# saiakarsh193/GenVox

Hardware: AMD Instinct MI355X
Metric: mel-frames/sec (teacher-forced batch) (higher is better)
Workload: dtype f32

## Files before the change

genvox_amd/_lib.py:

```python
from __future__ import annotations

import ctypes as C
import os

_HERE = os.path.dirname(os.path.abspath(__file__))
LIB_PATH = os.path.join(_HERE, os.environ.get("GVX_LIB", "libgenvox_amd.so"))


class GvxError(RuntimeError):
    pass


class gvx_dims(C.Structure):
    _fields_ = [(n, C.c_int32) for n in (
        "n_tokens", "embed_dim", "enc_kernel", "enc_n_conv", "prenet_dim", "att_rnn_dim", "dec_rnn_dim", "att_dim",
        "att_loc_filters", "att_loc_kernel", "postnet_dim", "postnet_kernel", "postnet_n_conv", "n_mels")]


class gvx_weight_desc(C.Structure):
    _fields_ = [("name", C.c_char_p), ("data", C.c_void_p), ("numel", C.c_int64)]


_vp, _i, _sz, _f, _l = C.c_void_p, C.c_int, C.c_size_t, C.c_float, C.c_long

# ... 137 lines not shown
    "gvx_wav_finalize_ragged": (_i, [_vp, _i, C.c_long, _vp, _i, _i, _i, C.POINTER(C.c_double), C.POINTER(C.c_double), _i, _vp, _vp, _vp]),
    "gvx_wav_to_mel_ragged_workspace_bytes": (_sz, [_vp, _i, C.c_long, _i]),
    "gvx_wav_trim_bounds": (_i, [_vp, _i, _i, C.c_long, _vp, _i, _f, _vp, _vp]),
    "gvx_wav_to_mel_ragged": (_i, [_vp, _vp, _i, _vp, _vp, _i, C.c_long, _vp, _i, _i, _i, _f, _i, _vp, _vp, _vp, _vp, _vp, _sz, _vp]),
    "gvx_resample_uses_lds_table": (_i, [_i, _i, _i]),
    "gvx_wav_mixdown": (_i, [_vp, _i, _i, C.c_long, _i, _vp, _vp]),
    "gvx_wav_resample_ragged": (_i, [_vp, _i, _i, C.c_long, _vp, _i, _i, _vp, _i, _vp, C.c_long, _vp, _vp]),
    "gvx_alignment_stats": (_i, [_vp, _vp, _vp, _i, _i, _i, _vp, _vp, _vp, _vp, _vp, _vp]),
    "gvx_mel_project": (_i, [_vp, _i, _i, _i, _vp, _i, _vp, _vp]),
    "gvx_dtw_workspace_bytes": (_sz, [_i, _i, _i, _i]),
    "gvx_dtw_uses_lds_tables": (_i, [_i, _i, _i]),
    "gvx_dtw_distance": (_i, [_vp, _vp, _vp, _vp, _i, _i, _i, _i, _vp, _vp, _vp, _sz, _vp]),
    "gvx_monotonic_align_workspace_bytes": (_sz, [_i, _i, _i]),
    "gvx_monotonic_align_uses_lds": (_i, [_i, _i]),
    "gvx_monotonic_align": (_i, [_vp, _vp, _vp, _i, _i, _i, _f, _vp, _vp, _vp, _vp, _vp, _vp, _vp, _sz, _vp]),
    "gvx_duration_scale": (_i, [_vp, _vp, _vp, _i, _i, _f, _vp, _vp, _vp, _vp, _vp]),
    "gvx_mel_time_warp": (_i, [_vp, _vp, _vp, _vp, _i, _i, _i, _i, _i, _vp, _vp, _vp, _vp, _vp]),
    "gvx_pitch_frames": (_i, [_l, _i]),
    "gvx_pitch_tile_frames": (_i, [C.POINTER(gvx_pitch_params)]),
    "gvx_pitch_yin": (_i, [_vp, _vp, _i, _l, C.POINTER(gvx_pitch_params), _vp, _vp, _vp, _vp, _vp]),
    "gvx_f0_compare": (_i, [_vp, _vp, _vp, _vp, _i, _i, _vp, _vp, _vp, _vp, _vp]),
    "gvx_psola_max_marks": (_l, [_l, _i]),
    "gvx_psola_max_grains": (_l, [_l, _i]),
    "gvx_psola_plan": (_i, [_vp, _vp, _vp, _vp, _i, _l, C.POINTER(gvx_psola_params), _vp, _vp, _vp, _vp, _vp, _vp, _vp]),
    "gvx_psola_synth": (_i, [_vp, _vp, _vp, _vp, _vp, _vp, _vp, _vp, _i, _l, C.POINTER(gvx_psola_params), _vp, _vp]),
    "gvx_melgan_blob_floats":(_sz, [C.POINTER(gvx_melgan_dims)]),
    "gvx_melgan_workspace_bytes": (_sz, [C.POINTER(gvx_melgan_dims), _i, _i]),
    "gvx_melgan_pack_weights_device": (_i, [C.POINTER(gvx_melgan_dims), C.POINTER(gvx_weight_desc), _i, _vp, _vp]),
    "gvx_melgan_create": (_i, [C.POINTER(gvx_melgan_dims), C.POINTER(_vp)]),
    "gvx_melgan_destroy": (None, [_vp]),
    "gvx_melgan_bind": (_i, [_vp, _vp]),
    "gvx_melgan_forward": (_i, [_vp, _vp, _vp, _i, _i, _vp, C.POINTER(_vp), _vp, _sz, _vp]),
    "gvx_melgan_timing_enable": (_i, [_vp, _i]),
    "gvx_melgan_stage_times_ms": (_i, [_vp, C.POINTER(_f), C.POINTER(_i)]),
    "gvx_melgan_tape_bytes": (_sz, [C.POINTER(gvx_melgan_dims), _i, _i]),
    "gvx_melgan_tape_layout": (_i, [C.POINTER(gvx_melgan_dims), _i, _i, C.POINTER(gvx_melgan_tape_entry), _i]),
    "gvx_melgan_backward_workspace_bytes": (_sz, [C.POINTER(gvx_melgan_dims), _i, _i]),
    "gvx_melgan_forward_train": (_i, [_vp, _vp, _vp, _i, _i, _vp, _vp, _sz, _vp, _sz, _vp]),
    "gvx_melgan_backward": (_i, [_vp, _vp, _vp, _i, _i, _vp, _sz, C.POINTER(gvx_weight_desc), _i, _vp, _vp, _sz, _vp]),
    "gvx_hifigan_blob_floats": (_sz, [C.POINTER(gvx_hifigan_dims)]),
    "gvx_hifigan_workspace_bytes": (_sz, [C.POINTER(gvx_hifigan_dims), _i, _i]),
    "gvx_hifigan_pack_weights_device": (_i, [C.POINTER(gvx_hifigan_dims), C.POINTER(gvx_weight_desc), _i, _vp, _vp]),
    "gvx_hifigan_create": (_i, [C.POINTER(gvx_hifigan_dims), C.POINTER(_vp)]),
    "gvx_hifigan_destroy": (None, [_vp]),
    "gvx_hifigan_bind": (_i, [_vp, _vp]),
    "gvx_hifigan_forward": (_i, [_vp, _vp, _vp, _i, _i, _vp, C.POINTER(_vp), _vp, _sz, _vp]),
    "gvx_hifigan_timing_enable": (_i, [_vp, _i]),
    "gvx_hifigan_stage_times_ms": (_i, [_vp, C.POINTER(_f), C.POINTER(_i)]),
    "gvx_hifigan_backward_stage_times_ms": (_i, [_vp, C.POINTER(_f), C.POINTER(_i)]),
    "gvx_hifigan_tape_bytes": (_sz, [C.POINTER(gvx_hifigan_dims), _i, _i]),
    "gvx_hifigan_tape_layout": (_i, [C.POINTER(gvx_hifigan_dims), _i, _i, C.POINTER(gvx_melgan_tape_entry), _i]),
    "gvx_hifigan_backward_workspace_bytes": (_sz, [C.POINTER(gvx_hifigan_dims), _i, _i]),
    "gvx_hifigan_forward_train": (_i, [_vp, _vp, _vp, _i, _i, _vp, _vp, _sz, _vp, _sz, _vp]),
    "gvx_hifigan_backward": (_i, [_vp, _vp, _vp, _i, _i, _vp, _sz, C.POINTER(gvx_weight_desc), _i, _vp, _vp, _sz, _vp]),
    "gvx_melgan_disc_blob_floats": (_sz, [C.POINTER(gvx_melgan_disc_dims)]),
    "gvx_melgan_disc_pack_weights_device": (_i, [C.POINTER(gvx_melgan_disc_dims), C.POINTER(gvx_weight_desc), _i, _vp, _vp]),
    "gvx_melgan_disc_create": (_i, [C.POINTER(gvx_melgan_disc_dims), C.POINTER(_vp)]),
    "gvx_melgan_disc_destroy": (None, [_vp]),
    "gvx_melgan_disc_bind": (_i, [_vp, _vp]),
    "gvx_melgan_disc_layout": (_i, [C.POINTER(gvx_melgan_disc_dims), _i, _i, C.POINTER(gvx_melgan_disc_entry), _i]),
    "gvx_melgan_disc_features_bytes": (_sz, [C.POINTER(gvx_melgan_disc_dims), _i, _i]),
    "gvx_melgan_disc_workspace_bytes": (_sz, [C.POINTER(gvx_melgan_disc_dims), _i, _i, _i]),
    "gvx_melgan_disc_forward": (_i, [_vp, _vp, _vp, _i, _i, _vp, _sz, _vp, _sz, _vp]),
    "gvx_melgan_disc_backward": (_i, [_vp, _vp, _vp, _i, _i, _vp, _vp, C.POINTER(gvx_weight_desc), _i, _vp, _vp, _sz, _vp]),
    "gvx_hifigan_mpd_blob_floats": (_sz, [C.POINTER(gvx_hifigan_mpd_dims)]),
    "gvx_hifigan_mpd_pack_weights_device": (_i, [C.POINTER(gvx_hifigan_mpd_dims), C.POINTER(gvx_weight_desc), _i, _vp, _vp]),
    "gvx_hifigan_mpd_create": (_i, [C.POINTER(gvx_hifigan_mpd_dims), C.POINTER(_vp)]),
    "gvx_hifigan_mpd_destroy": (None, [_vp]),
    "gvx_hifigan_mpd_bind": (_i, [_vp, _vp]),
    "gvx_hifigan_mpd_layout": (_i, [C.POINTER(gvx_hifigan_mpd_dims), _i, _i, C.POINTER(gvx_hifigan_mpd_entry), _i]),
    "gvx_hifigan_mpd_features_bytes": (_sz, [C.POINTER(gvx_hifigan_mpd_dims), _i, _i]),
    "gvx_hifigan_mpd_workspace_bytes": (_sz, [C.POINTER(gvx_hifigan_mpd_dims), _i, _i, _i]),
    "gvx_hifigan_mpd_forward": (_i, [_vp, _vp, _vp, _i, _i, _vp, _sz, _vp, _sz, _vp]),
    "gvx_hifigan_mpd_backward": (_i, [_vp, _vp, _vp, _i, _i, _vp, _vp, C.POINTER(gvx_weight_desc), _i, _vp, _vp, _sz, _vp]),
    "gvx_hifigan_mpd_timing_enable": (_i, [_vp, _i]),
    "gvx_hifigan_mpd_layer_times_ms": (_i, [_vp, C.POINTER(_f), C.POINTER(_f), C.POINTER(_i)]),
    "gvx_stft_loss_create": (_i, [C.POINTER(gvx_stft_resolution), _i, _f, _f, _f, C.POINTER(_vp)]),
    "gvx_stft_loss_destroy": (None, [_vp]),
    "gvx_stft_loss_workspace_bytes": (_sz, [_vp, _i, _l]),
    "gvx_stft_loss": (_i, [_vp, _vp, _vp, _vp, _i, _l, _vp, _vp, _vp, C.POINTER(gvx_stft_loss_debug), _vp, _sz, _vp]),
    "gvx_kernel_timing_enable": (_i, [_vp, _i]),
    "gvx_model_set_persistent_attention": (_i, [_vp, _i]),
    "gvx_model_set_resident_kernels": (_i, [_vp, _i]),
    "gvx_teacher_forced_rows_per_call": (_i, [_vp, _i]),
    "gvx_teacher_forced_resident": (_i, [_vp, _i, _i]),
    "gvx_teacher_forced_loop_kind": (_i, [_vp, _i, _i]),
    "gvx_autoregressive_loop_kind": (_i, [_vp, _i, _i]),
    "gvx_autoregressive_windowed_loop_kind": (_i, [_vp, _i, _i]),
    "gvx_kernel_times_ms": (_i, [_vp, C.POINTER(_f), C.POINTER(_f), C.POINTER(_i)]),
}

_lib = None


def load() -> C.CDLL:
    global _lib
    if _lib is not None:
        return _lib
    if not os.path.exists(LIB_PATH):
        raise ImportError(
            f"{LIB_PATH} not found: build the gfx950 library first (python -m genvox_amd.build, or "
            f"__graft_entry__.build()). genvox_amd has no CPU or eager fallback.")
    import torch

    lib = C.CDLL(LIB_PATH)
    for name, (res, args) in SIGNATURES.items():
        fn = getattr(lib, name)
        fn.restype = res
        fn.argtypes = args
    _lib = lib
    return lib


def check(rc: int) -> None:
    if rc != 0:
        msg = load().gvx_last_error()
        raise GvxError(f"genvox_amd error {rc}: {msg.decode() if msg else '?'}")
```

genvox_amd/build.py:

```python
from __future__ import annotations

import glob
import os
import subprocess
import sys
from concurrent.futures import ThreadPoolExecutor

HERE = os.path.dirname(os.path.abspath(__file__))
CSRC = os.path.join(HERE, "csrc")
LIB = os.path.join(HERE, "libgenvox_amd.so")
SOURCES = ["gemm_f32.hip", "skinny.hip", "dec_resident.hip", "attention.hip", "attn_persist.hip", "misc.hip", "griffinlim.hip", "wav_finalize.hip", "wav_to_mel.hip", "resample.hip", "eval_metrics.hip", "mas.hip", "time_warp.hip", "melgan.hip", "melgan_train.hip", "melgan_disc.hip", "hifigan.hip", "hifigan_train.hip", "hifigan_disc.hip", "pitch.hip", "psola.hip", "stft_loss.hip",
           "train_conv.hip", "train_ops.hip", "train_bptt_decoder.hip", "train_bptt_encoder.hip", "train_guided.hip", "gvx_pack.hip", "gvx_decoder.hip", "gvx_api.hip"]
ARCH = "gfx950"
HIPCC = os.environ.get("HIPCC", "/opt/rocm/bin/hipcc")
CXXFLAGS = ["-O3", "-std=c++17", "-fPIC", f"--offload-arch={ARCH}", "-Wall", "-Wno-unused-function",
            "-ffp-contract=off"]


def _newer(a: str, b: str) -> bool:
    return not os.path.exists(b) or os.path.getmtime(a) > os.path.getmtime(b)


def build(force: bool = False, verbose: bool = True, stamps: bool = False) -> str:
    objs, jobs = [], []
    flags = CXXFLAGS + (["-DGVX_STAMPS"] if stamps else []) + os.environ.get("GVX_EXTRA_FLAGS", "").split()
    lib = LIB.replace(".so", "_stamps.so") if stamps else LIB
    if os.environ.get("GVX_LIB_NAME"):
        lib = os.path.join(HERE, os.environ["GVX_LIB_NAME"])
    sfx = ".stamps.o" if stamps else ".o"
    if os.environ.get("GVX_LIB_NAME"):
        sfx = "." + os.environ["GVX_LIB_NAME"] + ".o"
    headers = sorted(glob.glob(os.path.join(CSRC, "*.h"))) + [os.path.join(os.path.dirname(HERE), "include", "genvox_amd.h")]
    for src in SOURCES:
        s = os.path.join(CSRC, src)
        o = os.path.join(CSRC, src.replace(".hip", sfx))
        objs.append(o)
        if force or _newer(s, o) or any(_newer(h, o) for h in headers):
            jobs.append([HIPCC, *flags, "-c", s, "-o", o])

    def run(cmd):
        if verbose:
            print(" ".join(cmd), flush=True)
        subprocess.run(cmd, check=True)

    if jobs:
        with ThreadPoolExecutor(max_workers=min(4, len(jobs))) as ex:
            list(ex.map(run, jobs))
    if jobs or not os.path.exists(lib):
        run([HIPCC, "-shared", "-fPIC", f"--offload-arch={ARCH}", *objs, "-L/opt/rocm/lib", "-lrocfft", "-Wl,-rpath,/opt/rocm/lib", "-o", lib])
    if not stamps and not os.environ.get("GVX_LIB_NAME"):
        variant = LIB.replace(".so", "_stamps.so")
        if os.path.exists(variant) and os.path.getmtime(variant) < os.path.getmtime(headers[-1]):
            os.remove(variant)
    return lib


if __name__ == "__main__":
    print(build(force="--force" in sys.argv, stamps="--stamps" in sys.argv))
```

genvox_amd/csrc/gemm_f32.hip:

```cpp
#include "gvx_kernels.h"

#include <cstdlib>

namespace gvx {

using f32x16 = __attribute__((ext_vector_type(16))) float;

constexpr int BK32 = 32;

__device__ __forceinline__ long row_off(const RowMap& m, int row) {
    return (long)(row / m.R) * m.s1 + (long)(row % m.R) * m.s0;
}

template <int WR, int WC, int TM, int TN, bool KMAJ = false, int BK = BK32>
__device__ __forceinline__ void gemm_f32_body(const GemmParams& p, const int block_x, const int tid, float* smem) {
    constexpr int LDS_LD = BK + 4;
    static_assert(BK == 32 || (BK == 64 && !KMAJ), "k-tiles of 32, or 64 for the row-major form");
    constexpr int BM = WR * TM * 32;
    constexpr int BN = WC * TN * 32;
    constexpr int NT = WR * WC * 64;
    constexpr int TPR = BK / 4;
    constexpr int RPP = NT / TPR;
    constexpr int A_V4 = (BM + RPP - 1) / RPP;
    constexpr int B_V4 = (BN + RPP - 1) / RPP;
    static_assert(!KMAJ || NT == 256, "the K-major loaders are written for 256 threads");
    float* As = smem;
    float* Bs = smem + 2 * BM * LDS_LD;

    const int lane = tid & 63, wave = tid >> 6;
    const int wr = wave / WC, wc = wave % WC;
    const int r = lane & 31, h = lane >> 5;
    const int n_tiles = (p.N + BN - 1) / BN;
    const int mt = block_x / n_tiles, nt = block_x % n_tiles;
    const int m0 = p.m_begin + mt * BM, n0 = nt * BN;
    const int k_begin = p.splitk > 1 ? (int)blockIdx.y * p.kchunk : 0;
    const int k_end = p.splitk > 1 ? min(p.K, k_begin + p.kchunk) : p.K;
    float* const Cout = p.C + (p.splitk > 1 ? (long)blockIdx.y * p.c_split : 0);

    const int ld_row = tid / TPR, ld_c4 = tid % TPR;
    const float* a_ptr[A_V4]; bool a_ok[A_V4];
    const float* b_ptr[B_V4]; bool b_ok[B_V4];
    constexpr int A_MQ = BM / 4, B_NQ = BN / 4;
    constexpr int A_P = (8 * A_MQ + 255) / 256, B_P = (8 * B_NQ + 255) / 256;
    const int amq = tid % A_MQ, akq = tid / A_MQ, bnq = tid % B_NQ, bkq = tid / B_NQ;
    const int a_col = min(m0 + 4 * amq, p.M - 4), b_col = min(n0 + 4 * bnq, p.N - 4);
    int ak_g[A_P], ak_i[A_P], bk_g[B_P], bk_i[B_P];
    long a_safe = 0, b_safe = 0;
    float4 ka_reg[A_P][4], kb_reg[B_P][4];
    if (KMAJ) {
#pragma unroll
        for (int i = 0; i < A_P; ++i) { const int k = k_begin + 4 * (akq + (256 / A_MQ) * i); ak_g[i] = k / p.amap.R; ak_i[i] = k - ak_g[i] * p.amap.R; }
#pragma unroll
        for (int i = 0; i < B_P; ++i) { const int k = k_begin + 4 * (bkq + (256 / B_NQ) * i); bk_g[i] = k / p.wmap.R; bk_i[i] = k - bk_g[i] * p.wmap.R; }
        a_safe = row_off(p.amap, k_begin); b_safe = row_off(p.wmap, k_begin);
    }
    if (!KMAJ) {
#pragma unroll
        for (int i = 0; i < A_V4; ++i) {
            int m = m0 + ld_row + RPP * i;
            a_ok[i] = m < p.M;
            a_ptr[i] = p.A + (a_ok[i] ? row_off(p.amap, m) : 0);
        }
#pragma unroll
        for (int i = 0; i < B_V4; ++i) {
            int n = n0 + ld_row + RPP * i;
            b_ok[i] = n < p.N;
            b_ptr[i] = p.W + (b_ok[i] ? (long)n * p.ldw : 0);
        }
    }
    float4 a_reg[A_V4], b_reg[B_V4];

#define GEMM_KMAJ_LOAD(NP, QPP, KQ, KG, KI, MAP, SAFE, PTR, COL, REG)                                        \
        _Pragma("unroll") for (int i = 0; i < NP; ++i) {                                                    \
            const int c_ = KQ + QPP * i;                                                                    \
            if (c_ < BK / 4) {                                                                              \
                const int kq_ = (K0_) + 4 * c_;                                                             \
                int g_ = KG[i], x_ = KI[i];                                                                 \
                _Pragma("unroll") for (int j = 0; j < 4; ++j) {                                             \
                    const bool ok_ = kq_ + j < k_end;                                                       \
                    REG[i][j] = *reinterpret_cast<const float4*>(PTR + (ok_ ? (long)g_ * MAP.s1 + (long)x_ * MAP.s0 : SAFE) + COL); \
                    if (++x_ == MAP.R) { x_ = 0; ++g_; }                                                    \
                }                                                                                           \
                x_ = KI[i] + BK; g_ = KG[i];                                                                \
                while (x_ >= MAP.R) { x_ -= MAP.R; ++g_; }                                                  \
                KI[i] = x_; KG[i] = g_;                                                                     \
            }                                                                                               \
        }
#define GEMM_LOAD_TILE(K0)                                                                                  \
    if (KMAJ) {                                                                                             \
        const int K0_ = (K0);                                                                               \
        GEMM_KMAJ_LOAD(A_P, (256 / A_MQ), akq, ak_g, ak_i, p.amap, a_safe, p.A, a_col, ka_reg)              \
        GEMM_KMAJ_LOAD(B_P, (256 / B_NQ), bkq, bk_g, bk_i, p.wmap, b_safe, p.W, b_col, kb_reg)              \
    } else                                                                                                  \
    {                                                                                                       \
        const int k_ = (K0) + 4 * ld_c4;                                                                    \
        const bool k_ok_ = k_ < k_end;                                                                      \
        const long a_koff_ = (long)(k_ >> 3) * p.a_kblk + (k_ & 7);                                         \
        _Pragma("unroll") for (int i = 0; i < A_V4; ++i) {                                                  \
            if (BM % RPP != 0 && ld_row + RPP * i >= BM) continue;                                          \
            a_reg[i] = *reinterpret_cast<const float4*>(a_ptr[i] + (k_ok_ ? a_koff_ : 0));                  \
        }                                                                                                   \
        _Pragma("unroll") for (int i = 0; i < B_V4; ++i) {                                                  \
            if (BN % RPP != 0 && ld_row + RPP * i >= BN) continue;                                          \
            b_reg[i] = *reinterpret_cast<const float4*>(b_ptr[i] + (k_ok_ ? k_ : 0));                       \
        }                                                                                                   \
    }
#define GEMM_KMAJ_STORE(NP, QPP, KQ, SM, ROWS, RQ, REG, BUF)                                                 \
        _Pragma("unroll") for (int i = 0; i < NP; ++i) {                                                    \
            const int c_ = KQ + QPP * i;                                                                    \
            if (c_ < BK / 4) {                                                                              \
                float* d_ = &SM[((BUF) * ROWS + 4 * RQ) * LDS_LD + 4 * c_];                                 \
                const int kq_ = (KS_) + 4 * c_;    \
                const bool o0_ = kq_ < k_end, o1_ = kq_ + 1 < k_end, o2_ = kq_ + 2 < k_end, o3_ = kq_ + 3 < k_end;   \
                *reinterpret_cast<float4*>(d_) = make_float4(o0_ ? REG[i][0].x : 0.f, o1_ ? REG[i][1].x : 0.f, o2_ ? REG[i][2].x : 0.f, o3_ ? REG[i][3].x : 0.f);              \
                *reinterpret_cast<float4*>(d_ + LDS_LD) = make_float4(o0_ ? REG[i][0].y : 0.f, o1_ ? REG[i][1].y : 0.f, o2_ ? REG[i][2].y : 0.f, o3_ ? REG[i][3].y : 0.f);     \
                *reinterpret_cast<float4*>(d_ + 2 * LDS_LD) = make_float4(o0_ ? REG[i][0].z : 0.f, o1_ ? REG[i][1].z : 0.f, o2_ ? REG[i][2].z : 0.f, o3_ ? REG[i][3].z : 0.f); \
                *reinterpret_cast<float4*>(d_ + 3 * LDS_LD) = make_float4(o0_ ? REG[i][0].w : 0.f, o1_ ? REG[i][1].w : 0.f, o2_ ? REG[i][2].w : 0.f, o3_ ? REG[i][3].w : 0.f); \
            }                                                                                               \
        }
#define GEMM_STORE_TILE(BUF, K0)                                                                            \
    if (KMAJ) {                                                                                             \
        const int KS_ = (K0);                                                                               \
        GEMM_KMAJ_STORE(A_P, (256 / A_MQ), akq, As, BM, amq, ka_reg, BUF)                                   \
        GEMM_KMAJ_STORE(B_P, (256 / B_NQ), bkq, Bs, BN, bnq, kb_reg, BUF)                                   \
    } else                                                                                                  \
    {                                                                                                       \
        const bool s_ok_ = (K0) + 4 * ld_c4 < k_end;    \
        _Pragma("unroll") for (int i = 0; i < A_V4; ++i)                                                    \
            if (BM % RPP == 0 || ld_row + RPP * i < BM)                                                     \
                *reinterpret_cast<float4*>(&As[((BUF) * BM + ld_row + RPP * i) * LDS_LD + 4 * ld_c4]) =     \
                    make_float4(s_ok_ ? a_reg[i].x : 0.f, s_ok_ ? a_reg[i].y : 0.f, s_ok_ ? a_reg[i].z : 0.f, s_ok_ ? a_reg[i].w : 0.f); \
        _Pragma("unroll") for (int i = 0; i < B_V4; ++i)                                                    \
            if (BN % RPP == 0 || ld_row + RPP * i < BN)                                                     \
                *reinterpret_cast<float4*>(&Bs[((BUF) * BN + ld_row + RPP * i) * LDS_LD + 4 * ld_c4]) =     \
                    make_float4(s_ok_ ? b_reg[i].x : 0.f, s_ok_ ? b_reg[i].y : 0.f, s_ok_ ? b_reg[i].z : 0.f, s_ok_ ? b_reg[i].w : 0.f); \
    }
#define GEMM_COMPUTE_TILE(BUF) GEMM_COMPUTE_KGS(BUF, 0, BK / 8)
#define GEMM_COMPUTE_KGS(BUF, KG0, KG1)              \
    {                                                                                                       \
        const float* a_base = &As[((BUF) * BM + wr * TM * 32 + r) * LDS_LD + 4 * h];                        \
        const float* b_base = &Bs[((BUF) * BN + wc * TN * 32 + r) * LDS_LD + 4 * h];                        \
        _Pragma("unroll") for (int kg = (KG0); kg < (KG1); ++kg) {                                          \
            float4 af[TM], bf[TN];                                                                          \
            _Pragma("unroll") for (int i = 0; i < TM; ++i)                                                  \
                af[i] = *reinterpret_cast<const float4*>(a_base + i * 32 * LDS_LD + 8 * kg);                \
            _Pragma("unroll") for (int j = 0; j < TN; ++j)                                                  \
                bf[j] = *reinterpret_cast<const float4*>(b_base + j * 32 * LDS_LD + 8 * kg);                \
            _Pragma("unroll") for (int i = 0; i < TM; ++i)                                                  \
                _Pragma("unroll") for (int j = 0; j < TN; ++j) {                                            \
                    acc[i][j] = __builtin_amdgcn_mfma_f32_32x32x2f32(af[i].x, bf[j].x, acc[i][j], 0, 0, 0); \
                    acc[i][j] = __builtin_amdgcn_mfma_f32_32x32x2f32(af[i].y, bf[j].y, acc[i][j], 0, 0, 0); \
                    acc[i][j] = __builtin_amdgcn_mfma_f32_32x32x2f32(af[i].z, bf[j].z, acc[i][j], 0, 0, 0); \
                    acc[i][j] = __builtin_amdgcn_mfma_f32_32x32x2f32(af[i].w, bf[j].w, acc[i][j], 0, 0, 0); \
                }                                                                                           \
        }                                                                                                   \
    }

    f32x16 acc[TM][TN];
#pragma unroll
    for (int i = 0; i < TM; ++i)
#pragma unroll
        for (int j = 0; j < TN; ++j)
#pragma unroll
            for (int q = 0; q < 16; ++q) acc[i][j][q] = 0.f;

    const int nkt = (k_end - k_begin + BK - 1) / BK;
    GEMM_LOAD_TILE(k_begin)
    GEMM_STORE_TILE(0, k_begin)
    __syncthreads();
    int kt = 0;
    for (; kt + 1 < nkt; ++kt) {
        const int cur = kt & 1;
        GEMM_LOAD_TILE(k_begin + (kt + 1) * BK)
        __builtin_amdgcn_sched_barrier(0);
        GEMM_COMPUTE_KGS(cur, 0, BK / 8 - 1)
        __builtin_amdgcn_sched_barrier(0);
        GEMM_COMPUTE_KGS(cur, BK / 8 - 1, BK / 8)
        GEMM_STORE_TILE(cur ^ 1, k_begin + (kt + 1) * BK)
        __syncthreads();
    }
    GEMM_COMPUTE_TILE(kt & 1)
#undef GEMM_LOAD_TILE
#undef GEMM_KMAJ_LOAD
#undef GEMM_KMAJ_STORE
#undef GEMM_STORE_TILE
#undef GEMM_COMPUTE_TILE
#undef GEMM_COMPUTE_KGS

#pragma unroll
    for (int i = 0; i < TM; ++i) {
#pragma unroll
        for (int q = 0; q < 16; ++q) {
            const int m = m0 + (wr * TM + i) * 32 + (q & 3) + 8 * (q >> 2) + 4 * h;
            if (m >= p.M) continue;
            const long c_off = row_off(p.cmap, m);
            const int grp = m / p.cmap.R, idx = m - grp * p.cmap.R;
            const bool live = !p.row_len || idx < p.row_len[grp];
            const bool halo_front = p.c_halo > 0 && idx < p.c_halo;
            const bool halo_back = p.c_halo > 0 && idx >= p.cmap.R - p.c_halo;
            const long halo_step = (long)p.c_halo * p.cmap.s0;
#pragma unroll
            for (int j = 0; j < TN; ++j) {
                const int n = n0 + (wc * TN + j) * 32 + r;
                if (n >= p.N) continue;
                float v = acc[i][j][q];
                if (p.bias) v += p.bias[n];
                if (p.act == ACT_RELU) v = fmaxf(v, 0.f);
                else if (p.act == ACT_TANH) v = tanhf(v);
                if (p.keep) v = p.keep[(long)m * p.keep_ld + n] ? 2.f * v : 0.f;
                const long col = (long)(n >> 3) * p.c_nblk + (n & 7);
                Cout[c_off + col] = live ? v : 0.f;
                if (halo_front) Cout[c_off - halo_step + col] = 0.f;
                if (halo_back) Cout[c_off + halo_step + col] = 0.f;
            }
        }
    }
}

template <int WR, int WC, int TM, int TN, bool KMAJ = false, int BK = BK32>
__global__ __launch_bounds__(WR * WC * 64) void gemm_f32_kernel(GemmParams p) {
    extern __shared__ __attribute__((aligned(16))) float smem[];
    gemm_f32_body<WR, WC, TM, TN, KMAJ, BK>(p, (int)blockIdx.x, (int)threadIdx.x, smem);
}

template <int WR, int WC, int TM, int TN, int BK = BK32>
static size_t lds_bytes_cfg() { return (size_t)2 * (WR * TM * 32 + WC * TN * 32) * (BK + 4) * sizeof(float); }

template <int WR, int WC, int TM, int TN, bool KMAJ = false, int BK = BK32>
static hipError_t init_cfg() {
    return hipFuncSetAttribute(reinterpret_cast<const void*>(gemm_f32_kernel<WR, WC, TM, TN, KMAJ, BK>),
                               hipFuncAttributeMaxDynamicSharedMemorySize, (int)lds_bytes_cfg<WR, WC, TM, TN, BK>());
}

hipError_t gemm_init() {
    hipError_t e = init_cfg<2, 2, 2, 2>();
    if (e != hipSuccess) return e;
    e = init_cfg<2, 2, 1, 2>();
    if (e != hipSuccess) return e;
    e = init_cfg<4, 1, 1, 3>();
    if (e != hipSuccess) return e;
    e = init_cfg<2, 3, 1, 1>();
    if (e != hipSuccess) return e;
    e = init_cfg<4, 2, 1, 2>();
    if (e != hipSuccess) return e;
    e = init_cfg<2, 2, 1, 1>();
    if (e != hipSuccess) return e;
    e = init_cfg<2, 2, 2, 2, true>();
    if (e != hipSuccess) return e;
    e = init_cfg<2, 2, 1, 2, true>();
    if (e != hipSuccess) return e;
    return init_cfg<4, 1, 1, 1>();
}

template <int WR, int WC, int TM, int TN, bool KMAJ = false, int BK = BK32>
static hipError_t launch_cfg(const GemmParams& p, hipStream_t s) {
    constexpr int BM = WR * TM * 32, BN = WC * TN * 32;
    const int grid = ((p.M - p.m_begin + BM - 1) / BM) * ((p.N + BN - 1) / BN);
    gemm_f32_kernel<WR, WC, TM, TN, KMAJ, BK><<<dim3(grid, p.splitk > 1 ? p.splitk : 1), dim3(WR * WC * 64), lds_bytes_cfg<WR, WC, TM, TN, BK>(), s>>>(p);
    return hipGetLastError();
}

static bool four_waves() {
    static const bool on = [] { const char* e = std::getenv("GVX_GEMM_8W"); return e && e[0] == '0'; }();
    return on;
}

GemmPlan plan_gemm(const GemmParams& p) {
    GemmPlan pl{hipSuccess, 0, 0};
    if (p.M <= 0 || p.N <= 0) return pl;
    if (p.kmajor) {
        if ((p.M & 3) || (p.N & 3) || p.M < 4 || p.N < 4 || ((p.amap.s0 | p.amap.s1 | p.wmap.s0 | p.wmap.s1) & 3)) { pl.err = hipErrorInvalidValue; return pl; }
        const long t128 = (long)((p.M + 127) / 128) * ((p.N + 127) / 128);
        pl.tile = t128 < 384 ? 2212 : 2222;
        return pl;
    }
    if (p.K & 3) { pl.err = hipErrorInvalidValue; return pl; }
    if (p.N <= 32) { pl.tile = 4111; return pl; }
    if (p.N <= 96) {
        pl.tile = p.M - p.m_begin <= 4096 ? 2311 : 4113;
        return pl;
    }
    const long n_tiles = (p.N + 127) / 128, tiles128 = (long)((p.M + 127) / 128) * n_tiles;
    if (tiles128 < 192) { pl.tile = 2211; return pl; }
    if (tiles128 < 384) { pl.tile = 2212; return pl; }
    pl.tile = four_waves() ? 2222 : 4212;
    const long rem = tiles128 % 256;
    if (p.splitk <= 1 && p.m_begin == 0 && rem > 0 && rem <= 64) {
        const long rows_big = ((tiles128 - rem) / n_tiles) * 128;
        if (rows_big > 0 && rows_big < p.M) pl.rows_big = (int)rows_big;
    }
    return pl;
}

static hipError_t launch_tile(int tile, const GemmParams& p, hipStream_t s) {
    switch (tile) {
        case 4111: return launch_cfg<4, 1, 1, 1>(p, s);
        case 2311: return launch_cfg<2, 3, 1, 1>(p, s);
        case 4113: return launch_cfg<4, 1, 1, 3>(p, s);
        case 2211: return launch_cfg<2, 2, 1, 1>(p, s);
        case 2212: return p.kmajor ? launch_cfg<2, 2, 1, 2, true>(p, s) : launch_cfg<2, 2, 1, 2>(p, s);
        case 2222: return p.kmajor ? launch_cfg<2, 2, 2, 2, true>(p, s) : launch_cfg<2, 2, 2, 2>(p, s);
        case 4212: return launch_cfg<4, 2, 1, 2>(p, s);
    }
    return hipErrorInvalidValue;
}

hipError_t launch_gemm(const GemmParams& p, hipStream_t s) {
    const GemmPlan pl = plan_gemm(p);
    if (pl.err != hipSuccess || pl.tile == 0) return pl.err;
    if (pl.rows_big == 0) return launch_tile(pl.tile, p, s);
    GemmParams a = p, b = p;
    a.M = pl.rows_big;
    b.m_begin = pl.rows_big;
    const hipError_t e = launch_tile(pl.tile, a, s);
    if (e != hipSuccess) return e;
    return launch_tile(2211, b, s);
}

void set_splitk(GemmParams& p, int splitk) {
    p.kchunk = ((p.K + splitk - 1) / splitk + 63) / 64 * 64;
    p.splitk = (p.K + p.kchunk - 1) / p.kchunk;
}

__global__ void splitk_reduce_kernel(const float* part, int splitk, long MN, int N, const float* bias, float* out, long ldc) {
    for (long i = (long)blockIdx.x * blockDim.x + threadIdx.x; i < MN; i += (long)gridDim.x * blockDim.x) {
        float v = part[i];
        for (int s = 1; s < splitk; ++s) v += part[(long)s * MN + i];
        const int n = (int)(i % N);
        if (bias) v += bias[n];
        out[(i / N) * ldc + n] = v;
    }
}

hipError_t launch_gemm_splitk(const GemmParams& p0, int splitk, float* scratch, hipStream_t s) {
    if (splitk <= 1) return launch_gemm(p0, s);
    if (p0.act != ACT_NONE || p0.keep || p0.row_len || p0.c_halo || p0.c_nblk != 8 || p0.cmap.s1 != 0 || p0.cmap.R < p0.M || !scratch)
        return hipErrorInvalidValue;
    GemmParams p = p0;
    set_splitk(p, splitk);
    p.C = scratch; p.cmap = RowMap{p.M, 0, (long)p.N};
    p.c_split = (long)p.M * p.N;
    p.bias = nullptr;
    hipError_t e = launch_gemm(p, s);
    if (e != hipSuccess) return e;
    const long MN = (long)p.M * p.N;
    long blocks = (MN + 255) / 256;
    if (blocks > 2048) blocks = 2048;
    splitk_reduce_kernel<<<dim3((unsigned)blocks), dim3(256), 0, s>>>(scratch, p.splitk, MN, p.N, p0.bias, p0.C, p0.cmap.s0);
    return hipGetLastError();
}

}
```

genvox_amd/csrc/gvx_api.hip:

```cpp
#include "gvx_internal.h"

namespace gvx {
#ifdef GVX_STAMPS
hipError_t read_stamps_skinny(unsigned long long* host96);
hipError_t read_stamps_attention(unsigned long long* host96);
hipError_t read_stamps_persist(unsigned long long* host96);
hipError_t read_wg_spans(unsigned long long* host1024);
hipError_t read_stamps_resident(unsigned long long* host480);
hipError_t read_wg_stamps_resident(unsigned long long* host896);
hipError_t read_wg_stamps_resident_ar(unsigned long long* host896);
hipError_t read_row_stamps_persist_ar(unsigned long long* host256);
hipError_t read_loc_stamps_persist(unsigned long long* host32);
hipError_t read_row_stamps_persist(unsigned long long* host512);
#endif
hipError_t skinny_init();
hipError_t gemm_init();
hipError_t attention_init();
hipError_t attention_persistent_init();
}

using namespace gvx;

namespace {
thread_local std::string g_err;
std::mutex g_capture_mutex;
}
namespace gvx {
int set_error(int code, const char* msg) { g_err = msg; return code; }

int fail(int code, const char* fmt, ...) {
    char buf[1024];
    va_list ap;
    va_start(ap, fmt);
    vsnprintf(buf, sizeof buf, fmt, ap);
    va_end(ap);
    g_err = buf;
    return code;
}

std::mutex& capture_mutex() { return g_capture_mutex; }

WsPlan make_ws_plan(const gvx_model* m, int B, int L, int T, int mode) {
    const gvx_dims& d = m->d;
    const int E = d.embed_dim, H = E / 2, M = d.n_mels, P = d.prenet_dim, A = d.att_rnn_dim, D = d.dec_rnn_dim;
    const int pe = (d.enc_kernel - 1) / 2, pp = (d.postnet_kernel - 1) / 2;
    WsPlan w{};
    size_t off = 0;
    auto take = [&](size_t floats) { size_t o = off; off = align_up(off + floats * sizeof(float), 256); return o; };
    w.flags = take(128);
    w.sync = take(HANDOFF_WORDS);
    w.xa = take((size_t)B * (L + 2 * pe) * E);
    w.xb = take((size_t)B * (L + 2 * pe) * E);
    w.xg = take((size_t)B * L * 8 * H);
    w.enc_h = take((size_t)2 * 2 * B * H);
    w.enc_c = take((size_t)2 * B * H);
    w.memory = take((size_t)B * L * E);
    w.len_copy = take((size_t)B);
    w.pm = take((size_t)B * L * d.att_dim);
    w.frames = take((size_t)(T + 1) * B * M);
    w.pre1 = take((size_t)(T + 1) * B * P);
    w.prenet = take((size_t)(T + 1) * B * P);
    w.h_a = take((size_t)RS_HA_SLOTS * B * A);
    w.c_a = take((size_t)B * A);
    w.c_d = take((size_t)B * D);
    w.hc = take((size_t)(T + 1) * B * (D + E));
    w.w_cum = take((size_t)B * L);
    w.q_slab = take((size_t)(A / 8) * B * d.att_dim);
    w.proj = take((size_t)B * T * m->PSB());
    w.energies = take((size_t)B * L);
    w.align_tm = take((size_t)T * B * L);
    w.loc = take((size_t)B * L * d.att_dim);
    w.p_slab = take((size_t)(D / 8) * B * m->PSB());
    w.p_ctx = take((size_t)B * m->PSB());
    w.att_part = take((size_t)2 * B * 4 * A);
    w.dec_part = take((size_t)2 * B * 4 * D);
    w.pre_gate = take(mode == WS_TEACHER_FORCED && plan_teacher_forced(m, B, L, TF_INFERENCE).pre_gate ? (size_t)T * B * 4 * A : 0);
    w.xchg = take(attention_persistent_xchg_floats(B));
    w.ar_masks = take(((size_t)2 * T * B * P + 3) / 4);
    const int cmax = d.postnet_dim > M ? d.postnet_dim : M;
    w.ya = take((size_t)B * (T + 2 * pp) * cmax);
    w.yb = take((size_t)B * (T + 2 * pp) * cmax);
    w.total = off;
    return w;
}

gvx_model::GraphSet* touch_graph_set(gvx_model* m, std::vector<gvx_model::GraphSet>& cache, const gvx_model::LoopKey& key) {
    gvx_model::GraphSet* hit = nullptr;
    for (auto& gs : cache)
        if (gs.key == key) hit = &gs;
    if (!hit) {
        if (cache.size() >= gvx_model::GRAPH_SETS) {
            size_t lru = 0;
            for (size_t i = 1; i < cache.size(); ++i)
                if (cache[i].last_use < cache[lru].last_use) lru = i;
            for (auto e : cache[lru].execs)
                if (e) (void)hipGraphExecDestroy(e);
            cache.erase(cache.begin() + lru);
        }
        cache.emplace_back();
        hit = &cache.back();
        hit->key = key;
    }
    ++hit->sightings;
    hit->last_use = ++m->use_clock;
    return hit;
}

int check_common(const gvx_model* m, int B, int L, int T, void* ws, size_t ws_bytes, int mode) {
    if (!m) return fail(GVX_ERR_INVALID_ARG, "null model");
    if (!m->dev_blob) return fail(GVX_ERR_STATE, "weights not bound (call gvx_model_bind_blob)");
    if (B < 1 || B > 64) return fail(GVX_ERR_UNSUPPORTED, "batch %d not in [1, 64] (shard larger batches across calls / GPUs)", B);
    if (L < 1 || T < 1) return fail(GVX_ERR_INVALID_ARG, "L and T must be >= 1");
    if (!ws) return fail(GVX_ERR_WORKSPACE, "null workspace");
    if (reinterpret_cast<uintptr_t>(ws) & 255) return fail(GVX_ERR_WORKSPACE, "workspace must be 256-byte aligned");
    const size_t need = make_ws_plan(m, B, L, T, mode).total;
    if (ws_bytes < need) return fail(GVX_ERR_WORKSPACE, "workspace too small: %zu < %zu bytes", ws_bytes, need);
    if (!attention_supported(L, m->d.att_dim, m->d.att_loc_filters, m->d.att_loc_kernel, m->d.embed_dim))
        return fail(GVX_ERR_UNSUPPORTED, "L = %d is too long for the attention kernels' LDS budget", L);
    return GVX_OK;
}

}

namespace {

int check_dims(const gvx_dims& d) {
    if (d.n_tokens < 1) return fail(GVX_ERR_INVALID_ARG, "n_tokens must be >= 1");
    const int dims8[] = {d.embed_dim, d.prenet_dim, d.att_rnn_dim, d.dec_rnn_dim, d.att_dim, d.postnet_dim, d.n_mels};
    const char* names[] = {"embed_dim", "prenet_dim", "att_rnn_dim", "dec_rnn_dim", "att_dim", "postnet_dim", "n_mels"};
    for (int i = 0; i < 7; ++i)
        if (dims8[i] < 8 || dims8[i] % 8) return fail(GVX_ERR_UNSUPPORTED, "%s = %d must be a positive multiple of 8", names[i], dims8[i]);
    if (d.embed_dim % 16) return fail(GVX_ERR_UNSUPPORTED, "embed_dim = %d must be a multiple of 16 (BiLSTM halves are multiples of 8)", d.embed_dim);
    if (d.att_dim > 256) return fail(GVX_ERR_UNSUPPORTED, "att_dim = %d > 256 is not supported", d.att_dim);
    if (d.att_loc_filters < 1 || d.att_loc_filters > 32) return fail(GVX_ERR_UNSUPPORTED, "att_loc_filters = %d must be in [1, 32]", d.att_loc_filters);
    const int ks[] = {d.enc_kernel, d.att_loc_kernel, d.postnet_kernel};
    for (int k : ks)
        if (k < 1 || k % 2 == 0) return fail(GVX_ERR_UNSUPPORTED, "kernel size %d must be odd (the reference pads (k-1)/2 on both sides)", k);
    if (d.enc_n_conv < 1 || d.enc_n_conv > MAX_CONV || d.postnet_n_conv < 1 || d.postnet_n_conv > MAX_CONV)
        return fail(GVX_ERR_UNSUPPORTED, "number of convolutions must be in [1, %d]", MAX_CONV);
    return GVX_OK;
}

void read_knobs(gvx_model* m) {
    auto env = [](const char* name) { const char* e = std::getenv(name); return e ? e : ""; };
    auto flag = [&](const char* name, bool dflt) { const char c = env(name)[0]; return c == '\0' ? dflt : dflt ? c != '0' : c == '1'; };
    auto number = [&](const char* name, int dflt) { const char* e = env(name); return e[0] ? std::atoi(e) : dflt; };
    m->use_graph = !flag("GVX_NO_GRAPH", false);
    m->capture_first = flag("GVX_GRAPH_FIRST", false);
    m->attn_one_launch = !flag("GVX_ATTN_SPLIT", false);
    m->attn_persistent = flag("GVX_ATTN_PERSISTENT", true);
    for (const char* name : {"AMD_SERIALIZE_KERNEL", "HIP_LAUNCH_BLOCKING"})
        if (env(name)[0] != '\0' && env(name)[0] != '0') m->attn_persistent = false;
    m->ar_resident = flag("GVX_AR_RESIDENT", false);
    m->ar_split_h = flag("GVX_AR_SPLIT_H", true);
    m->enc_persistent = flag("GVX_ENC_PERSISTENT", true);
    m->enc_fork_after = number("GVX_ENC_FORK_AFTER", 1);
    m->train_resident = flag("GVX_TRAIN_RESIDENT", true);
    m->train_resident_loop = flag("GVX_TRAIN_RESIDENT_LOOP", true);
    m->tf_rows64 = flag("GVX_TF_ROWS64", false);
    m->tf_resident = flag("GVX_TF_RESIDENT", true);
    m->ar_resident_loop = flag("GVX_AR_RESIDENT_LOOP", true);
    m->tf_long_rows_224 = flag("GVX_TF_LONG_224", true);
    m->attn_prefetch = flag("GVX_ATTN_PREFETCH", true);
    m->pa_depth = number("GVX_PA_DEPTH", 4) == 6 ? 6 : 4;
    m->side_pool = env("GVX_SIDE_POOL")[0] == '2' ? 2u : 1u;
    m->spin_limit = (unsigned)std::strtoul(env("GVX_HANDOFF_SPIN_LIMIT"), nullptr, 10);
    m->rs_debug = number("GVX_RS_DEBUG", 0);
    m->debug_skip_resident = flag("GVX_DEBUG_SKIP_RESIDENT", false);
    m->debug_enc_skip_block = number("GVX_DEBUG_ENC_SKIP_BLOCK", -1);
    m->debug_plan = std::getenv("GVX_DEBUG_PLAN") != nullptr;
}

}

extern "C" {

const char* gvx_last_error(void) { return g_err.c_str(); }
int gvx_version(void) { return 1; }

int gvx_model_create(const gvx_dims* dims, gvx_model** out) {
    if (!dims || !out) return fail(GVX_ERR_INVALID_ARG, "null argument");
    int rc = check_dims(*dims);
    if (rc != GVX_OK) return rc;
    gvx_model* m = new gvx_model();
    m->d = *dims;
    m->blob = make_blob_layout(*dims);
    read_knobs(m);
    *out = m;
    return GVX_OK;
}

void gvx_model_destroy(gvx_model* m) {
    if (m) {
        if (m->gather_off) (void)hipFree(m->gather_off);
        if (m->gather_tid) (void)hipFree(m->gather_tid);
    }
    if (!m) return;
    if (m->ev_valid)
        for (auto& e : m->ev) (void)hipEventDestroy(e);
    for (auto& e : m->kev) (void)hipEventDestroy(e);
    m->drop_graphs();
    if (m->cap_stream) (void)hipStreamDestroy(m->cap_stream);
    if (m->pa_fork) (void)hipEventDestroy(m->pa_fork);
    if (m->pa_join) (void)hipEventDestroy(m->pa_join);
    if (m->enc_mid) (void)hipEventDestroy(m->enc_mid);
    if (m->ar_done_host) (void)hipHostFree(m->ar_done_host);
    for (hipEvent_t e : m->ar_ev)
        if (e) (void)hipEventDestroy(e);
    delete m;
}

size_t gvx_model_blob_bytes(const gvx_model* m) { return m ? m->blob.total * sizeof(float) : 0; }

int gvx_model_bind_blob(gvx_model* m, const void* device_blob) {
    if (!m || !device_blob) return fail(GVX_ERR_INVALID_ARG, "null argument");
    if (reinterpret_cast<uintptr_t>(device_blob) & 255) return fail(GVX_ERR_INVALID_ARG, "blob must be 256-byte aligned");
    if (m->dev_blob != device_blob) m->drop_graphs();
    m->dev_blob = reinterpret_cast<const float*>(device_blob);
    HIP_TRY(gemm_init());
    HIP_TRY(skinny_init());
    HIP_TRY(attention_init());
    HIP_TRY(attention_persistent_init());
    HIP_TRY(decoder_resident_init());
    return GVX_OK;
}

size_t gvx_workspace_bytes(const gvx_model* m, int B, int L, int T) {
    if (!m || B < 1 || L < 1 || T < 1) return 0;
    return make_ws_plan(m, B, L, T).total;
}

size_t gvx_workspace_bytes_autoregressive(const gvx_model* m, int B, int L, int max_steps) {
    if (!m || B < 1 || L < 1 || max_steps < 1) return 0;
    return make_ws_plan(m, B, L, max_steps, WS_AUTOREGRESSIVE).total;
}

}

namespace {

int conv_layer(const gvx_model* m, const float* in, float* out, int B, int T, int cin, int cout, int k, size_t w_off, size_t b_off,
               int act, int out_halo, hipStream_t s) {
    const int p = (k - 1) / 2;
    GemmParams g{};
    g.A = in; g.amap = RowMap{T, (long)(T + 2 * p) * cin, (long)cin};
    g.W = m->dev_blob + w_off; g.ldw = (long)k * cin;
    g.C = out + (long)out_halo * cout; g.cmap = RowMap{T, (long)(T + 2 * out_halo) * cout, (long)cout};
    g.bias = m->dev_blob + b_off;
    g.M = B * T; g.N = cout; g.K = k * cin; g.act = act;
    HIP_TRY(launch_gemm(g, s));
    return GVX_OK;
}

// ... 11 lines not shown
    float* cur = xa;
    float* nxt = xb;
    if (conv_out) {
        HIP_TRY(launch_to_channels_last(conv_out, xa, B, E, L, pe, nullptr, s));
    } else {
        HIP_TRY(launch_embed(tokens, m->dev_blob + m->blob.emb, d.n_tokens, xa, xb, B, L, E, pe, flags + FLAG_TOKEN, s));
        for (int i = 0; i < d.enc_n_conv; ++i) {
            if (dense_done && i == m->enc_fork_after) { HIP_TRY(hipEventRecord(dense_done, s)); dense_done = nullptr; }
            int rc = conv_layer(m, cur, nxt, B, L, E, E, d.enc_kernel, m->blob.enc_w[i], m->blob.enc_b[i], ACT_RELU, pe, s);
            if (rc != GVX_OK) return rc;
            float* t = cur; cur = nxt; nxt = t;
        }
    }
    if (dense_done) HIP_TRY(hipEventRecord(dense_done, s));
    {
        GemmParams g{};
        g.A = cur + (long)pe * E; g.amap = RowMap{L, (long)(L + 2 * pe) * E, (long)E};
        g.W = m->dev_blob + m->blob.enc_wih; g.ldw = E;
        g.C = xg; g.cmap = RowMap{B * L, 0, (long)8 * H};
        g.bias = m->dev_blob + m->blob.enc_bih;
        g.M = B * L; g.N = 8 * H; g.K = E; g.act = ACT_NONE;
        HIP_TRY(launch_gemm(g, s));
    }
    const bool resident = m->enc_persistent && encoder_persistent_supported(B, H);
    if (!resident) HIP_TRY(zero_async(enc_h, (size_t)4 * B * H * sizeof(float), s));
    if (!resident) HIP_TRY(zero_async(enc_c, (size_t)2 * B * H * sizeof(float), s));
    float* mem_ws = ws_ptr<float>(ws, wp.memory);
    if (!resident) HIP_TRY(zero_async(mem_ws, (size_t)B * L * E * sizeof(float), s));
    const int32_t* len_ws = nullptr;
    if (lengths) {
        int32_t* lc = ws_ptr<int32_t>(ws, wp.len_copy);
        HIP_TRY(hipMemcpyAsync(lc, lengths, (size_t)B * sizeof(int32_t), hipMemcpyDeviceToDevice, s));
        len_ws = lc;
    }
    auto enqueue = [&](hipStream_t st) -> int {
        for (int step = 0; step < L; ++step) {
            SkinnyJob jobs[2];
            for (int dir = 0; dir < 2; ++dir) {
                SkinnyJob& J = jobs[dir];
                std::memset(&J, 0, sizeof J);
                float* h_cur = enc_h + ((size_t)dir * 2 + (step & 1)) * B * H;
                float* h_nxt = enc_h + ((size_t)dir * 2 + ((step + 1) & 1)) * B * H;
                J.Wp = m->dev_blob + m->blob.enc_whh_frag[dir];
                J.x[0] = XSeg{h_cur, H};
                J.N = 4 * H; J.nkg = H / 8; J.mode = 0; J.B = B;
                J.c = enc_c + (size_t)dir * B * H;
                J.h_out = h_nxt;
                J.addend = xg + (size_t)dir * 4 * H; J.add_bs = (long)L * 8 * H; J.add_ts = 8 * H;
                J.lengths = len_ws; J.step = step; J.reverse = dir; J.seq_len = L;
                J.seq_out = mem_ws + (size_t)dir * H; J.seq_bs = (long)L * E; J.seq_ts = E;
                if (c_seq_out) J.c_seq_out = c_seq_out + (size_t)dir * H;
                J.h_prev = h_cur;
            }
            HIP_TRY(launch_skinny(jobs, 2, SK_ENCODER, st));
        }
        return GVX_OK;
    };
    if (resident) {
        unsigned* sync = ws_ptr<unsigned>(ws, wp.sync);
        void* const zp[2] = {enc_h, sync + HANDOFF_TIMEOUT};
        const size_t zb[2] = {(size_t)4 * B * H * sizeof(float), sizeof(unsigned)};
        HIP_TRY(launch_zero_many(zp, zb, 2, s));
        EncPersistParams ep{};
        ep.Wp[0] = m->dev_blob + m->blob.enc_whh_frag[0]; ep.Wp[1] = m->dev_blob + m->blob.enc_whh_frag[1];
        ep.xg = xg; ep.lengths = len_ws; ep.hx = enc_h; ep.seq_out = mem_ws; ep.c_seq_out = c_seq_out;
        ep.sync = sync; ep.spin_limit = m->spin_limit; ep.B = B; ep.L = L; ep.H = H;
        ep.debug_skip_block = m->debug_enc_skip_block;
        HIP_TRY(launch_encoder_persistent(ep, s));
        float* outs[2] = {mem_ws, c_seq_out};
        const size_t counts[2] = {(size_t)B * L * E, (size_t)B * L * E};
        HIP_TRY(launch_poison_on_timeout(sync + HANDOFF_TIMEOUT, flags + FLAG_TIMEOUT, outs, counts, c_seq_out ? 2 : 1, s));
    } else {
        const gvx_model::LoopKey key{ws, mem_ws, m->dev_blob, B, L, 0, lengths != nullptr};
        const int rc = run_chunk(m, m->use_graph && !c_seq_out ? touch_graph_set(m, m->enc_graphs, key) : nullptr, 0, s, enqueue);
        if (rc != GVX_OK) return rc;
    }
    if (xg_out) HIP_TRY(hipMemcpyAsync(xg_out, xg, (size_t)B * L * 8 * H * sizeof(float), hipMemcpyDeviceToDevice, s));
    if (memory_out != mem_ws)
        HIP_TRY(hipMemcpyAsync(memory_out, mem_ws, (size_t)B * L * E * sizeof(float), hipMemcpyDeviceToDevice, s));
    return GVX_OK;
}

int postnet_impl(gvx_model* m, const float* mel_in, const int32_t* mel_lengths, int B, int T, float* mel_post_out, float* ya,
                 float* yb, hipStream_t s) {
    const gvx_dims& d = m->d;
    const int M = d.n_mels, pp = (d.postnet_kernel - 1) / 2, n = d.postnet_n_conv;
    HIP_TRY(launch_to_channels_last(mel_in, ya, B, M, T, pp, mel_lengths, s));
    float* cur = ya;
    float* nxt = yb;
    for (int i = 0; i < n; ++i) {
        const int cin = i == 0 ? M : d.postnet_dim, cout = i == n - 1 ? M : d.postnet_dim;
        const bool last = i == n - 1;
        const int out_halo = last ? 0 : pp;
        const bool fused_halo = out_halo > 0 && T >= out_halo;
        if (out_halo > 0 && !fused_halo) HIP_TRY(launch_zero_halo(nxt, B, T, pp, cout, s));
        GemmParams g{};
        g.A = cur; g.amap = RowMap{T, (long)(T + 2 * pp) * cin, (long)cin};
        g.W = m->dev_blob + m->blob.post_w[i]; g.ldw = (long)d.postnet_kernel * cin;
        g.C = nxt + (long)out_halo * cout; g.cmap = RowMap{T, (long)(T + 2 * out_halo) * cout, (long)cout};
        g.bias = m->dev_blob + m->blob.post_b[i];
        g.M = B * T; g.N = cout; g.K = d.postnet_kernel * cin; g.act = last ? ACT_NONE : ACT_TANH;
        g.row_len = last ? nullptr : mel_lengths;
        g.c_halo = fused_halo ? out_halo : 0;
        HIP_TRY(launch_gemm(g, s));
        float* t = cur; cur = nxt; nxt = t;
    }
    HIP_TRY(launch_residual_to_channels_first(mel_in, cur, mel_post_out, B, M, T, mel_lengths, s));
    return GVX_OK;
}

struct PostnetPlan { size_t ya, yb, total; };
PostnetPlan make_postnet_plan(const gvx_model* m, int B, int T) {
    const gvx_dims& d = m->d;
    const int pp = (d.postnet_kernel - 1) / 2, cmax = d.postnet_dim > d.n_mels ? d.postnet_dim : d.n_mels;
    const size_t buf = align_up((size_t)B * (T + 2 * pp) * cmax * sizeof(float), 256);
    PostnetPlan p;
    p.ya = align_up((128 + HANDOFF_WORDS) * sizeof(float), 256);
    p.yb = p.ya + buf;
    p.total = p.yb + buf;
    return p;
}

}

extern "C" {

int gvx_teacher_forced_rows_per_call(const gvx_model* m, int L) {
    if (!m) return 0;
    return plan_teacher_forced(m, 64, L, TF_INFERENCE).kind != 0 ? 64 : 32;
}

int gvx_teacher_forced_resident(const gvx_model* m, int B, int L) {
    if (!m || B < 1 || L < 1) return 0;
    return plan_teacher_forced(m, B, L, TF_INFERENCE).kind != 0 ? 1 : 0;
}

int gvx_teacher_forced_loop_kind(const gvx_model* m, int B, int L) {
    if (!m || B < 1 || L < 1) return 0;
    return plan_teacher_forced(m, B, L, TF_INFERENCE).kind;
}

int gvx_autoregressive_loop_kind(const gvx_model* m, int B, int L) {
    if (!m || B < 1 || L < 1) return 0;
    return plan_autoregressive(m, B, L).kind;
}

int gvx_autoregressive_windowed_loop_kind(const gvx_model* m, int B, int L) {
    if (!m || B < 1 || L < 1) return 0;
    return plan_autoregressive(m, B, L, true).kind;
}

int gvx_debug_decoder_plan_windowed(const gvx_model* m, int B, int L, int* out) {
    if (!m || !out) return fail(GVX_ERR_INVALID_ARG, "null argument");
    if (B < 1 || L < 1) return fail(GVX_ERR_INVALID_ARG, "B, L >= 1 (got %d, %d)", B, L);
    const ArLoopPlan a = plan_autoregressive(m, B, L, true);
    out[0] = a.kind; out[1] = a.split_h; out[2] = a.fold; out[3] = a.graph;
    return GVX_OK;
}

int gvx_debug_decoder_plan(const gvx_model* m, int mode, int B, int L, int* out) {
    if (!m || !out) return fail(GVX_ERR_INVALID_ARG, "null argument");
    if (mode < 0 || mode > 2 || B < 1 || L < 1) return fail(GVX_ERR_INVALID_ARG, "mode must be 0, 1 or 2 and B, L >= 1 (got %d, %d, %d)", mode, B, L);
    const TfLoopPlan t = plan_teacher_forced(m, B, L, (TfMode)mode);
    const ArLoopPlan a = plan_autoregressive(m, B, L);
    const int v[12] = {t.kind, t.pa_layout, t.tile_layout, t.rows64, t.pre_gate, t.timeout_check, t.side_stream, t.graph,
                       a.kind, a.split_h, a.fold, a.graph};
    for (int i = 0; i < 12; ++i) out[i] = v[i];
    return GVX_OK;
}

long long gvx_debug_graph_replays(const gvx_model* m) { return m ? (long long)m->graph_replays : -1; }

int gvx_debug_encoder_resident(const gvx_model* m, int B) {
    if (!m || B < 1) return 0;
    return m->enc_persistent && encoder_persistent_supported(B, m->H()) ? 1 : 0;
}

int gvx_model_set_persistent_attention(gvx_model* m, int enable) {
    if (!m) return fail(GVX_ERR_INVALID_ARG, "null argument");
    m->attn_persistent = enable != 0;
    return GVX_OK;
}

int gvx_model_set_resident_kernels(gvx_model* m, int enable) {
    if (!m) return fail(GVX_ERR_INVALID_ARG, "null argument");
    m->attn_persistent = m->enc_persistent = m->tf_resident = enable != 0;
    if (!enable) m->ar_resident = false;
    return GVX_OK;
}

int gvx_workspace_status(const gvx_model* m, void* ws, size_t ws_bytes, void* stream, int32_t* host_out) {
    if (!m || !ws || !host_out) return fail(GVX_ERR_INVALID_ARG, "null argument");
    const WsPlan wp = make_ws_plan(m, 1, 1, 1, WS_AUTOREGRESSIVE);
    if (ws_bytes < wp.flags + 4 * sizeof(int32_t)) return fail(GVX_ERR_WORKSPACE, "workspace too small");
    hipStream_t s = (hipStream_t)stream;
    int32_t h[4] = {0, 0, 0, 0}, tmo = 0;
    int32_t* flags = ws_ptr<int32_t>(ws, wp.flags);
    HIP_TRY(hipMemcpyAsync(h, flags, sizeof h, hipMemcpyDeviceToHost, s));
    if (ws_bytes >= wp.sync + HANDOFF_WORDS * sizeof(unsigned))
        HIP_TRY(hipMemcpyAsync(&tmo, reinterpret_cast<const char*>(ws) + wp.sync + HANDOFF_TIMEOUT * sizeof(unsigned), sizeof tmo,
                               hipMemcpyDeviceToHost, s));
    HIP_TRY(zero_async(flags + FLAG_TOKEN, sizeof(int32_t), s));
    HIP_TRY(zero_async(flags + FLAG_TIMEOUT, sizeof(int32_t), s));
    if (ws_bytes >= wp.sync + HANDOFF_WORDS * sizeof(unsigned))
        HIP_TRY(zero_async(ws_ptr<unsigned>(ws, wp.sync) + HANDOFF_TIMEOUT, sizeof(unsigned), s));
    HIP_TRY(hipStreamSynchronize(s));
    host_out[0] = h[FLAG_TOKEN];
    host_out[1] = h[FLAG_TIMEOUT] ? h[FLAG_TIMEOUT] : tmo;
    return GVX_OK;
}

int gvx_encoder_forward(gvx_model* m, const int64_t* tokens, const int32_t* lengths, int B, int L, float* memory_out,
                        void* ws, size_t ws_bytes, void* stream) {
    int rc = check_common(m, B, L, 1, ws, ws_bytes, WS_AUTOREGRESSIVE);
    if (rc != GVX_OK) return rc;
    if (!tokens || !memory_out) return fail(GVX_ERR_INVALID_ARG, "null argument");
    return encoder_impl(m, tokens, lengths, B, L, memory_out, ws, make_ws_plan(m, B, L, 1, WS_AUTOREGRESSIVE), (hipStream_t)stream);
}

int gvx_decoder_teacher_forced(gvx_model* m, const float* memory, const int32_t* lengths, int B, int L, const float* mel_in, int T,
                               const uint8_t* keep_masks, float* mel_out, float* gate_out, float* align_out, void* ws,
                               size_t ws_bytes, void* stream) {
    int rc = check_common(m, B, L, T, ws, ws_bytes);
    if (rc != GVX_OK) return rc;
    if (!memory || !mel_in || !keep_masks || !mel_out || !gate_out || !align_out) return fail(GVX_ERR_INVALID_ARG, "null argument");
    const WsPlan wp = make_ws_plan(m, B, L, T);
    rc = decoder_tf_impl(m, memory, lengths, B, L, mel_in, T, keep_masks, mel_out, gate_out, align_out, ws, wp, (hipStream_t)stream);
    if (rc != GVX_OK) return rc;
    float* outs[3] = {mel_out, gate_out, align_out};
    const size_t counts[3] = {(size_t)B * m->d.n_mels * T, (size_t)B * T, (size_t)B * T * L};
    return poison_if_timed_out(m, B, L, ws, wp, outs, counts, 3, (hipStream_t)stream);
}

int gvx_encoder_lstm_forward(gvx_model* m, const float* conv_out, const int32_t* lengths, int B, int L, float* memory_out,
                             float* cell_states_out, float* input_preact_out, void* ws, size_t ws_bytes, void* stream) {
    int rc = check_common(m, B, L, 1, ws, ws_bytes, WS_AUTOREGRESSIVE);
    if (rc != GVX_OK) return rc;
    if (!conv_out || !memory_out) return fail(GVX_ERR_INVALID_ARG, "null argument");
    if (cell_states_out) HIP_TRY(zero_async(cell_states_out, (size_t)B * L * m->d.embed_dim * sizeof(float), (hipStream_t)stream));
    return encoder_impl(m, nullptr, lengths, B, L, memory_out, ws, make_ws_plan(m, B, L, 1, WS_AUTOREGRESSIVE), (hipStream_t)stream, conv_out,
                        cell_states_out, input_preact_out);
}

int gvx_decoder_teacher_forced_train(gvx_model* m, const float* memory, const int32_t* lengths, int B, int L, const float* mel_in, int T,
                                     const uint8_t* keep_masks, const uint8_t* att_keep, const uint8_t* dec_keep, float p_att, float p_dec,
                                     float* mel_out, float* gate_out, float* align_out, float* att_hidden_all, float* att_cell_all,
                                     float* dec_cell_all, float* dec_hidden_context_all, float* att_preact_all, float* dec_preact_all,
                                     void* ws, size_t ws_bytes, void* stream) {
    int rc = check_common(m, B, L, T, ws, ws_bytes);
    if (rc != GVX_OK) return rc;
    if (!memory || !mel_in || !keep_masks || !att_keep || !dec_keep || !mel_out || !gate_out || !align_out) return fail(GVX_ERR_INVALID_ARG, "null argument");
    if (!(p_att >= 0.f && p_att < 1.f && p_dec >= 0.f && p_dec < 1.f)) return fail(GVX_ERR_INVALID_ARG, "dropout probabilities must be in [0, 1)");
    if (plan_teacher_forced(m, B, L, TF_TRAIN_PARTIAL_TAPE).rows64)
        return fail(GVX_ERR_UNSUPPORTED, "training mode with %d rows on a GVX_TF_ROWS64 handle: the 64-row loop has no dropout and no tape (at most 32 rows per call)", B);
    hipStream_t s = (hipStream_t)stream;
    const int A = m->d.att_rnn_dim, D = m->d.dec_rnn_dim, E = m->d.embed_dim;
    const LstmDropout tr{att_keep, dec_keep, 1.f / (1.f - p_att), 1.f / (1.f - p_dec), att_hidden_all, att_cell_all, dec_cell_all, att_preact_all, dec_preact_all};
    if (att_hidden_all) HIP_TRY(zero_async(att_hidden_all, (size_t)B * A * sizeof(float), s));
    if (att_cell_all) HIP_TRY(zero_async(att_cell_all, (size_t)B * A * sizeof(float), s));
    if (dec_cell_all) HIP_TRY(zero_async(dec_cell_all, (size_t)B * D * sizeof(float), s));
    const WsPlan wp = make_ws_plan(m, B, L, T);
    rc = decoder_tf_impl(m, memory, lengths, B, L, mel_in, T, keep_masks, mel_out, gate_out, align_out, ws, wp, s, false, &tr);
    if (rc != GVX_OK) return rc;
    {
        float* outs[3] = {mel_out, gate_out, align_out};
        const size_t counts[3] = {(size_t)B * m->d.n_mels * T, (size_t)B * T, (size_t)B * T * L};
        rc = poison_if_timed_out(m, B, L, ws, wp, outs, counts, 3, s);
        if (rc != GVX_OK) return rc;
    }
    if (dec_hidden_context_all)
        HIP_TRY(hipMemcpyAsync(dec_hidden_context_all, ws_ptr<float>(ws, wp.hc), (size_t)(T + 1) * B * (D + E) * sizeof(float),
                               hipMemcpyDeviceToDevice, s));
    return GVX_OK;
}

int gvx_train_export(const gvx_model* m, const void* ws_c, size_t ws_bytes, int B, int L, int T, int what, float* dst, void* stream) {
    void* ws = const_cast<void*>(ws_c);
    if (!m || !ws || !dst) return fail(GVX_ERR_INVALID_ARG, "null argument");
    const WsPlan wp = make_ws_plan(m, B, L, T);
    if (ws_bytes < wp.total) return fail(GVX_ERR_WORKSPACE, "workspace too small");
    const gvx_dims& d = m->d;
    hipStream_t s = (hipStream_t)stream;
    const size_t rows = (size_t)(T + 1) * B;
    switch (what) {
        case 0: HIP_TRY(hipMemcpyAsync(dst, ws_ptr<float>(ws, wp.frames), rows * d.n_mels * sizeof(float), hipMemcpyDeviceToDevice, s)); break;
        case 1: HIP_TRY(hipMemcpyAsync(dst, ws_ptr<float>(ws, wp.pre1), rows * d.prenet_dim * sizeof(float), hipMemcpyDeviceToDevice, s)); break;
        case 2: return gvx_train_unblock(ws_ptr<float>(ws, wp.prenet), dst, T + 1, B, d.prenet_dim, stream);
        case 3: HIP_TRY(hipMemcpyAsync(dst, ws_ptr<float>(ws, wp.pm), (size_t)B * L * d.att_dim * sizeof(float), hipMemcpyDeviceToDevice, s)); break;
        default: return fail(GVX_ERR_INVALID_ARG, "gvx_train_export: unknown buffer %d", what);
    }
    return GVX_OK;
}

size_t gvx_postnet_workspace_bytes(const gvx_model* m, int B, int T) {
    if (!m || B < 1 || T < 1) return 0;
    return make_postnet_plan(m, B, T).total;
}

int gvx_postnet_forward(gvx_model* m, const float* mel_in, const int32_t* mel_lengths, int B, int T, float* mel_post_out, void* ws,
                        size_t ws_bytes, void* stream) {
    if (!m) return fail(GVX_ERR_INVALID_ARG, "null model");
    if (!m->dev_blob) return fail(GVX_ERR_STATE, "weights not bound (call gvx_model_bind_blob)");
    if (B < 1 || T < 1) return fail(GVX_ERR_INVALID_ARG, "B and T must be >= 1");
    if ((long)B * T > (1L << 30)) return fail(GVX_ERR_UNSUPPORTED, "B * T = %ld frames exceed the GEMM row index range", (long)B * T);
    if (!ws) return fail(GVX_ERR_WORKSPACE, "null workspace");
    if (reinterpret_cast<uintptr_t>(ws) & 255) return fail(GVX_ERR_WORKSPACE, "workspace must be 256-byte aligned");
    const PostnetPlan pp = make_postnet_plan(m, B, T);
    if (ws_bytes < pp.total) return fail(GVX_ERR_WORKSPACE, "workspace too small: %zu < %zu bytes", ws_bytes, pp.total);
    if (!mel_in || !mel_post_out) return fail(GVX_ERR_INVALID_ARG, "null argument");
    return postnet_impl(m, mel_in, mel_lengths, B, T, mel_post_out, ws_ptr<float>(ws, pp.ya), ws_ptr<float>(ws, pp.yb), (hipStream_t)stream);
}

int gvx_mask_padding(float* mel, float* mel_post, float* gate, const int32_t* mel_lengths, int B, int n_mels, int T, void* stream) {
    if (!mel_lengths || B < 1 || T < 1 || n_mels < 1) return fail(GVX_ERR_INVALID_ARG, "bad argument");
    HIP_TRY(launch_mask_padding(mel, mel_post, gate, mel_lengths, B, n_mels, T, (hipStream_t)stream));
    return GVX_OK;
}

int gvx_tacotron2_forward(gvx_model* m, const int64_t* tokens, const int32_t* token_lengths, int B, int L, const float* mel_in,
                          const int32_t* mel_lengths, int T, const uint8_t* keep_masks, float* mel_out, float* mel_post_out,
                          float* gate_out, float* align_out, void* ws, size_t ws_bytes, void* stream) {
    int rc = check_common(m, B, L, T, ws, ws_bytes);
    if (rc != GVX_OK) return rc;
    if (!tokens || !mel_in || !keep_masks || !mel_out || !gate_out || !align_out)
        return fail(GVX_ERR_INVALID_ARG, "null argument");
    hipStream_t s = (hipStream_t)stream;
    const WsPlan wp = make_ws_plan(m, B, L, T);
    const bool timed = m->timing && m->ev_valid;
    float* memory = ws_ptr<float>(ws, wp.memory);
    if (timed) HIP_TRY(hipEventRecord(m->ev[0], s));
    const bool overlap = plan_teacher_forced(m, B, L, TF_INFERENCE).side_stream;
    if (overlap) {
        rc = ensure_side_stream(m);
        if (rc != GVX_OK) return rc;
        HIP_TRY(hipEventRecord(m->pa_fork, s));
        HIP_TRY(hipStreamWaitEvent(m->pa_stream, m->pa_fork, 0));
        rc = encoder_impl(m, tokens, token_lengths, B, L, memory, ws, wp, m->pa_stream, nullptr, nullptr, nullptr, m->enc_mid);
        if (rc != GVX_OK) return rc;
        rc = decoder_init_states(m, memory, B, L, decoder_buffers(ws, wp), m->pa_stream);
        if (rc != GVX_OK) return rc;
        HIP_TRY(hipEventRecord(m->pa_join, m->pa_stream));
        HIP_TRY(hipStreamWaitEvent(s, m->enc_mid, 0));
        rc = decoder_prenet_part(m, B, L, mel_in, T, keep_masks, ws, wp, s);
        if (rc != GVX_OK) return rc;
        HIP_TRY(hipStreamWaitEvent(s, m->pa_join, 0));
    } else {
        rc = encoder_impl(m, tokens, token_lengths, B, L, memory, ws, wp, s);
        if (rc != GVX_OK) return rc;
    }
    if (timed) HIP_TRY(hipEventRecord(m->ev[1], s));
    rc = decoder_tf_impl(m, memory, token_lengths, B, L, mel_in, T, keep_masks, mel_out, gate_out, align_out, ws, wp, s, overlap);
    if (rc != GVX_OK) return rc;
    if (timed) HIP_TRY(hipEventRecord(m->ev[4], s));
    if (mel_post_out) {
        rc = postnet_impl(m, mel_out, nullptr, B, T, mel_post_out, ws_ptr<float>(ws, wp.ya), ws_ptr<float>(ws, wp.yb), s);
        if (rc != GVX_OK) return rc;
        if (mel_lengths) HIP_TRY(launch_mask_padding(mel_out, mel_post_out, gate_out, mel_lengths, B, m->d.n_mels, T, s));
    }
    float* outs[4] = {mel_out, gate_out, align_out, mel_post_out};
    const size_t nm = (size_t)B * m->d.n_mels * T;
    const size_t counts[4] = {nm, (size_t)B * T, (size_t)B * T * L, nm};
    rc = poison_if_timed_out(m, B, L, ws, wp, outs, counts, mel_post_out ? 4 : 3, s);
    if (rc != GVX_OK) return rc;
    if (timed) HIP_TRY(hipEventRecord(m->ev[5], s));
    return GVX_OK;
}

int gvx_tacotron2_loss(const float* mel_out, const float* mel_post_out, const float* gate_out, const float* mel_target,
                       const float* gate_target, int B, int n_mels, int T, float* loss_out, void* scratch, size_t scratch_bytes,
                       void* stream) {
    if (!mel_out || !mel_post_out || !gate_out || !mel_target || !gate_target || !loss_out || !scratch)
        return fail(GVX_ERR_INVALID_ARG, "null argument");
    if (B < 1 || n_mels < 1 || T < 1) return fail(GVX_ERR_INVALID_ARG, "B, n_mels and T must be >= 1");
    if (scratch_bytes < loss_scratch_bytes() || (reinterpret_cast<uintptr_t>(scratch) & 7))
        return fail(GVX_ERR_WORKSPACE, "scratch too small (%zu bytes needed) or not 8-byte aligned", loss_scratch_bytes());
    HIP_TRY(launch_tacotron2_loss(mel_out, mel_post_out, gate_out, mel_target, gate_target, (long)B * n_mels * T, (long)B * T,
                                  reinterpret_cast<double*>(scratch), loss_out, (hipStream_t)stream));
    return GVX_OK;
}

int gvx_prenet_masks_generate(uint8_t* masks_out, size_t n, uint64_t seed, void* stream) {
    if (!masks_out) return fail(GVX_ERR_INVALID_ARG, "null argument");
    HIP_TRY(launch_mask_gen(masks_out, n, seed, (hipStream_t)stream));
    return GVX_OK;
}

int gvx_stage_timing_enable(gvx_model* m, int enable) {
    if (!m) return fail(GVX_ERR_INVALID_ARG, "null model");
    if (enable && !m->ev_valid) {
        for (auto& e : m->ev) HIP_TRY(hipEventCreate(&e));
        m->ev_valid = true;
    }
    m->timing = enable != 0;
    return GVX_OK;
}

int gvx_kernel_timing_enable(gvx_model* m, int enable) {
    if (!m) return fail(GVX_ERR_INVALID_ARG, "null model");
    m->ktiming = enable != 0;
    return GVX_OK;
}

int gvx_kernel_times_ms(gvx_model* m, float* lstm_avg_ms, float* attn_avg_ms, int* n_steps) {
    if (!m || !lstm_avg_ms || !attn_avg_ms) return fail(GVX_ERR_INVALID_ARG, "null argument");
    if (m->n_lstm_ev < 1) return fail(GVX_ERR_STATE, "no timed decoder loop has run");
    HIP_TRY(hipEventSynchronize(m->kev[2]));
    float a = 0, b = 0;
    HIP_TRY(hipEventElapsedTime(&a, m->kev[0], m->kev[1]));
    HIP_TRY(hipEventElapsedTime(&b, m->kev[1], m->kev[2]));
    *lstm_avg_ms = a / m->n_lstm_ev;
    *attn_avg_ms = m->n_attn_ev > 0 ? b / m->n_attn_ev : 0.f;
    if (n_steps) *n_steps = m->n_lstm_ev;
    return GVX_OK;
}

int gvx_stage_times_ms(gvx_model* m, float* t5, int* launches) {
    if (!m || !t5) return fail(GVX_ERR_INVALID_ARG, "null argument");
    if (!m->ev_valid) return fail(GVX_ERR_STATE, "stage timing was not enabled");
    HIP_TRY(hipEventSynchronize(m->ev[5]));
    for (int i = 0; i < 5; ++i) HIP_TRY(hipEventElapsedTime(&t5[i], m->ev[i], m->ev[i + 1]));
    if (launches) *launches = m->last_decoder_launches;
    return GVX_OK;
}
#ifdef GVX_STAMPS
int gvx_debug_read_stamps_skinny(unsigned long long* host96) {
    HIP_TRY(hipDeviceSynchronize());
    HIP_TRY(gvx::read_stamps_skinny(host96));
    return GVX_OK;
}
int gvx_debug_read_stamps_persist(unsigned long long* host96) {
    HIP_TRY(hipDeviceSynchronize());
    HIP_TRY(gvx::read_stamps_persist(host96));
    return GVX_OK;
}
int gvx_debug_read_wg_spans(unsigned long long* host1024) {
    HIP_TRY(hipDeviceSynchronize());
    HIP_TRY(gvx::read_wg_spans(host1024));
    return GVX_OK;
// ... 35 lines not shown
```

genvox_amd/csrc/gvx_internal.h:

```cpp
#pragma once
#include "../../include/genvox_amd.h"
#include "gvx_kernels.h"

#include <cmath>
#include <cstdarg>
#include <cstdio>
#include <cstdlib>
#include <cstring>
#include <mutex>
#include <string>
#include <unordered_map>
#include <vector>

namespace gvx {

int fail(int code, const char* fmt, ...);

#define HIP_TRY(expr)                                                                          \
    do {                                                                                       \
        hipError_t _e = (expr);                                                                \
        if (_e != hipSuccess) return fail(GVX_ERR_HIP, "%s failed: %s", #expr, hipGetErrorString(_e)); \
    } while (0)

constexpr int MAX_CONV = 8;
constexpr double BN_EPS = 1e-5;

struct Blob {
    size_t emb;
    size_t enc_w[MAX_CONV], enc_b[MAX_CONV];
    size_t enc_wih, enc_bih, enc_whh_frag[2];
    size_t pre_w0, pre_w1, pre_w0_t, pre_w1_t;
    size_t att_frag, att_bias, att_wpre, wq_t, wmem, v, loc_conv, loc_dense;
    size_t dec_frag, dec_bias;
    size_t proj_w, proj_b, proj_frag, proj_hd_t, proj_ctx_frag, proj_ctx_t;
    size_t post_w[MAX_CONV], post_b[MAX_CONV];
    size_t total;
};
Blob make_blob_layout(const gvx_dims& d);

inline size_t frag_floats(int N, int K) { return (size_t)((N + 31) / 32) * (K / 8) * 64 * 4; }

struct WsPlan {
    size_t xa, xb, xg, enc_h, enc_c, flags, sync, memory;
    size_t pm, frames, pre1, prenet, h_a, c_a, c_d, hc, w_cum, q_slab, proj, energies, align_tm, len_copy, loc, ar_masks, p_slab, p_ctx;
    size_t att_part, dec_part, pre_gate, xchg;
    size_t ya, yb;
    size_t total;
};

}

struct gvx_model {
    gvx_dims d;
    gvx::Blob blob;
    const float* dev_blob = nullptr;
    bool use_graph = true;
    bool capture_first = false;
    bool attn_one_launch = true;
    bool attn_persistent = true;
    bool ar_resident = false;
    bool enc_persistent = true;
    bool ar_split_h = true;
    bool tf_rows64 = false;
    bool tf_resident = true;
    bool ar_resident_loop = true;
    bool tf_long_rows_224 = true;
    bool train_resident = true;
    bool train_resident_loop = true;
    bool attn_prefetch = true;
    int enc_fork_after = 1;
    int pa_depth = 4;
    unsigned side_pool = 1;
    unsigned spin_limit = 0;
    int rs_debug = 0;
    bool debug_skip_resident = false;
    int debug_enc_skip_block = -1;
    bool debug_plan = false;
    bool timing = false;
    hipEvent_t ev[6] = {nullptr, nullptr, nullptr, nullptr, nullptr, nullptr};
    bool ev_valid = false;
    int last_decoder_launches = 0;
    struct LoopKey {
        const void* ws; const void* memory; const void* blob; int B, L, T; bool has_len;
        float threshold = 0.f;
        int variant = 0;
        const void* centres = nullptr; int win_back = 0, win_ahead = 0;
        bool operator==(const LoopKey& o) const {
            return ws == o.ws && memory == o.memory && blob == o.blob && B == o.B && L == o.L && T == o.T &&
                   has_len == o.has_len && threshold == o.threshold && variant == o.variant && centres == o.centres &&
                   win_back == o.win_back && win_ahead == o.win_ahead;
        }
    };
    struct GraphSet {
        LoopKey key;
        int sightings = 0;
        uint64_t last_use = 0;
        std::vector<hipGraphExec_t> execs;
    };
    static constexpr size_t GRAPH_SETS = 4;
    std::vector<GraphSet> ar_graphs, loop_graphs, enc_graphs;
    uint64_t use_clock = 0;
    uint64_t graph_replays = 0;
    hipStream_t pa_stream = nullptr;
    hipEvent_t pa_fork = nullptr, pa_join = nullptr, enc_mid = nullptr;
    int32_t* ar_done_host = nullptr;
    hipEvent_t ar_ev[2] = {nullptr, nullptr};
    std::vector<std::string> gather_names;
    std::vector<int64_t> gather_numel;
    int32_t* gather_off = nullptr;
    uint8_t* gather_tid = nullptr;
    void drop_graphs() {
        for (auto* c : {&ar_graphs, &loop_graphs, &enc_graphs}) {
            for (auto& gs : *c)
                for (auto e : gs.execs)
                    if (e) (void)hipGraphExecDestroy(e);
            c->clear();
        }
    }
    hipStream_t cap_stream = nullptr;
    bool ktiming = false;
    std::vector<hipEvent_t> kev;
    int n_lstm_ev = 0, n_attn_ev = 0;
    int reserve_events(size_t n) {
        while (kev.size() < n) {
            hipEvent_t e;
            if (hipEventCreate(&e) != hipSuccess) return GVX_ERR_HIP;
            kev.push_back(e);
        }
        return GVX_OK;
    }
    int H() const { return d.embed_dim / 2; }
    int PS() const { return (d.n_mels + 1 + 3) & ~3; }
    int PSB() const { return (d.n_mels + 1 + 7) & ~7; }
};

namespace gvx {

enum TfMode : int { TF_INFERENCE = 0, TF_TRAIN_WHOLE_TAPE = 1, TF_TRAIN_PARTIAL_TAPE = 2 };
struct TfLoopPlan {
    int kind;
    int pa_layout;
    int tile_layout;
    bool rows64;
    bool pre_gate;
    bool timeout_check;
    bool side_stream;
    bool graph;
};
struct ArLoopPlan {
    int kind;
    bool split_h;
    bool fold;
    bool graph;
};
TfLoopPlan plan_teacher_forced(const gvx_model* m, int B, int L, TfMode mode);
ArLoopPlan plan_autoregressive(const gvx_model* m, int B, int L, bool windowed = false);

enum WsMode : int { WS_TEACHER_FORCED = 0, WS_AUTOREGRESSIVE = 1 };

constexpr int FLAG_TOKEN = 0;
constexpr int FLAG_AR_DONE = 1;
constexpr int FLAG_TIMEOUT = 2;
constexpr int FLAG_AR_FRAMES = 64;

WsPlan make_ws_plan(const gvx_model* m, int B, int L, int T, int mode = WS_TEACHER_FORCED);
int check_common(const gvx_model* m, int B, int L, int T, void* ws, size_t ws_bytes, int mode = WS_TEACHER_FORCED);

template <typename T>
T* ws_ptr(void* ws, size_t off) { return reinterpret_cast<T*>(reinterpret_cast<char*>(ws) + off); }

inline hipError_t zero_async(void* p, size_t bytes, hipStream_t s) { return hipMemsetAsync(p, 0, bytes, s); }

gvx_model::GraphSet* touch_graph_set(gvx_model* m, std::vector<gvx_model::GraphSet>& cache, const gvx_model::LoopKey& key);
std::mutex& capture_mutex();

template <class F>
int run_chunk(gvx_model* m, gvx_model::GraphSet* gs, size_t chunk, hipStream_t s, F&& enqueue) {
    if (!m->use_graph || !gs || (gs->sightings < 2 && !m->capture_first)) return enqueue(s);
    if (gs->execs.size() <= chunk) gs->execs.resize(chunk + 1, nullptr);
    hipGraphExec_t exec = gs->execs[chunk];
    if (!exec) {
        std::lock_guard<std::mutex> lock(capture_mutex());
        hipGraph_t graph = nullptr;
        if (!m->cap_stream) HIP_TRY(hipStreamCreateWithFlags(&m->cap_stream, hipStreamNonBlocking));
        HIP_TRY(hipStreamBeginCapture(m->cap_stream, hipStreamCaptureModeThreadLocal));
        const int rc = enqueue(m->cap_stream);
        const hipError_t ce = hipStreamEndCapture(m->cap_stream, &graph);
        if (rc != GVX_OK) { if (graph) (void)hipGraphDestroy(graph); return rc; }
        HIP_TRY(ce);
        HIP_TRY(hipGraphInstantiate(&exec, graph, nullptr, nullptr, 0));
        HIP_TRY(hipGraphDestroy(graph));
        gs->execs[chunk] = exec;
    }
    HIP_TRY(hipGraphLaunch(exec, s));
    ++m->graph_replays;
    return GVX_OK;
}

struct DecoderBuffers {
    float *pm, *frames, *pre1, *prenet, *h_a, *c_a, *c_d, *hc, *w_cum, *q_slab, *proj, *energies, *align_tm, *loc, *p_slab, *p_ctx;
    float *att_part, *dec_part, *pre_gate;
    int32_t* len_copy;
};
DecoderBuffers decoder_buffers(void* ws, const WsPlan& wp);

struct LstmDropout {
    const uint8_t* att_keep; const uint8_t* dec_keep; float att_scale, dec_scale;
    float* h_a_all; float* c_a_all; float* c_d_all;
    float* pre_a_all; float* pre_d_all;
};

int ensure_side_stream(gvx_model* m);
int decoder_init_states(gvx_model* m, const float* memory, int B, int L, const DecoderBuffers& db, hipStream_t s);
int decoder_prenet_part(gvx_model* m, int B, int L, const float* mel_in, int T, const uint8_t* keep_masks, void* ws, const WsPlan& wp,
                        hipStream_t s);
int decoder_tf_impl(gvx_model* m, const float* memory, const int32_t* lengths, int B, int L, const float* mel_in, int T,
                    const uint8_t* keep_masks, float* mel_out, float* gate_out, float* align_out, void* ws, const WsPlan& wp,
                    hipStream_t s, bool prenet_done = false, const LstmDropout* train = nullptr);
int poison_if_timed_out(const gvx_model* m, int B, int L, void* ws, const WsPlan& wp, float* const* outs, const size_t* counts, int n,
                        hipStream_t s);

}
```

genvox_amd/csrc/gvx_kernels.h:

```cpp
#pragma once
#include <hip/hip_runtime.h>
#include <stddef.h>
#include <stdint.h>

#ifdef GVX_STAMPS
namespace gvx { namespace { __device__ unsigned long long gvx_stamps[3][32]; } }
#define GVX_STAMP(k, i)                                                                         \
    do {                                                                                        \
        if (blockIdx.x == 0 && blockIdx.y == 0 && threadIdx.x == 0) gvx::gvx_stamps[k][i] = wall_clock64(); \
    } while (0)
#else
#define GVX_STAMP(k, i) do { } while (0)
#endif

namespace gvx {

int set_error(int code, const char* msg);

inline size_t align_up(size_t x, size_t a) { return (x + a - 1) / a * a; }

enum Act : int { ACT_NONE = 0, ACT_RELU = 1, ACT_TANH = 2 };

struct RowMap {
    int R;
    long s1, s0;
};

struct GemmParams {
    const float* A; RowMap amap; long a_kblk = 8;
    const float* W; long ldw;
    float* C; RowMap cmap; long c_nblk = 8;
    const float* bias;
    const uint8_t* keep; long keep_ld;
    int M, N, K;
    int act;
    int splitk = 1; int kchunk = 0; long c_split = 0;
    bool kmajor = false; RowMap wmap{1, 0, 0};
    int m_begin = 0;
    const int32_t* row_len = nullptr;
    int c_halo = 0;
};
hipError_t launch_gemm(const GemmParams& p, hipStream_t s);
struct GemmPlan { hipError_t err; int tile; int rows_big; };
GemmPlan plan_gemm(const GemmParams& p);
void set_splitk(GemmParams& p, int splitk);
hipError_t launch_gemm_splitk(const GemmParams& p, int splitk, float* scratch, hipStream_t s);

struct XSeg { const float* p; int len; };

struct SkinnyJob {
    const float* Wp;
    const float* bias;
    XSeg x[3];
    int N;
    int nkg;
    int kg0, nkg_w;
    int mode;
    float* c;
    float* h_out;
    const float* addend; long add_bs, add_ts;
    const float* addend2;
    const int32_t* lengths; int step; int reverse; int seq_len;
    float* seq_out; long seq_bs, seq_ts;
    const float* h_prev;
    const uint8_t* h_keep; float h_scale;
    float* c_out; float* c_seq_out;
    float* pre_out;
    const float* Wq_t;
    float* q_slab; int att_dim;
    const float* xw; const float* xsrc;
    int defer_seg;
    const unsigned* ctx_cnt; unsigned ctx_target;
    unsigned* start_cnt;
    const unsigned* ready_cnt; unsigned ready_target;
    unsigned* tmo;
    unsigned spin_limit;
    float* y;
    const uint8_t* keep; long keep_stride;
    int act;
    int B;
};
struct LocJob {
    const float* w_prev; long w_prev_bs;
    const float* w_cum;
    const float* loc_conv_t;
    const float* loc_dense_t;
    const float* pm;
    float* loc_out;
    int B, L, a, kl, G;
};
enum SkinnyKind : int { SK_DECODER = 0, SK_ENCODER = 1, SK_AR = 2, SK_TRAIN = 3 };
hipError_t launch_skinny(const SkinnyJob* jobs, int njobs, int kind, hipStream_t s, const LocJob* loc = nullptr);
struct AttnParams;
hipError_t launch_skinny_attn(const SkinnyJob* jobs, int njobs, const AttnParams& ap, hipStream_t s);
struct EncPersistParams {
    const float* Wp[2];
    const float* xg;
    const int32_t* lengths;
    float* hx;
    float* seq_out;
    float* c_seq_out;
    unsigned* sync;
    unsigned spin_limit;
    int B, L, H;
    int debug_skip_block;
};
bool encoder_persistent_supported(int B, int H);
hipError_t launch_encoder_persistent(const EncPersistParams& p, hipStream_t s);
hipError_t launch_skinny_pa(const SkinnyJob& att, const SkinnyJob* dec, hipStream_t s, int depth = 4, int layout = 1);
hipError_t launch_skinny_pa64(const SkinnyJob* jobs, int njobs, hipStream_t s);

struct AttnParams {
    const float* q_slab; int n_slabs;
    float* w_cum;
    const float* loc;
    const float* v;
    const float* pm;
    const float* memory;
    const int32_t* lengths;
    float* energies;
    float* w_out; long w_out_bs;
    float* ctx_out;
    int B, L, a, F, kl, E, G;
// ... 67 lines not shown
    const uint8_t* tr_keep_a; const uint8_t* tr_keep_d; float tr_scale_a, tr_scale_d;
    float* tr_c_a; float* tr_c_d; float* tr_pre_a; float* tr_pre_d;
};
struct ArResidentParams {
    const float* att_frag; const float* att_bias; const float* wq_t;
    const float* dec_frag; const float* dec_bias;
    const float* proj_hd_t;
    const float* proj_ctx_t;
    const float* pre_w1;
    const uint8_t* keep1;
    float* prenet;
    const float* y1;
    float* h_a; float* hc; float* q_slab;
    float* p_slab;
    float* c_a; float* c_d;
    const int32_t* n_done;
    unsigned* sync;
    unsigned att_frag_bytes;
    int B, T, PSB;
    unsigned spin_limit;
    int debug;
};
bool decoder_resident_supported(int B, int L);
hipError_t launch_decoder_ar_resident(const ArResidentParams& p, hipStream_t s);
hipError_t decoder_resident_init();
hipError_t launch_decoder_resident(const DecResidentParams& p, hipStream_t s);

bool attention_persistent_supported(int B, int L, int a, int F, int kl, int E, int att_rnn_dim, int dec_rnn_dim);
int attention_persistent_layout(int B, int L);
int attention_persistent_slabs(int layout);
int attention_persistent_workgroups(int B, int L);
size_t attention_persistent_xchg_floats(int B);
hipError_t attention_persistent_init();
hipError_t launch_attention_persistent(const AttnPersistParams& p, hipStream_t s);
hipError_t launch_handoff_set(unsigned* word, hipStream_t s);

#if defined(__HIPCC__)
typedef __attribute__((ext_vector_type(4))) unsigned gvx_u32x4;
__device__ __forceinline__ __amdgpu_buffer_rsrc_t make_rsrc(const void* p) {
    return __builtin_amdgcn_make_buffer_rsrc(const_cast<void*>(p), 0, 0x7fffffff, 0x00020000);
}
__device__ __forceinline__ float4 load_sc1(__amdgpu_buffer_rsrc_t r, unsigned byte_off) {
    const gvx_u32x4 v = __builtin_amdgcn_raw_buffer_load_b128(r, (int)byte_off, 0, 16);
    return make_float4(__uint_as_float(v.x), __uint_as_float(v.y), __uint_as_float(v.z), __uint_as_float(v.w));
}
__device__ __forceinline__ float load_sc1_f32(__amdgpu_buffer_rsrc_t r, unsigned byte_off) {
    return __uint_as_float(__builtin_amdgcn_raw_buffer_load_b32(r, (int)byte_off, 0, 16));
}
__device__ __forceinline__ void store_sc1(__amdgpu_buffer_rsrc_t r, unsigned byte_off, float4 v) {
    gvx_u32x4 u;
    u.x = __float_as_uint(v.x); u.y = __float_as_uint(v.y); u.z = __float_as_uint(v.z); u.w = __float_as_uint(v.w);
    __builtin_amdgcn_raw_buffer_store_b128(u, r, (int)byte_off, 0, 16);
}
template <bool FEW_WAITERS = false>
__device__ __forceinline__ bool handoff_wait(const unsigned* cnt, unsigned target, unsigned* tmo, unsigned code, unsigned limit = 0u,
                                             const unsigned* stop = nullptr) {
    if (limit == 0u) limit = HANDOFF_SPIN_LIMIT;
    unsigned spins = 0;
    while (__hip_atomic_load(cnt, __ATOMIC_RELAXED, __HIP_MEMORY_SCOPE_AGENT) < target) {
        ++spins;
        if ((spins & (FEW_WAITERS ? 127u : 7u)) == 1u) {
            if (__hip_atomic_load(tmo, __ATOMIC_RELAXED, __HIP_MEMORY_SCOPE_AGENT) != 0u) return false;
            if (stop && __hip_atomic_load(stop, __ATOMIC_RELAXED, __HIP_MEMORY_SCOPE_AGENT) != 0u) return false;
            if (spins > (FEW_WAITERS ? 16u : 1u) * limit) {
                __hip_atomic_store(tmo, code, __ATOMIC_RELAXED, __HIP_MEMORY_SCOPE_AGENT);
                return false;
            }
        }
        if (FEW_WAITERS || spins < 8u) __builtin_amdgcn_s_sleep(FEW_WAITERS ? 2 : 8);
        else __builtin_amdgcn_s_sleep(64);
    }
    return true;
}
#endif

hipError_t launch_embed(const int64_t* tokens, const float* emb, int n_tokens, float* x, float* x2, int B, int L, int E, int halo,
                        int* err_flag, hipStream_t s);
hipError_t launch_frames_from_mel(const float* mel_in, float* frames, int B, int M, int T, hipStream_t s);
hipError_t launch_split_projection(const float* proj, float* mel_out, float* gate_out, int B, int M, int T, hipStream_t s);
hipError_t launch_to_channels_last(const float* src, float* dst, int B, int M, int T, int halo, const int32_t* lens, hipStream_t s);
hipError_t launch_residual_to_channels_first(const float* mel, const float* y, float* mel_post, int B, int M, int T,
                                             const int32_t* lens, hipStream_t s);
hipError_t launch_zero_halo(float* buf, int B, int T, int halo, int C, hipStream_t s);
hipError_t launch_mask_padding(float* mel, float* mel_post, float* gate, const int32_t* mel_lengths, int B, int M, int T,
                               hipStream_t s);
hipError_t launch_zero_many(void* const* ptrs, const size_t* bytes, int n_arrays, hipStream_t s);
hipError_t launch_poison_on_timeout(const unsigned* tmo, int* sticky, float* const* ptrs, const size_t* counts, int n_arrays, hipStream_t s);
hipError_t launch_permute01(const float* src, float* dst, int T, int B, int n, hipStream_t s);
size_t loss_scratch_bytes();
hipError_t launch_tacotron2_loss(const float* mel, const float* mel_post, const float* gate, const float* mel_t, const float* gate_t,
                                 long n_mel, long n_gate, double* scratch, float* out3, hipStream_t s);
hipError_t launch_mask_gen(uint8_t* out, size_t n, uint64_t seed, hipStream_t s);
hipError_t launch_ar_stop(const float* proj_t, int gate_col, float threshold, int t, int B,
                          int32_t* n_frames, int32_t* n_done, hipStream_t s);
hipError_t launch_ar_project(const float* p_slab, int n_slabs, const float* p_ctx, float* proj_t, int M, float threshold, int t, int B,
                             int32_t* n_frames, int32_t* n_done, const float* w0t, const float* w1t, int P, const uint8_t* keep0,
                             const uint8_t* keep1, float* prenet_out, hipStream_t s);
hipError_t launch_ar_centres_finish(int32_t* centres, const int32_t* n_frames, const unsigned* tmo, int B, int T, hipStream_t s);
hipError_t launch_ar_emit_all(const float* proj, float* mel_out, float* gate_out, int B, int M, int Tmax, int steps,
                              const int32_t* n_frames, hipStream_t s);
hipError_t launch_permute01_partial(const float* src, float* dst, int steps, int Tdst, int B, int n, const int32_t* n_frames,
                                    hipStream_t s);

}
```

genvox_amd/csrc/gvx_pack.hip:

```cpp
#include "gvx_internal.h"

using namespace gvx;

namespace gvx {

Blob make_blob_layout(const gvx_dims& d) {
    Blob b{};
    size_t off = 0;
    auto take = [&](size_t n) { size_t o = off; off = align_up(off + n, 64); return o; };
    const int E = d.embed_dim, H = E / 2, M = d.n_mels, P = d.prenet_dim, A = d.att_rnn_dim, D = d.dec_rnn_dim;
    b.emb = take((size_t)d.n_tokens * E);
    for (int i = 0; i < d.enc_n_conv; ++i) { b.enc_w[i] = take((size_t)E * d.enc_kernel * E); b.enc_b[i] = take(E); }
    b.enc_wih = take((size_t)8 * H * E);
    b.enc_bih = take((size_t)8 * H);
    for (int dir = 0; dir < 2; ++dir) b.enc_whh_frag[dir] = take(frag_floats(4 * H, H));
    b.pre_w0 = take((size_t)P * M); b.pre_w1 = take((size_t)P * P);
    b.pre_w0_t = take((size_t)M * P);
    b.pre_w1_t = take((size_t)P * P);
    b.att_frag = take(frag_floats(4 * A, P + E + A)); b.att_bias = take((size_t)4 * A);
    b.att_wpre = take((size_t)4 * A * P);
    b.wq_t = take((size_t)A * d.att_dim);
    b.wmem = take((size_t)d.att_dim * E); b.v = take(d.att_dim);
    b.loc_conv = take((size_t)2 * d.att_loc_kernel * 32);
    b.loc_dense = take((size_t)32 * d.att_dim);
    b.dec_frag = take(frag_floats(4 * D, A + E + D)); b.dec_bias = take((size_t)4 * D);
    b.proj_w = take((size_t)(M + 1) * (D + E)); b.proj_b = take(M + 1);
    b.proj_frag = take(frag_floats(M + 1, D + E));
    b.proj_hd_t = take((size_t)D * ((M + 1 + 7) & ~7));
    b.proj_ctx_frag = take(frag_floats(M + 1, E));
    b.proj_ctx_t = take((size_t)(E / 4) * ((M + 1 + 7) & ~7) * 4);
    for (int i = 0; i < d.postnet_n_conv; ++i) {
        const int cin = i == 0 ? M : d.postnet_dim, cout = i == d.postnet_n_conv - 1 ? M : d.postnet_dim;
        b.post_w[i] = take((size_t)cout * d.postnet_kernel * cin);
        b.post_b[i] = take(cout);
    }
    b.total = off;
    return b;
}

}

namespace {

void pack_frag(const std::vector<float>& W, int N, int K, float* out) {
    const int ntiles = (N + 31) / 32, nkg = K / 8;
    for (int t = 0; t < ntiles; ++t)
        for (int kg = 0; kg < nkg; ++kg)
            for (int lane = 0; lane < 64; ++lane) {
                const int n = t * 32 + (lane & 31), k = 8 * kg + 4 * (lane >> 5);
                float* o = out + (((size_t)t * nkg + kg) * 64 + lane) * 4;
                for (int s = 0; s < 4; ++s) o[s] = n < N ? W[(size_t)n * K + k + s] : 0.f;
            }
}

struct WeightTable {
    std::unordered_map<std::string, const gvx_weight_desc*> map;
    const float* get(const std::string& name, int64_t numel, int* rc) const {
        auto it = map.find(name);
        if (it == map.end()) { *rc = fail(GVX_ERR_MISSING_WEIGHT, "missing weight '%s'", name.c_str()); return nullptr; }
        if (it->second->numel != numel) {
            *rc = fail(GVX_ERR_SHAPE, "weight '%s' has %lld elements, expected %lld", name.c_str(), (long long)it->second->numel, (long long)numel);
            return nullptr;
        }
        return it->second->data;
    }
};

int pack_conv(const WeightTable& wt, const std::string& prefix, int cout, int cin, int k, float* w_out, float* b_out) {
    int rc = GVX_OK;
    const float* w = wt.get(prefix + ".0.conv.weight", (int64_t)cout * cin * k, &rc); if (!w) return rc;
    const float* b = wt.get(prefix + ".0.conv.bias", cout, &rc); if (!b) return rc;
    const float* g = wt.get(prefix + ".1.weight", cout, &rc); if (!g) return rc;
    const float* beta = wt.get(prefix + ".1.bias", cout, &rc); if (!beta) return rc;
    const float* mu = wt.get(prefix + ".1.running_mean", cout, &rc); if (!mu) return rc;
    const float* var = wt.get(prefix + ".1.running_var", cout, &rc); if (!var) return rc;
    for (int co = 0; co < cout; ++co) {
        const double scale = (double)g[co] / std::sqrt((double)var[co] + BN_EPS);
        for (int kk = 0; kk < k; ++kk)
            for (int ci = 0; ci < cin; ++ci)
                w_out[((size_t)co * k + kk) * cin + ci] = (float)((double)w[((size_t)co * cin + ci) * k + kk] * scale);
        b_out[co] = (float)(((double)b[co] - (double)mu[co]) * scale + (double)beta[co]);
    }
    return GVX_OK;
}

int pack_lstm(const WeightTable& wt, const std::string& wih_name, const std::string& whh_name, const std::string& bih_name,
              const std::string& bhh_name, int Hd, int Kin, std::vector<float>* wcat, float* bias_out) {
    int rc = GVX_OK;
    const float* wih = wt.get(wih_name, (int64_t)4 * Hd * Kin, &rc); if (!wih) return rc;
    const float* whh = wt.get(whh_name, (int64_t)4 * Hd * Hd, &rc); if (!whh) return rc;
    const float* bih = wt.get(bih_name, 4 * Hd, &rc); if (!bih) return rc;
    const float* bhh = wt.get(bhh_name, 4 * Hd, &rc); if (!bhh) return rc;
    const int K = Kin + Hd;
    wcat->assign((size_t)4 * Hd * K, 0.f);
    for (int j = 0; j < Hd; ++j)
        for (int q = 0; q < 4; ++q) {
            const int src = q * Hd + j, dst = 4 * j + q;
            std::memcpy(&(*wcat)[(size_t)dst * K], wih + (size_t)src * Kin, sizeof(float) * Kin);
            std::memcpy(&(*wcat)[(size_t)dst * K + Kin], whh + (size_t)src * Hd, sizeof(float) * Hd);
            bias_out[dst] = bih[src] + bhh[src];
        }
    return GVX_OK;
}

}

extern "C" {

int gvx_model_pack_weights(gvx_model* m, const gvx_weight_desc* table, int n, void* host_blob) {
    if (!m || !table || !host_blob) return fail(GVX_ERR_INVALID_ARG, "null argument");
    WeightTable wt;
    for (int i = 0; i < n; ++i) wt.map[table[i].name] = &table[i];
    const gvx_dims& d = m->d;
    const Blob& bl = m->blob;
    float* out = reinterpret_cast<float*>(host_blob);
    std::memset(out, 0, bl.total * sizeof(float));
    const int E = d.embed_dim, H = E / 2, M = d.n_mels, P = d.prenet_dim, A = d.att_rnn_dim, D = d.dec_rnn_dim, a = d.att_dim;
    int rc = GVX_OK;
    const float* src;

    if (!(src = wt.get("embedding.weight", (int64_t)d.n_tokens * E, &rc))) return rc;
    std::memcpy(out + bl.emb, src, sizeof(float) * d.n_tokens * E);

    for (int i = 0; i < d.enc_n_conv; ++i) {
        rc = pack_conv(wt, "encoder.convolutions." + std::to_string(i), E, E, d.enc_kernel, out + bl.enc_w[i], out + bl.enc_b[i]);
        if (rc != GVX_OK) return rc;
    }
    {
        const char* sfx[2] = {"", "_reverse"};
        for (int dir = 0; dir < 2; ++dir) {
            std::vector<float> wcat;
            std::vector<float> bias(4 * H);
            rc = pack_lstm(wt, std::string("encoder.lstm.weight_ih_l0") + sfx[dir], std::string("encoder.lstm.weight_hh_l0") + sfx[dir],
                           std::string("encoder.lstm.bias_ih_l0") + sfx[dir], std::string("encoder.lstm.bias_hh_l0") + sfx[dir], H, E, &wcat, bias.data());
            if (rc != GVX_OK) return rc;
            std::vector<float> whh((size_t)4 * H * H);
            for (int r = 0; r < 4 * H; ++r) {
                std::memcpy(out + bl.enc_wih + ((size_t)dir * 4 * H + r) * E, &wcat[(size_t)r * (E + H)], sizeof(float) * E);
                std::memcpy(&whh[(size_t)r * H], &wcat[(size_t)r * (E + H) + E], sizeof(float) * H);
            }
            std::memcpy(out + bl.enc_bih + (size_t)dir * 4 * H, bias.data(), sizeof(float) * 4 * H);
            pack_frag(whh, 4 * H, H, out + bl.enc_whh_frag[dir]);
        }
    }
    {
        if (!(src = wt.get("decoder.prenet.layers.0.linear_layer.weight", (int64_t)P * M, &rc))) return rc;
        std::memcpy(out + bl.pre_w0, src, sizeof(float) * P * M);
        for (int j = 0; j < P; ++j)
            for (int k = 0; k < M; ++k) out[bl.pre_w0_t + (size_t)k * P + j] = src[(size_t)j * M + k];
        if (!(src = wt.get("decoder.prenet.layers.1.linear_layer.weight", (int64_t)P * P, &rc))) return rc;
        std::memcpy(out + bl.pre_w1, src, sizeof(float) * P * P);
        for (int j = 0; j < P; ++j)
            for (int k = 0; k < P; ++k) out[bl.pre_w1_t + (size_t)k * P + j] = src[(size_t)j * P + k];
    }
    {
        std::vector<float> wcat;
        rc = pack_lstm(wt, "decoder.attention_rnn.weight_ih", "decoder.attention_rnn.weight_hh", "decoder.attention_rnn.bias_ih",
                       "decoder.attention_rnn.bias_hh", A, P + E, &wcat, out + bl.att_bias);
        if (rc != GVX_OK) return rc;
        pack_frag(wcat, 4 * A, P + E + A, out + bl.att_frag);
        for (int n = 0; n < 4 * A; ++n) std::memcpy(out + bl.att_wpre + (size_t)n * P, &wcat[(size_t)n * (P + E + A)], sizeof(float) * P);
    }
    {
        const std::string att = "decoder.attention_layer.";
        if (!(src = wt.get(att + "query_layer.linear_layer.weight", (int64_t)a * A, &rc))) return rc;
        for (int t = 0; t < A / 8; ++t)
            for (int dd = 0; dd < a; ++dd)
                for (int jj = 0; jj < 8; ++jj) out[bl.wq_t + ((size_t)t * a + dd) * 8 + jj] = src[(size_t)dd * A + t * 8 + jj];
        if (!(src = wt.get(att + "memory_layer.linear_layer.weight", (int64_t)a * E, &rc))) return rc;
        std::memcpy(out + bl.wmem, src, sizeof(float) * a * E);
        if (!(src = wt.get(att + "v.linear_layer.weight", a, &rc))) return rc;
        std::memcpy(out + bl.v, src, sizeof(float) * a);
        const int64_t nconv = (int64_t)d.att_loc_filters * 2 * d.att_loc_kernel;
        if (!(src = wt.get(att + "location_layer.location_conv.conv.weight", nconv, &rc))) return rc;
        for (int c = 0; c < d.att_loc_filters; ++c)
            for (int ck = 0; ck < 2 * d.att_loc_kernel; ++ck) out[bl.loc_conv + (size_t)ck * 32 + c] = src[(size_t)c * 2 * d.att_loc_kernel + ck];
        if (!(src = wt.get(att + "location_layer.location_dense.linear_layer.weight", (int64_t)a * d.att_loc_filters, &rc))) return rc;
        for (int dd = 0; dd < a; ++dd)
            for (int c = 0; c < d.att_loc_filters; ++c) out[bl.loc_dense + ((size_t)(c >> 2) * a + dd) * 4 + (c & 3)] = src[(size_t)dd * d.att_loc_filters + c];
    }
    {
        std::vector<float> wcat;
        rc = pack_lstm(wt, "decoder.decoder_rnn.weight_ih", "decoder.decoder_rnn.weight_hh", "decoder.decoder_rnn.bias_ih",
                       "decoder.decoder_rnn.bias_hh", D, A + E, &wcat, out + bl.dec_bias);
        if (rc != GVX_OK) return rc;
        pack_frag(wcat, 4 * D, A + E + D, out + bl.dec_frag);
    }
    {
        const int K = D + E;
        std::vector<float> w((size_t)(M + 1) * K);
        if (!(src = wt.get("decoder.linear_projection.linear_layer.weight", (int64_t)M * K, &rc))) return rc;
        std::memcpy(w.data(), src, sizeof(float) * M * K);
        if (!(src = wt.get("decoder.gate_layer.linear_layer.weight", K, &rc))) return rc;
        std::memcpy(w.data() + (size_t)M * K, src, sizeof(float) * K);
        std::memcpy(out + bl.proj_w, w.data(), sizeof(float) * w.size());
        pack_frag(w, M + 1, K, out + bl.proj_frag);
        const int PSBp = (M + 1 + 7) & ~7;
        for (int t = 0; t < D / 8; ++t)
            for (int n = 0; n < PSBp; ++n)
                for (int jj = 0; jj < 8; ++jj)
                    out[bl.proj_hd_t + ((size_t)t * PSBp + n) * 8 + jj] = n <= M ? w[(size_t)n * K + t * 8 + jj] : 0.f;
        std::vector<float> wc((size_t)(M + 1) * E);
        for (int n = 0; n <= M; ++n) std::memcpy(&wc[(size_t)n * E], &w[(size_t)n * K + D], sizeof(float) * E);
        pack_frag(wc, M + 1, E, out + bl.proj_ctx_frag);
        for (int t = 0; t < E / 4; ++t)
            for (int n = 0; n < PSBp; ++n)
                for (int jj = 0; jj < 4; ++jj)
                    out[bl.proj_ctx_t + ((size_t)t * PSBp + n) * 4 + jj] = n <= M ? w[(size_t)n * K + D + t * 4 + jj] : 0.f;
        if (!(src = wt.get("decoder.linear_projection.linear_layer.bias", M, &rc))) return rc;
        std::memcpy(out + bl.proj_b, src, sizeof(float) * M);
        if (!(src = wt.get("decoder.gate_layer.linear_layer.bias", 1, &rc))) return rc;
        out[bl.proj_b + M] = src[0];
    }
    for (int i = 0; i < d.postnet_n_conv; ++i) {
        const int cin = i == 0 ? M : d.postnet_dim, cout = i == d.postnet_n_conv - 1 ? M : d.postnet_dim;
        rc = pack_conv(wt, "postnet.convolutions." + std::to_string(i), cout, cin, d.postnet_kernel, out + bl.post_w[i], out + bl.post_b[i]);
        if (rc != GVX_OK) return rc;
    }
    return GVX_OK;
}

}

namespace {

constexpr int PACK_MAX_TENSORS = 192;
struct PackSources { const float* p[PACK_MAX_TENSORS]; };

__global__ void pack_gather_kernel(PackSources src, const int32_t* off, const uint8_t* tid, long n, float* blob) {
    for (long i = (long)blockIdx.x * blockDim.x + threadIdx.x; i < n; i += (long)gridDim.x * blockDim.x) {
        const int t = tid[i];
        if (t == 255) continue;
        blob[i] = t ? src.p[t - 1][off[i]] : 0.f;
    }
}
__global__ void pack_conv_fold_kernel(const float* w, const float* b, const float* g, const float* beta, const float* mu, const float* var,
                                      int cout, int cin, int k, float* w_out, float* b_out) {
    const long n = (long)cout * cin * k;
    for (long i = (long)blockIdx.x * blockDim.x + threadIdx.x; i < n; i += (long)gridDim.x * blockDim.x) {
        const int ci = (int)(i % cin), kk = (int)((i / cin) % k), co = (int)(i / ((long)cin * k));
        const double scale = (double)g[co] / sqrt((double)var[co] + BN_EPS);
        w_out[i] = (float)((double)w[((long)co * cin + ci) * k + kk] * scale);
        if (ci == 0 && kk == 0) b_out[co] = (float)(((double)b[co] - (double)mu[co]) * scale + (double)beta[co]);
    }
}
__global__ void pack_lstm_bias_kernel(const float* bih, const float* bhh, int Hd, float* out) {
    const int i = blockIdx.x * blockDim.x + threadIdx.x;
    if (i < 4 * Hd) { const int j = i >> 2, q = i & 3; out[i] = bih[q * Hd + j] + bhh[q * Hd + j]; }
}

struct DevTable {
    std::unordered_map<std::string, int> idx;
    const gvx_weight_desc* t;
    const float* get(const std::string& name, int64_t numel, int* rc) const {
        auto it = idx.find(name);
        if (it == idx.end()) { *rc = fail(GVX_ERR_MISSING_WEIGHT, "missing weight '%s'", name.c_str()); return nullptr; }
        if (t[it->second].numel != numel) { *rc = fail(GVX_ERR_SHAPE, "weight '%s' has %lld elements, expected %lld", name.c_str(), (long long)t[it->second].numel, (long long)numel); return nullptr; }
        return t[it->second].data;
    }
};

int ensure_gather_map(gvx_model* m, const gvx_weight_desc* table, int n) {
    bool same = m->gather_off && (int)m->gather_names.size() == n;
    for (int i = 0; same && i < n; ++i) same = m->gather_names[i] == table[i].name && m->gather_numel[i] == table[i].numel;
    if (same) return GVX_OK;
    if (n > PACK_MAX_TENSORS || n > 254) return fail(GVX_ERR_UNSUPPORTED, "pack_weights_device: more than %d tensors", 254);
    const size_t total = m->blob.total;
    std::vector<std::vector<float>> lo(n), hi(n);
    std::vector<gvx_weight_desc> tl(n), th(n);
    for (int i = 0; i < n; ++i) {
        if (table[i].numel < 0 || table[i].numel >= (int64_t)1 << 31) return fail(GVX_ERR_UNSUPPORTED, "pack_weights_device: tensor too large");
        lo[i].resize((size_t)table[i].numel); hi[i].resize((size_t)table[i].numel);
        for (int64_t e = 0; e < table[i].numel; ++e) { lo[i][e] = (float)((e & 4095) + 1); hi[i][e] = (float)((e >> 12) * 256 + i + 1); }
        tl[i] = gvx_weight_desc{table[i].name, lo[i].data(), table[i].numel};
        th[i] = gvx_weight_desc{table[i].name, hi[i].data(), table[i].numel};
    }
    std::vector<float> bl(total), bh(total);
    int rc = gvx_model_pack_weights(m, tl.data(), n, bl.data());
    if (rc != GVX_OK) return rc;
    rc = gvx_model_pack_weights(m, th.data(), n, bh.data());
    if (rc != GVX_OK) return rc;
    std::vector<int32_t> off(total);
    std::vector<uint8_t> tid(total);
    for (size_t i = 0; i < total; ++i) {
        if (bl[i] == 0.f && bh[i] == 0.f) { off[i] = 0; tid[i] = 0; continue; }
        const long h = (long)bh[i] - 1, l = (long)bl[i] - 1;
        const int t = (int)(h % 256);
        off[i] = (int32_t)((h / 256) * 4096 + l);
        tid[i] = (uint8_t)(t + 1);
    }
    const gvx_dims& d = m->d;
    const Blob& b = m->blob;
    auto mark = [&](size_t o, size_t cnt) { std::fill(tid.begin() + o, tid.begin() + o + cnt, (uint8_t)255); };
    const int E = d.embed_dim, H = E / 2, M = d.n_mels;
    for (int i = 0; i < d.enc_n_conv; ++i) { mark(b.enc_w[i], (size_t)E * d.enc_kernel * E); mark(b.enc_b[i], E); }
    for (int i = 0; i < d.postnet_n_conv; ++i) {
        const int cin = i == 0 ? M : d.postnet_dim, cout = i == d.postnet_n_conv - 1 ? M : d.postnet_dim;
        mark(b.post_w[i], (size_t)cout * d.postnet_kernel * cin); mark(b.post_b[i], cout);
    }
    mark(b.enc_bih, (size_t)8 * H); mark(b.att_bias, (size_t)4 * d.att_rnn_dim); mark(b.dec_bias, (size_t)4 * d.dec_rnn_dim);
    for (size_t i = 0; i < total; ++i)
        if (tid[i] && tid[i] != 255 && (tid[i] > n || off[i] < 0 || off[i] >= table[tid[i] - 1].numel))
            return fail(GVX_ERR_UNSUPPORTED, "pack_weights_device: gather map is inconsistent at blob float %zu", i);
    if (m->gather_off) { (void)hipFree(m->gather_off); m->gather_off = nullptr; }
    if (m->gather_tid) { (void)hipFree(m->gather_tid); m->gather_tid = nullptr; }
    HIP_TRY(hipMalloc(reinterpret_cast<void**>(&m->gather_off), total * sizeof(int32_t)));
    HIP_TRY(hipMalloc(reinterpret_cast<void**>(&m->gather_tid), total));
    HIP_TRY(hipMemcpy(m->gather_off, off.data(), total * sizeof(int32_t), hipMemcpyHostToDevice));
    HIP_TRY(hipMemcpy(m->gather_tid, tid.data(), total, hipMemcpyHostToDevice));
    m->gather_names.clear(); m->gather_numel.clear();
    for (int i = 0; i < n; ++i) { m->gather_names.push_back(table[i].name); m->gather_numel.push_back(table[i].numel); }
    return GVX_OK;
}

}

extern "C" {

int gvx_model_pack_weights_device(gvx_model* m, const gvx_weight_desc* table, int n, void* device_blob, void* stream) {
    if (!m || !table || !device_blob || n < 1) return fail(GVX_ERR_INVALID_ARG, "null argument");
    if (reinterpret_cast<uintptr_t>(device_blob) & 255) return fail(GVX_ERR_INVALID_ARG, "blob must be 256-byte aligned");
    int rc = ensure_gather_map(m, table, n);
    if (rc != GVX_OK) return rc;
    hipStream_t s = (hipStream_t)stream;
    float* out = reinterpret_cast<float*>(device_blob);
    PackSources src{};
    for (int i = 0; i < n; ++i) src.p[i] = table[i].data;
    const long total = (long)m->blob.total;
    hipLaunchKernelGGL(pack_gather_kernel, dim3(4096), dim3(256), 0, s, src, m->gather_off, m->gather_tid, total, out);
    DevTable dt; dt.t = table;
    for (int i = 0; i < n; ++i) dt.idx[table[i].name] = i;
    const gvx_dims& d = m->d;
    const Blob& bl = m->blob;
    const int E = d.embed_dim, H = E / 2, M = d.n_mels;
    auto conv = [&](const std::string& prefix, int cout, int cin, int k, size_t w_off, size_t b_off) -> int {
        int r = GVX_OK;
        const float* w = dt.get(prefix + ".0.conv.weight", (int64_t)cout * cin * k, &r); if (!w) return r;
        const float* b = dt.get(prefix + ".0.conv.bias", cout, &r); if (!b) return r;
        const float* g = dt.get(prefix + ".1.weight", cout, &r); if (!g) return r;
        const float* beta = dt.get(prefix + ".1.bias", cout, &r); if (!beta) return r;
        const float* mu = dt.get(prefix + ".1.running_mean", cout, &r); if (!mu) return r;
        const float* var = dt.get(prefix + ".1.running_var", cout, &r); if (!var) return r;
        const long cnt = (long)cout * cin * k;
        hipLaunchKernelGGL(pack_conv_fold_kernel, dim3((unsigned)((cnt + 255) / 256)), dim3(256), 0, s, w, b, g, beta, mu, var, cout, cin, k, out + w_off, out + b_off);
        return GVX_OK;
    };
    for (int i = 0; i < d.enc_n_conv; ++i)
        if ((rc = conv("encoder.convolutions." + std::to_string(i), E, E, d.enc_kernel, bl.enc_w[i], bl.enc_b[i])) != GVX_OK) return rc;
    for (int i = 0; i < d.postnet_n_conv; ++i) {
        const int cin = i == 0 ? M : d.postnet_dim, cout = i == d.postnet_n_conv - 1 ? M : d.postnet_dim;
        if ((rc = conv("postnet.convolutions." + std::to_string(i), cout, cin, d.postnet_kernel, bl.post_w[i], bl.post_b[i])) != GVX_OK) return rc;
    }
    auto bias = [&](const std::string& bih_n, const std::string& bhh_n, int Hd, size_t o) -> int {
        int r = GVX_OK;
        const float* bih = dt.get(bih_n, 4 * Hd, &r); if (!bih) return r;
        const float* bhh = dt.get(bhh_n, 4 * Hd, &r); if (!bhh) return r;
        hipLaunchKernelGGL(pack_lstm_bias_kernel, dim3((4 * Hd + 255) / 256), dim3(256), 0, s, bih, bhh, Hd, out + o);
        return GVX_OK;
    };
    if ((rc = bias("encoder.lstm.bias_ih_l0", "encoder.lstm.bias_hh_l0", H, bl.enc_bih)) != GVX_OK) return rc;
    if ((rc = bias("encoder.lstm.bias_ih_l0_reverse", "encoder.lstm.bias_hh_l0_reverse", H, bl.enc_bih + (size_t)4 * H)) != GVX_OK) return rc;
    if ((rc = bias("decoder.attention_rnn.bias_ih", "decoder.attention_rnn.bias_hh", d.att_rnn_dim, bl.att_bias)) != GVX_OK) return rc;
    if ((rc = bias("decoder.decoder_rnn.bias_ih", "decoder.decoder_rnn.bias_hh", d.dec_rnn_dim, bl.dec_bias)) != GVX_OK) return rc;
    HIP_TRY(hipGetLastError());
    return GVX_OK;
}

}
```

genvox_amd/csrc/train_ops.hip:

```cpp
#include "train_internal.h"

#include <cmath>
#include <cstdio>

namespace gvx {
namespace {

__global__ __launch_bounds__(1024) void col_reduce_kernel(const float* X, const float* Y, long rows, int C, float* sum_x, float* sum_xy) {
    __shared__ double sx[CR_LANES][33], sxy[CR_LANES][33];
    const int cl = threadIdx.x & 31, rl = threadIdx.x >> 5, c = blockIdx.x * 32 + cl;
    double a0 = 0.0, a1 = 0.0, a2 = 0.0, a3 = 0.0, b0 = 0.0, b1 = 0.0, b2 = 0.0, b3 = 0.0;
    if (c < C) {
        long r = rl;
        for (; r + 3 * CR_LANES < rows; r += 4 * CR_LANES) {
            const float x0 = X[r * C + c], x1 = X[(r + CR_LANES) * C + c], x2 = X[(r + 2 * CR_LANES) * C + c], x3 = X[(r + 3 * CR_LANES) * C + c];
            a0 += x0; a1 += x1; a2 += x2; a3 += x3;
            if (Y) {
                b0 += (double)x0 * (double)Y[r * C + c]; b1 += (double)x1 * (double)Y[(r + CR_LANES) * C + c];
                b2 += (double)x2 * (double)Y[(r + 2 * CR_LANES) * C + c]; b3 += (double)x3 * (double)Y[(r + 3 * CR_LANES) * C + c];
            }
        }
        for (; r < rows; r += CR_LANES) {
            const double x = X[r * C + c];
            a0 += x;
// ... 86 lines not shown
        if (e0 < E) demb[(long)row * E + e0] = a0;
        if (e1 < E) demb[(long)row * E + e1] = a1;
        if (e2 < E) demb[(long)row * E + e2] = a2;
        if (e3 < E) demb[(long)row * E + e3] = a3;
    }
}
constexpr int SQN_BLOCKS = 64;
__global__ __launch_bounds__(256) void sqnorm_many_kernel(const gvx_tensor_ref* refs, double* partials) {
    __shared__ double red[256];
    const gvx_tensor_ref r = refs[blockIdx.y];
    double s0 = 0.0, s1 = 0.0;
    long i = (long)blockIdx.x * 256 + threadIdx.x;
    const long stride = (long)SQN_BLOCKS * 256;
    for (; i + stride < r.numel; i += 2 * stride) {
        const double a = r.data[i], b = r.data[i + stride];
        s0 += a * a; s1 += b * b;
    }
    if (i < r.numel) { const double a = r.data[i]; s0 += a * a; }
    red[threadIdx.x] = s0 + s1;
    __syncthreads();
    for (int o = 128; o > 0; o >>= 1) { if ((int)threadIdx.x < o) red[threadIdx.x] += red[threadIdx.x + o]; __syncthreads(); }
    if (threadIdx.x == 0) partials[(long)blockIdx.y * SQN_BLOCKS + blockIdx.x] = red[0];
}
__global__ __launch_bounds__(256) void sqnorm_finish_kernel(const double* partials, int n, double* out) {
    __shared__ double red[256];
    double s = 0.0;
    for (int i = threadIdx.x; i < n; i += 256) s += partials[i];
    red[threadIdx.x] = s;
    __syncthreads();
    for (int o = 128; o > 0; o >>= 1) { if ((int)threadIdx.x < o) red[threadIdx.x] += red[threadIdx.x + o]; __syncthreads(); }
    if (threadIdx.x == 0) out[0] = red[0];
}
__global__ void adam_many_kernel(const gvx_adam_ref* refs, float gscale, float lr, float wd, float b1, float b2, float eps, float bc1,
                                 float bc2_sqrt) {
    const gvx_adam_ref r = refs[blockIdx.y];
    for (long i = (long)blockIdx.x * blockDim.x + threadIdx.x; i < r.numel; i += (long)gridDim.x * blockDim.x) {
        const float gi = r.grad[i] * gscale + wd * r.param[i];
        const float mi = b1 * r.exp_avg[i] + (1.f - b1) * gi;
        const float vi = b2 * r.exp_avg_sq[i] + (1.f - b2) * gi * gi;
        r.exp_avg[i] = mi; r.exp_avg_sq[i] = vi;
        r.param[i] -= (lr / bc1) * mi / (sqrtf(vi) / bc2_sqrt + eps);
    }
}

inline int train_gemm_splitk(int M, int N, int K, bool have_scratch, size_t scratch_bytes) {
    const long tiles = (long)((M + 63) / 64) * ((N + 127) / 128);
    int splitk = have_scratch ? choose_splitk(tiles, K) : 1;
    while (splitk > 1 && (size_t)splitk * M * N * sizeof(float) > scratch_bytes) --splitk;
    return splitk;
}

}

int tfail_hip(const char* expr, hipError_t e) {
    thread_local char msg[256];
    snprintf(msg, sizeof msg, "%s failed: %s", expr, hipGetErrorString(e));
    return set_error(GVX_ERR_HIP, msg);
}

void launch_col_reduce(const float* X, const float* Y, long rows, int C, float* sum_x, float* sum_xy, hipStream_t s) {
    hipLaunchKernelGGL(col_reduce_kernel, dim3((C + 31) / 32), dim3(1024), 0, s, X, Y, rows, C, sum_x, sum_xy);
}

}

using namespace gvx;

extern "C" {

int gvx_debug_gemm_plan(int M, int N, int K, int kmajor, int have_scratch, size_t scratch_bytes, int* tile_out, int* rows_big_out, int* k_pieces_out) {
    if (!tile_out || !rows_big_out || !k_pieces_out || M < 1 || N < 1 || K < 1) return GVX_ERR_INVALID_ARG;
    GemmParams g{};
    g.kmajor = kmajor != 0;
    g.amap = kmajor ? RowMap{K, 0, (long)M} : RowMap{M, 0, (long)K};
    g.wmap = RowMap{K, 0, (long)N};
    g.M = M; g.N = N; g.K = K;
    const int splitk = train_gemm_splitk(M, N, K, have_scratch != 0, scratch_bytes);
    if (splitk > 1) set_splitk(g, splitk);
    const GemmPlan pl = plan_gemm(g);
    *tile_out = pl.tile; *rows_big_out = pl.rows_big; *k_pieces_out = g.splitk;
    return pl.err == hipSuccess ? GVX_OK : GVX_ERR_INVALID_ARG;
}

int gvx_train_gemm_nt(const float* A, long lda, const float* W, long ldw, float* C, long ldc, int M, int N, int K, const float* bias,
                      float* scratch, size_t scratch_bytes, void* stream) {
    if (!A || !W || !C || M < 1 || N < 1 || K < 4 || (K & 3)) return tfail(GVX_ERR_INVALID_ARG, "gemm_nt: null argument or K not a positive multiple of 4");
    GemmParams g{};
    g.A = A; g.amap = RowMap{M, 0, lda};
    g.W = W; g.ldw = ldw;
    g.C = C; g.cmap = RowMap{M, 0, ldc};
    g.bias = bias; g.M = M; g.N = N; g.K = K; g.act = ACT_NONE;
    TR_TRY(launch_gemm_splitk(g, train_gemm_splitk(M, N, K, scratch != nullptr, scratch_bytes), scratch, (hipStream_t)stream));
    return GVX_OK;
}
int gvx_train_gemm_tn(const float* A, long lda, const float* Bm, long ldb, float* C, long ldc, int M, int N, long rows, float* scratch,
                      size_t scratch_bytes, void* stream) {
    if (!A || !Bm || !C || M < 1 || N < 1 || rows < 1 || rows > (1L << 30)) return tfail(GVX_ERR_INVALID_ARG, "gemm_tn: bad argument");
    GemmParams g{};
    g.kmajor = true;
    g.A = A; g.amap = RowMap{(int)rows, 0, lda};
    g.W = Bm; g.wmap = RowMap{(int)rows, 0, ldb};
    g.C = C; g.cmap = RowMap{M, 0, ldc};
    g.M = M; g.N = N; g.K = (int)rows; g.act = ACT_NONE;
    TR_TRY(launch_gemm_splitk(g, train_gemm_splitk(M, N, (int)rows, scratch != nullptr, scratch_bytes), scratch, (hipStream_t)stream));
    return GVX_OK;
}
int gvx_train_transpose(const float* src, long ld_src, float* dst, long rows, int cols, long rows_p, void* stream) {
    if (!src || !dst || rows < 1 || cols < 1 || rows_p < rows) return tfail(GVX_ERR_INVALID_ARG, "transpose: bad argument");
    if (ld_src != cols) return tfail(GVX_ERR_UNSUPPORTED, "transpose: source must be dense (ld == cols)");
    hipLaunchKernelGGL(transpose_pad_kernel, dim3((unsigned)((rows_p + 31) / 32), (cols + 31) / 32), dim3(256), 0, (hipStream_t)stream, src, dst, rows, cols, rows_p);
    TR_TRY(hipGetLastError());
    return GVX_OK;
}
int gvx_train_colsum(const float* X, long rows, int C, float* out, void* stream) {
    if (!X || !out || rows < 1 || C < 1) return tfail(GVX_ERR_INVALID_ARG, "colsum: bad argument");
    launch_col_reduce(X, nullptr, rows, C, out, nullptr, (hipStream_t)stream);
    TR_TRY(hipGetLastError());
    return GVX_OK;
}
int gvx_train_axpby(const float* a, long lda, float alpha, const float* b, long ldb, float beta, float* y, long ldy, long rows, int cols, void* stream) {
    if (!a || !y || rows < 1 || cols < 1) return tfail(GVX_ERR_INVALID_ARG, "axpby: bad argument");
    hipLaunchKernelGGL(axpby_kernel, dim3(blocks_for(rows * cols)), dim3(256), 0, (hipStream_t)stream, a, lda, alpha, b, ldb, beta, y, ldy, rows, cols);
    TR_TRY(hipGetLastError());
    return GVX_OK;
}
int gvx_train_relu_dropout_backward(const float* dy, const float* act_out, const uint8_t* keep, float scale, long n, float* dz, void* stream) {
    if (!dy || !act_out || !keep || !dz || n < 1) return tfail(GVX_ERR_INVALID_ARG, "relu_dropout_backward: bad argument");
    hipLaunchKernelGGL(relu_drop_bwd_kernel, dim3(blocks_for(n)), dim3(256), 0, (hipStream_t)stream, dy, act_out, keep, scale, n, dz);
    TR_TRY(hipGetLastError());
    return GVX_OK;
}
int gvx_train_unblock(const float* blocked, float* rows_out, long n_slots, int B, int K, void* stream) {
    if (!blocked || !rows_out || n_slots < 1 || B < 1 || K < 8 || (K & 7)) return tfail(GVX_ERR_INVALID_ARG, "unblock: bad argument");
    hipLaunchKernelGGL(unblock_kernel, dim3(blocks_for(n_slots * B * K)), dim3(256), 0, (hipStream_t)stream, blocked, rows_out, n_slots, B, K);
    TR_TRY(hipGetLastError());
    return GVX_OK;
}
int gvx_train_embedding_backward(const int64_t* tokens, const float* dx, long n_tokens_in_batch, int E, int n_rows, float* demb, void* stream) {
    if (!tokens || !dx || !demb || n_tokens_in_batch < 1 || E < 1 || n_rows < 1) return tfail(GVX_ERR_INVALID_ARG, "embedding_backward: bad argument");
    hipLaunchKernelGGL(embedding_bwd_kernel, dim3(n_rows), dim3(256), 0, (hipStream_t)stream, tokens, dx, n_tokens_in_batch, E, n_rows, demb);
    TR_TRY(hipGetLastError());
    return GVX_OK;
}
int gvx_train_sqnorm_many(const gvx_tensor_ref* refs_device, int n_tensors, double* scratch, double* sumsq_out, void* stream) {
    if (!refs_device || !scratch || !sumsq_out || n_tensors < 1) return tfail(GVX_ERR_INVALID_ARG, "sqnorm_many: bad argument");
    hipLaunchKernelGGL(sqnorm_many_kernel, dim3(SQN_BLOCKS, n_tensors), dim3(256), 0, (hipStream_t)stream, refs_device, scratch);
    hipLaunchKernelGGL(sqnorm_finish_kernel, dim3(1), dim3(256), 0, (hipStream_t)stream, scratch, SQN_BLOCKS * n_tensors, sumsq_out);
    TR_TRY(hipGetLastError());
    return GVX_OK;
}
size_t gvx_train_sqnorm_scratch_bytes(int n_tensors) { return n_tensors < 1 ? 0 : (size_t)SQN_BLOCKS * n_tensors * sizeof(double); }
int gvx_train_adam_step_many(const gvx_adam_ref* refs_device, int n_tensors, float grad_scale, float lr, float weight_decay, float beta1,
                             float beta2, float eps, int step, void* stream) {
    if (!refs_device || n_tensors < 1 || step < 1) return tfail(GVX_ERR_INVALID_ARG, "adam_step_many: bad argument");
    const float bc1 = (float)(1.0 - std::pow((double)beta1, (double)step)), bc2s = (float)std::sqrt(1.0 - std::pow((double)beta2, (double)step));
    hipLaunchKernelGGL(adam_many_kernel, dim3(128, n_tensors), dim3(256), 0, (hipStream_t)stream, refs_device, grad_scale, lr, weight_decay, beta1, beta2,
                       eps, bc1, bc2s);
    TR_TRY(hipGetLastError());
    return GVX_OK;
}

}
```

genvox_amd/tacotron2.py:

```python
from __future__ import annotations

import ctypes as C
import os
import math
import warnings
from typing import Dict, Optional

import numpy as np
import torch
from torch import nn

from . import _lib
from .configs import AudioConfig, BaseConfig, Tacotron2Config, TextConfig
from .weights import state_dict_spec

MAX_CALL_BATCH = 64
STREAM_ROWS = 32

_GAIN = {"linear": "linear", "sigmoid": "sigmoid", "tanh": "tanh", "relu": "relu"}


class _Node(nn.Module):

    def child(self, name: str) -> "_Node":
        if name not in self._modules:
            self.add_module(name, _Node())
        return self._modules[name]


def dims_from_configs(mc: Tacotron2Config, ac: AudioConfig, tc: TextConfig) -> _lib.gvx_dims:
    assert tc.n_tokens is not None and tc.n_tokens >= 1, "text_config.n_tokens must be set (size of the token map)"
    return _lib.gvx_dims(
        n_tokens=tc.n_tokens, embed_dim=mc.encoder_embedding_dim, enc_kernel=mc.encoder_kernel_size,
        enc_n_conv=mc.encoder_n_convolutions, prenet_dim=mc.prenet_dim, att_rnn_dim=mc.attention_rnn_dim,
        dec_rnn_dim=mc.decoder_rnn_dim, att_dim=mc.attention_dim, att_loc_filters=mc.attention_location_n_filters,
        att_loc_kernel=mc.attention_location_kernel_size, postnet_dim=mc.postnet_embedding_dim,
        postnet_kernel=mc.postnet_kernel_size, postnet_n_conv=mc.postnet_n_convolutions, n_mels=ac.n_mels)


class Tacotron2(nn.Module):
    def __init__(self, model_config: Tacotron2Config, audio_config: AudioConfig, text_config: TextConfig) -> None:
        super().__init__()
        self.model_name = self.__class__.__name__
        self.model_config = model_config
        self.audio_config = audio_config
        self.text_config = text_config
        self._spec = state_dict_spec(model_config, audio_config, text_config)
        for key, (shape, kind, arg) in self._spec.items():
            *path, leaf = key.split(".")
            node = self
            for name in path:
                node = node.child(name)
            if kind == "count":
                node.register_buffer(leaf, torch.zeros((), dtype=torch.long))
            elif kind in ("bn_mean", "bn_var"):
                node.register_buffer(leaf, torch.ones(shape) if kind == "bn_var" else torch.zeros(shape))
            else:
                t = torch.empty(shape)
                if kind == "xavier":
                    nn.init.xavier_uniform_(t, gain=nn.init.calculate_gain(_GAIN[arg]))
                elif kind == "uniform":
                    t.uniform_(-arg, arg)
                elif kind == "bn_w":
                    t.fill_(1.0)
                elif kind == "bn_b":
                    t.zero_()
                node.register_parameter(leaf, nn.Parameter(t, requires_grad=False))
        self._handle: Optional[int] = None
        self._key_tensors = None
        self._blob: Optional[torch.Tensor] = None
        self._host_repack = os.environ.get("GVX_HOST_REPACK") == "1"
        self._packed_key = None
        self._workspace: Optional[torch.Tensor] = None
        self._lane_ws = [None, None]
        self._lane_streams = None
        self._lane_handles = [None, None]
        self._timing = False
        self._sticky_bad = False
        self._sticky_stalled = False
        self._resident_off = False
        self._enc_bptt_resident = True
        self._enc_bptt_workspaces = []
        self.eval()

    def child(self, name: str) -> _Node:
        return _Node.child(self, name)

    def __del__(self):
        try:
            for h in [self._handle] + list(getattr(self, "_lane_handles", [])):
                if h is not None:
                    _lib.load().gvx_model_destroy(h)
        except Exception:
            pass

    def _device(self) -> torch.device:
        return self.embedding.weight.device

    def _require_gpu(self) -> torch.device:
        dev = self._device()
        if dev.type != "cuda":
            raise RuntimeError("genvox_amd.Tacotron2 runs on an MI355X only: move the model with .to('cuda:0'). "
                               "There is no CPU fallback (the reference's CPU path is the oracle under oracle/).")
        if self._lane_streams is None:
            self._lane_streams = [torch.cuda.Stream(device=dev), torch.cuda.Stream(device=dev)]
            for lane in self._lane_streams:
                with torch.cuda.stream(lane):
                    torch.zeros(1, device=dev)
        return dev

    def _weights_key(self):
        ts = self._key_tensors
        if ts is None:
            ts = self._key_tensors = [v for v in self.state_dict(keep_vars=True).values()]
        return (str(self._device()),) + tuple((v.data_ptr(), v._version) for v in ts)

    def _apply(self, fn, *args, **kwargs):
        out = super()._apply(fn, *args, **kwargs)
        self._key_tensors = None
        return out

    def _ensure_handle(self) -> int:
        if self._handle is None:
            h = C.c_void_p()
            dims = dims_from_configs(self.model_config, self.audio_config, self.text_config)
            _lib.check(_lib.load().gvx_model_create(C.byref(dims), C.byref(h)))
            self._handle = h.value
        return self._handle

    def blob_numel(self) -> int:
        return _lib.load().gvx_model_blob_bytes(self._ensure_handle()) // 4

    def pack_weights_host(self) -> torch.Tensor:
        lib = _lib.load()
        h = self._ensure_handle()
        host = {k: v.detach().to("cpu", torch.float32).contiguous() for k, v in self.state_dict().items()
                if v.is_floating_point()}
        table = (_lib.gvx_weight_desc * len(host))()
        for i, (k, v) in enumerate(host.items()):
            table[i] = _lib.gvx_weight_desc(k.encode(), v.data_ptr(), v.numel())
        blob_host = torch.empty(self.blob_numel(), dtype=torch.float32)
        _lib.check(lib.gvx_model_pack_weights(h, table, len(host), blob_host.data_ptr()))
        return blob_host

    def pack_weights_device(self, out: Optional[torch.Tensor] = None) -> torch.Tensor:
        dev = self._require_gpu()
        lib = _lib.load()
        h = self._ensure_handle()
        srcs = {k: v.detach() for k, v in self.state_dict().items() if v.is_floating_point()}
        for k, v in srcs.items():
            if v.device != dev or v.dtype != torch.float32 or not v.is_contiguous():
                srcs[k] = v.to(device=dev, dtype=torch.float32).contiguous()
        table = (_lib.gvx_weight_desc * len(srcs))()
        for i, (k, v) in enumerate(srcs.items()):
            table[i] = _lib.gvx_weight_desc(k.encode(), v.data_ptr(), v.numel())
        blob = torch.empty(self.blob_numel(), dtype=torch.float32, device=dev) if out is None else out
        _lib.check(lib.gvx_model_pack_weights_device(h, table, len(srcs), blob.data_ptr(), self._stream()))
        return blob
# ... 20 lines not shown
            _lib.check(lib.gvx_stage_timing_enable(self._handle, 1))

    def packed_blob(self) -> torch.Tensor:
        if self._device().type != "cuda":
            return self.pack_weights_host()
        self._ensure_packed()
        return self._blob

    def bind_packed_blob(self, blob: torch.Tensor) -> None:
        assert blob.dtype == torch.float32 and blob.is_contiguous() and blob.device == self._device()
        assert blob.numel() == self.blob_numel(), "blob size does not match this model's dims"
        if blob.device.type == "cuda":
            self._bind(blob)
        else:
            self._blob = blob
        self._packed_key = self._weights_key()

    def _get_workspace(self, B: int, L: int, T: int) -> torch.Tensor:
        return self._workspace_of(_lib.load().gvx_workspace_bytes(self._handle, B, L, T))

    def _workspace_of(self, need: int) -> torch.Tensor:
        dev = self._device()
        if self._workspace is None or self._workspace.numel() < need or self._workspace.device != dev:
            if self._workspace is not None:
                self._poll_status()
            self._workspace = self._new_workspace(need, dev)
        return self._workspace

    def _stream(self) -> int:
        return torch.cuda.current_stream(self._device()).cuda_stream

    @staticmethod
    def _new_workspace(nbytes: int, dev) -> torch.Tensor:
        ws = torch.empty(nbytes, dtype=torch.uint8, device=dev)
        ws[:65536].zero_()
        return ws

    def _poll_status(self) -> None:
        out = (C.c_int32 * 2)()
        for ws in [self._workspace] + self._lane_ws:
            if ws is None:
                continue
            _lib.check(_lib.load().gvx_workspace_status(self._handle, ws.data_ptr(), ws.numel(), self._stream(), out))
            self._sticky_bad |= bool(out[0])
            self._sticky_stalled |= bool(out[1])

    def check_status(self) -> None:
        self._poll_status()
        bad, stalled = self._sticky_bad, self._sticky_stalled
        self._sticky_bad = self._sticky_stalled = False
        if stalled:
            raise RuntimeError("genvox_amd: an in-launch hand-off of the decoder loop timed out; the last outputs are invalid")
        if bad:
            raise IndexError("genvox_amd: token id outside [0, n_tokens)")

    def _stalled_once(self) -> bool:
        self._poll_status()
        if not self._sticky_stalled:
            return False
        self._sticky_stalled = False
        if self._resident_off:
            raise RuntimeError("genvox_amd: a hand-off timed out although the resident kernels are switched off")
        import warnings

        warnings.warn("genvox_amd: an in-launch hand-off of a resident kernel timed out (the kernels could not run at the same "
                      "time on this GPU); switching this model to the launch-per-step kernels and running the call again")
        lib = _lib.load()
        for h in [self._handle] + self._lane_handles:
            if h is not None:
                _lib.check(lib.gvx_model_set_resident_kernels(h, 0))
        self._resident_off = True
        return True

    def _ensure_lane_handles(self) -> None:
        lib = _lib.load()
        for i in range(2):
            if self._lane_handles[i] is None:
                h = C.c_void_p()
                dims = dims_from_configs(self.model_config, self.audio_config, self.text_config)
                _lib.check(lib.gvx_model_create(C.byref(dims), C.byref(h)))
                _lib.check(lib.gvx_model_set_persistent_attention(h.value, 0))
                if self._resident_off:
                    _lib.check(lib.gvx_model_set_resident_kernels(h.value, 0))
                _lib.check(lib.gvx_model_bind_blob(h.value, self._blob.data_ptr()))
                if self._timing:
                    _lib.check(lib.gvx_stage_timing_enable(h.value, 1))
                self._lane_handles[i] = h.value

    def _lanes(self, dev, need_bytes: int):
        if self._lane_streams is None:
            self._lane_streams = [torch.cuda.Stream(device=dev), torch.cuda.Stream(device=dev)]
        for i in range(2):
            if self._lane_ws[i] is None or self._lane_ws[i].numel() < need_bytes or self._lane_ws[i].device != dev:
                if self._lane_ws[i] is not None:
                    self._poll_status()
                self._lane_ws[i] = self._new_workspace(need_bytes, dev)
        return self._lane_streams, self._lane_ws

    def enable_stage_timing(self, enable: bool = True) -> None:
        self._timing = enable
        for h in [self._handle] + self._lane_handles:
            if h is not None:
                _lib.check(_lib.load().gvx_stage_timing_enable(h, int(enable)))

    def stage_times_ms(self, lane: Optional[int] = None):
        t = (C.c_float * 5)()
        n = C.c_int()
        _lib.check(_lib.load().gvx_stage_times_ms(self._handle if lane is None else self._lane_handles[lane], t, C.byref(n)))
        names = ("encoder", "prenet", "decoder_loop", "projection", "postnet")
        return dict(zip(names, list(t))), n.value

    def enable_kernel_timing(self, enable: bool = True) -> None:
        self._ensure_packed()
        _lib.check(_lib.load().gvx_kernel_timing_enable(self._handle, int(enable)))

    def loop_kind(self, B: int, L: int) -> int:
        self._ensure_packed()
        return int(_lib.load().gvx_teacher_forced_loop_kind(self._handle, B, L))

    def ar_loop_kind(self, B: int, L: int) -> int:
        self._ensure_packed()
        return int(_lib.load().gvx_autoregressive_loop_kind(self._handle, B, L))

    def ar_windowed_loop_kind(self, B: int, L: int) -> int:
        self._ensure_packed()
        return int(_lib.load().gvx_autoregressive_windowed_loop_kind(self._handle, B, L))

    @staticmethod
    def _check_window(window):
        if window is None:
            return None
        try:
            back, ahead = (int(v) for v in window)
        except (TypeError, ValueError):
            raise ValueError(f"attention_window must be a pair (back, ahead) of non-negative integers, got {window!r}") from None
        if back < 0 or ahead < 0 or (back, ahead) != tuple(window):
            raise ValueError(f"attention_window must be a pair (back, ahead) of non-negative integers, got {window!r}")
        return back, ahead

    def kernel_times_ms(self):
        a, b, n = C.c_float(), C.c_float(), C.c_int()
        _lib.check(_lib.load().gvx_kernel_times_ms(self._handle, C.byref(a), C.byref(b), C.byref(n)))
        return {"decoder_lstm_step": a.value, "attention_step": b.value, "steps": n.value}

    def _keep_masks(self, given: Optional[torch.Tensor], n: int, dev) -> torch.Tensor:
        if given is not None:
            m = given.to(device=dev, dtype=torch.uint8).contiguous()
            assert m.numel() == n, f"prenet_keep_masks has {m.numel()} elements, expected {n}"
            return m
        seed = int(torch.randint(0, 2 ** 62, (1,)).item())
        m = torch.empty(n, dtype=torch.uint8, device=dev)
        _lib.check(_lib.load().gvx_prenet_masks_generate(m.data_ptr(), n, seed, self._stream()))
        return m

    def forward(self, batch: Dict[str, torch.Tensor], strict: bool = True) -> Dict[str, torch.Tensor]:
        out = self._forward_once(batch)
        if strict and not self.training and self._stalled_once():
            out = self._forward_once(batch)
            self._stalled_once()
        return out

    def _forward_once(self, batch: Dict[str, torch.Tensor]) -> Dict[str, torch.Tensor]:
        dev = self._require_gpu()
        if self.training:
            return self._forward_train(batch)[0]
        self._ensure_packed()
        tokens = batch["token_padded"].to(device=dev, dtype=torch.int64).contiguous()
        tok_len = batch["token_lengths"].to(device=dev, dtype=torch.int32).contiguous()
        mel_in = batch["mel_padded"].to(device=dev, dtype=torch.float32).contiguous()
        mel_len = batch["mel_lengths"].to(device=dev, dtype=torch.int32).contiguous()
        B, L = tokens.shape
        _, M, T = mel_in.shape
        assert M == self.audio_config.n_mels
        P = self.model_config.prenet_dim
        given = batch.get("prenet_keep_masks")
        if given is not None:
            given = given.to(device=dev, dtype=torch.uint8).reshape(2, T + 1, B, P)
        out = {"mel_outputs": torch.empty(B, M, T, device=dev), "mel_outputs_postnet": torch.empty(B, M, T, device=dev),
               "gate_outputs": torch.empty(B, T, device=dev), "alignments": torch.empty(B, T, L, device=dev)}
        lib = _lib.load()

        def run(lo: int, hi: int, ws: torch.Tensor, handle: int, postnet: bool = True) -> None:
            n = hi - lo
            masks = self._keep_masks(given[:, :, lo:hi].contiguous() if given is not None else None, 2 * (T + 1) * n * P, dev)
            _lib.check(lib.gvx_tacotron2_forward(
                handle, tokens[lo:hi].data_ptr(), tok_len[lo:hi].data_ptr(), n, L, mel_in[lo:hi].data_ptr(),
                mel_len[lo:hi].data_ptr() if self.model_config.mask_padding else None, T, masks.data_ptr(),
                out["mel_outputs"][lo:hi].data_ptr(), out["mel_outputs_postnet"][lo:hi].data_ptr() if postnet else None,
                out["gate_outputs"][lo:hi].data_ptr(), out["alignments"][lo:hi].data_ptr(),
                ws.data_ptr(), ws.numel(), self._stream()))

        rows = STREAM_ROWS
        if B > STREAM_ROWS and lib.gvx_teacher_forced_rows_per_call(self._handle, L) == MAX_CALL_BATCH:
            rows = MAX_CALL_BATCH
        self.last_forward_lanes = B > rows and rows == STREAM_ROWS
        self.last_forward_sequential32 = False
        if B <= rows:
# ... 441 lines not shown
```

include/genvox_amd.h:

```cpp
#ifndef GENVOX_AMD_H
#define GENVOX_AMD_H

#include <stddef.h>
#include <stdint.h>

#ifdef __cplusplus
extern "C" {
#endif

typedef enum gvx_status {
    GVX_OK = 0,
    GVX_ERR_INVALID_ARG = -1,
    GVX_ERR_UNSUPPORTED = -2,
    GVX_ERR_MISSING_WEIGHT = -3,
    GVX_ERR_SHAPE = -4,
    GVX_ERR_WORKSPACE = -5,
    GVX_ERR_HIP = -6,
    GVX_ERR_STATE = -7
} gvx_status;

typedef struct gvx_dims {
    int32_t n_tokens;
    int32_t embed_dim;
    int32_t enc_kernel;
    int32_t enc_n_conv;
    int32_t prenet_dim;
    int32_t att_rnn_dim;
    int32_t dec_rnn_dim;
    int32_t att_dim;
    int32_t att_loc_filters;
    int32_t att_loc_kernel;
    int32_t postnet_dim;
    int32_t postnet_kernel;
    int32_t postnet_n_conv;
    int32_t n_mels;
} gvx_dims;

typedef struct gvx_weight_desc {
    const char* name;
    const float* data;
    int64_t numel;
} gvx_weight_desc;

typedef struct gvx_model gvx_model;

#define GVX_WORKSPACE_CLEAR_BYTES 12804

const char* gvx_last_error(void);
int gvx_version(void);

int gvx_model_create(const gvx_dims* dims, gvx_model** out);
void gvx_model_destroy(gvx_model* model);
size_t gvx_model_blob_bytes(const gvx_model* model);
int gvx_model_pack_weights(gvx_model* model, const gvx_weight_desc* table, int n, void* host_blob);
int gvx_model_bind_blob(gvx_model* model, const void* device_blob);
int gvx_model_pack_weights_device(gvx_model* model, const gvx_weight_desc* table, int n, void* device_blob, void* stream);

size_t gvx_workspace_bytes(const gvx_model* model, int B, int L, int T);
size_t gvx_workspace_bytes_autoregressive(const gvx_model* model, int B, int L, int max_steps);

int gvx_workspace_status(const gvx_model* model, void* workspace, size_t workspace_bytes, void* stream, int32_t* host_out);

int gvx_model_set_persistent_attention(gvx_model* model, int enable);

int gvx_model_set_resident_kernels(gvx_model* model, int enable);

int gvx_teacher_forced_rows_per_call(const gvx_model* model, int L);

int gvx_teacher_forced_resident(const gvx_model* model, int B, int L);

int gvx_teacher_forced_loop_kind(const gvx_model* model, int B, int L);

int gvx_autoregressive_loop_kind(const gvx_model* model, int B, int L);
int gvx_autoregressive_windowed_loop_kind(const gvx_model* model, int B, int L);

int gvx_encoder_forward(gvx_model* model, const int64_t* tokens, const int32_t* lengths, int B, int L,
                        float* memory_out, void* workspace, size_t workspace_bytes, void* stream);

int gvx_decoder_teacher_forced(gvx_model* model, const float* memory, const int32_t* lengths, int B, int L,
                               const float* mel_in, int T, const uint8_t* keep_masks,
                               float* mel_out, float* gate_out, float* align_out,
                               void* workspace, size_t workspace_bytes, void* stream);

int gvx_decoder_autoregressive(gvx_model* model, const float* memory, const int32_t* lengths, int B, int L,
                               int max_steps, float gate_threshold, const uint8_t* keep_masks,
                               float* mel_out, float* gate_out, float* align_out, int32_t* n_frames_out,
                               int* steps_run_out, void* workspace, size_t workspace_bytes, void* stream);

int gvx_decoder_autoregressive_windowed(gvx_model* model, const float* memory, const int32_t* lengths, int B, int L,
                                        int max_steps, float gate_threshold, const uint8_t* keep_masks,
                                        float* mel_out, float* gate_out, float* align_out, int32_t* n_frames_out,
                                        int* steps_run_out, void* workspace, size_t workspace_bytes, void* stream,
                                        int window_back, int window_ahead, int32_t* centres_out);

size_t gvx_postnet_workspace_bytes(const gvx_model* model, int B, int T);
int gvx_postnet_forward(gvx_model* model, const float* mel_in, const int32_t* mel_lengths, int B, int T, float* mel_post_out,
                        void* workspace, size_t workspace_bytes, void* stream);

int gvx_mask_padding(float* mel, float* mel_post, float* gate, const int32_t* mel_lengths,
                     int B, int n_mels, int T, void* stream);

int gvx_tacotron2_forward(gvx_model* model, const int64_t* tokens, const int32_t* token_lengths, int B, int L,
                          const float* mel_in, const int32_t* mel_lengths, int T, const uint8_t* keep_masks,
                          float* mel_out, float* mel_post_out, float* gate_out, float* align_out,
                          void* workspace, size_t workspace_bytes, void* stream);

int gvx_tacotron2_loss(const float* mel_out, const float* mel_post_out, const float* gate_out, const float* mel_target,
                       const float* gate_target, int B, int n_mels, int T, float* loss_out, void* scratch, size_t scratch_bytes,
                       void* stream);

int gvx_encoder_lstm_forward(gvx_model* model, const float* conv_out, const int32_t* lengths, int B, int L, float* memory_out,
                             float* cell_states_out, float* input_preact_out, void* workspace, size_t workspace_bytes, void* stream);
int gvx_decoder_teacher_forced_train(gvx_model* model, const float* memory, const int32_t* lengths, int B, int L, const float* mel_in,
                                     int T, const uint8_t* keep_masks, const uint8_t* att_keep, const uint8_t* dec_keep, float p_att,
                                     float p_dec, float* mel_out, float* gate_out, float* align_out, float* att_hidden_all,
                                     float* att_cell_all, float* dec_cell_all, float* dec_hidden_context_all, float* att_preact_all,
                                     float* dec_preact_all, void* workspace, size_t workspace_bytes, void* stream);
int gvx_train_export(const gvx_model* model, const void* workspace, size_t workspace_bytes, int B, int L, int T, int what, float* dst, void* stream);
size_t gvx_conv_train_saved_bytes(int B, int Cin, int Cout, int T, int k);
size_t gvx_conv_train_workspace_bytes(int B, int Cin, int Cout, int T, int k);
int gvx_conv_bn_act_train_forward(const float* x, const float* w, const float* bias, const float* gamma, const float* beta,
                                  float* running_mean, float* running_var, int B, int Cin, int Cout, int T, int k, int act,
                                  const uint8_t* keep, float p_drop, float* y, void* saved, size_t saved_bytes, void* workspace,
                                  size_t workspace_bytes, void* stream);
int gvx_conv_bn_act_train_backward(const float* dy, const void* saved, size_t saved_bytes, const float* w, const float* gamma,
                                   const float* x_wgrad, int B, int Cin, int Cout, int T, int k, int act, const uint8_t* keep,
                                   float p_drop, float* dx, float* dw, float* dbias, float* dgamma, float* dbeta, void* workspace,
                                   size_t workspace_bytes, void* stream);
int gvx_tacotron2_loss_backward(const float* mel_out, const float* mel_post_out, const float* gate_out, const float* mel_target,
                                const float* gate_target, int B, int n_mels, int T, float* dmel_out, float* dmel_post_out,
                                float* dgate_out, void* stream);

int gvx_train_gemm_nt(const float* A, long lda, const float* W, long ldw, float* C, long ldc, int M, int N, int K, const float* bias,
                      float* scratch, size_t scratch_bytes, void* stream);
int gvx_train_gemm_tn(const float* A, long lda, const float* Bm, long ldb, float* C, long ldc, int M, int N, long rows, float* scratch,
                      size_t scratch_bytes, void* stream);
int gvx_train_transpose(const float* src, long ld_src, float* dst, long rows, int cols, long rows_padded, void* stream);
int gvx_train_colsum(const float* X, long rows, int C, float* out, void* stream);
int gvx_train_axpby(const float* a, long lda, float alpha, const float* b, long ldb, float beta, float* y, long ldy, long rows, int cols, void* stream);
int gvx_train_relu_dropout_backward(const float* dy, const float* act_out, const uint8_t* keep, float scale, long n, float* dz, void* stream);
int gvx_train_unblock(const float* blocked, float* rows_out, long n_slots, int B, int K, void* stream);
int gvx_train_embedding_backward(const int64_t* tokens, const float* dx, long n_tokens_in_batch, int E, int n_rows, float* demb, void* stream);
typedef struct gvx_tensor_ref { const float* data; int64_t numel; } gvx_tensor_ref;
typedef struct gvx_adam_ref { float* param; const float* grad; float* exp_avg; float* exp_avg_sq; int64_t numel; } gvx_adam_ref;
size_t gvx_train_sqnorm_scratch_bytes(int n_tensors);
int gvx_train_sqnorm_many(const gvx_tensor_ref* refs_device, int n_tensors, double* scratch, double* sumsq_out, void* stream);
int gvx_train_adam_step_many(const gvx_adam_ref* refs_device, int n_tensors, float grad_scale, float lr, float weight_decay, float beta1,
                             float beta2, float eps, int step, void* stream);
// ... 347 lines not shown
```

Measured before the change: 1.863 million.

## Add Winograd F(4,5) path for middle postnet convolutions with batched sliced GEMM

Replaces the direct 5-tap convolution of the inner postnet layers with Winograd F(4,5). The input is transformed into 8 points, multiplied by pre-transformed weights through 8 batched GEMM slices, and transformed back with bias, tanh, masking and halo zeroing fused into the output step. The GEMM kernel gains a slice dimension on gridDim.y so all 8 point-wise products run in one launch. This cuts the multiply count per output by about 5/2, at the cost of extra transform passes, scratch memory traffic and the reduced fp32 accuracy that large Winograd constants bring.

```diff
diff --git a/genvox_amd/_lib.py b/genvox_amd/_lib.py
--- a/genvox_amd/_lib.py
+++ b/genvox_amd/_lib.py
@@ -243,6 +243,8 @@
     "gvx_kernel_timing_enable": (_i, [_vp, _i]),
     "gvx_model_set_persistent_attention": (_i, [_vp, _i]),
     "gvx_model_set_resident_kernels": (_i, [_vp, _i]),
+    "gvx_model_set_winograd": (_i, [_vp, _i]),
+    "gvx_debug_conv_plan": (_i, [_vp, _i, _i, _i]),
     "gvx_teacher_forced_rows_per_call": (_i, [_vp, _i]),
     "gvx_teacher_forced_resident": (_i, [_vp, _i, _i]),
     "gvx_teacher_forced_loop_kind": (_i, [_vp, _i, _i]),
diff --git a/genvox_amd/build.py b/genvox_amd/build.py
--- a/genvox_amd/build.py
+++ b/genvox_amd/build.py
@@ -9,7 +9,7 @@
 HERE = os.path.dirname(os.path.abspath(__file__))
 CSRC = os.path.join(HERE, "csrc")
 LIB = os.path.join(HERE, "libgenvox_amd.so")
-SOURCES = ["gemm_f32.hip", "skinny.hip", "dec_resident.hip", "attention.hip", "attn_persist.hip", "misc.hip", "griffinlim.hip", "wav_finalize.hip", "wav_to_mel.hip", "resample.hip", "eval_metrics.hip", "mas.hip", "time_warp.hip", "melgan.hip", "melgan_train.hip", "melgan_disc.hip", "hifigan.hip", "hifigan_train.hip", "hifigan_disc.hip", "pitch.hip", "psola.hip", "stft_loss.hip",
+SOURCES = ["gemm_f32.hip", "winograd_conv.hip", "skinny.hip", "dec_resident.hip", "attention.hip", "attn_persist.hip", "misc.hip", "griffinlim.hip", "wav_finalize.hip", "wav_to_mel.hip", "resample.hip", "eval_metrics.hip", "mas.hip", "time_warp.hip", "melgan.hip", "melgan_train.hip", "melgan_disc.hip", "hifigan.hip", "hifigan_train.hip", "hifigan_disc.hip", "pitch.hip", "psola.hip", "stft_loss.hip",
            "train_conv.hip", "train_ops.hip", "train_bptt_decoder.hip", "train_bptt_encoder.hip", "train_guided.hip", "gvx_pack.hip", "gvx_decoder.hip", "gvx_api.hip"]
 ARCH = "gfx950"
 HIPCC = os.environ.get("HIPCC", "/opt/rocm/bin/hipcc")
diff --git a/genvox_amd/csrc/gemm_f32.hip b/genvox_amd/csrc/gemm_f32.hip
--- a/genvox_amd/csrc/gemm_f32.hip
+++ b/genvox_amd/csrc/gemm_f32.hip
@@ -35,7 +35,10 @@
     const int m0 = p.m_begin + mt * BM, n0 = nt * BN;
     const int k_begin = p.splitk > 1 ? (int)blockIdx.y * p.kchunk : 0;
     const int k_end = p.splitk > 1 ? min(p.K, k_begin + p.kchunk) : p.K;
-    float* const Cout = p.C + (p.splitk > 1 ? (long)blockIdx.y * p.c_split : 0);
+    const long slice = p.splitk > 1 ? 0 : (long)blockIdx.y;
+    const float* const Ab = p.A + slice * p.a_slice;
+    const float* const Wb = p.W + slice * p.w_slice;
+    float* const Cout = p.C + (p.splitk > 1 ? (long)blockIdx.y * p.c_split : slice * p.c_slice);
 
     const int ld_row = tid / TPR, ld_c4 = tid % TPR;
     const float* a_ptr[A_V4]; bool a_ok[A_V4];
@@ -59,13 +62,13 @@
         for (int i = 0; i < A_V4; ++i) {
             int m = m0 + ld_row + RPP * i;
             a_ok[i] = m < p.M;
-            a_ptr[i] = p.A + (a_ok[i] ? row_off(p.amap, m) : 0);
+            a_ptr[i] = Ab + (a_ok[i] ? row_off(p.amap, m) : 0);
         }
 #pragma unroll
         for (int i = 0; i < B_V4; ++i) {
             int n = n0 + ld_row + RPP * i;
             b_ok[i] = n < p.N;
-            b_ptr[i] = p.W + (b_ok[i] ? (long)n * p.ldw : 0);
+            b_ptr[i] = Wb + (b_ok[i] ? (long)n * p.ldw : 0);
         }
     }
     float4 a_reg[A_V4], b_reg[B_V4];
@@ -89,8 +92,8 @@
 #define GEMM_LOAD_TILE(K0)                                                                                  \
     if (KMAJ) {                                                                                             \
         const int K0_ = (K0);                                                                               \
-        GEMM_KMAJ_LOAD(A_P, (256 / A_MQ), akq, ak_g, ak_i, p.amap, a_safe, p.A, a_col, ka_reg)              \
-        GEMM_KMAJ_LOAD(B_P, (256 / B_NQ), bkq, bk_g, bk_i, p.wmap, b_safe, p.W, b_col, kb_reg)              \
+        GEMM_KMAJ_LOAD(A_P, (256 / A_MQ), akq, ak_g, ak_i, p.amap, a_safe, Ab, a_col, ka_reg)              \
+        GEMM_KMAJ_LOAD(B_P, (256 / B_NQ), bkq, bk_g, bk_i, p.wmap, b_safe, Wb, b_col, kb_reg)              \
     } else                                                                                                  \
     {                                                                                                       \
         const int k_ = (K0) + 4 * ld_c4;                                                                    \
@@ -256,7 +259,7 @@
 static hipError_t launch_cfg(const GemmParams& p, hipStream_t s) {
     constexpr int BM = WR * TM * 32, BN = WC * TN * 32;
     const int grid = ((p.M - p.m_begin + BM - 1) / BM) * ((p.N + BN - 1) / BN);
-    gemm_f32_kernel<WR, WC, TM, TN, KMAJ, BK><<<dim3(grid, p.splitk > 1 ? p.splitk : 1), dim3(WR * WC * 64), lds_bytes_cfg<WR, WC, TM, TN, BK>(), s>>>(p);
+    gemm_f32_kernel<WR, WC, TM, TN, KMAJ, BK><<<dim3(grid, p.splitk > 1 ? p.splitk : p.slices > 1 ? p.slices : 1), dim3(WR * WC * 64), lds_bytes_cfg<WR, WC, TM, TN, BK>(), s>>>(p);
     return hipGetLastError();
 }
 
@@ -268,6 +271,7 @@
 GemmPlan plan_gemm(const GemmParams& p) {
     GemmPlan pl{hipSuccess, 0, 0};
     if (p.M <= 0 || p.N <= 0) return pl;
+    if (p.slices > 1 && (p.splitk > 1 || p.kmajor || p.keep || p.slices > 65535)) { pl.err = hipErrorInvalidValue; return pl; }
     if (p.kmajor) {
         if ((p.M & 3) || (p.N & 3) || p.M < 4 || p.N < 4 || ((p.amap.s0 | p.amap.s1 | p.wmap.s0 | p.wmap.s1) & 3)) { pl.err = hipErrorInvalidValue; return pl; }
         const long t128 = (long)((p.M + 127) / 128) * ((p.N + 127) / 128);
@@ -280,7 +284,7 @@
         pl.tile = p.M - p.m_begin <= 4096 ? 2311 : 4113;
         return pl;
     }
-    const long n_tiles = (p.N + 127) / 128, tiles128 = (long)((p.M + 127) / 128) * n_tiles;
+    const long n_tiles = (long)((p.N + 127) / 128) * (p.slices > 1 ? p.slices : 1), tiles128 = (long)((p.M + 127) / 128) * n_tiles;
     if (tiles128 < 192) { pl.tile = 2211; return pl; }
     if (tiles128 < 384) { pl.tile = 2212; return pl; }
     pl.tile = four_waves() ? 2222 : 4212;
diff --git a/genvox_amd/csrc/gvx_api.hip b/genvox_amd/csrc/gvx_api.hip
--- a/genvox_amd/csrc/gvx_api.hip
+++ b/genvox_amd/csrc/gvx_api.hip
@@ -39,6 +39,20 @@
 }
 
 std::mutex& capture_mutex() { return g_capture_mutex; }
+
+bool conv_uses_winograd(const gvx_model* m, int cin, int cout, int k) {
+    if (m->winograd <= 0 || !winograd_shape_ok(cin, cout, k)) return false;
+    return m->winograd >= 2 || cin >= WINOGRAD_MIN_CHANNELS;
+}
+
+size_t winograd_scratch_floats(const gvx_model* m, int B, int T) {
+    bool any = false;
+    for (int i = 0; i < m->d.postnet_n_conv; ++i) any = any || postnet_layer_winograd_shape(m->d, i);
+    if (!any) return 0;
+    const size_t tile = (size_t)2 * WINO_PTS * m->d.postnet_dim, all = (size_t)B * ((T + WINO_OUT - 1) / WINO_OUT) * tile;
+    const size_t budget = WINOGRAD_GROUP_BYTES / sizeof(float) / tile * tile;
+    return all <= budget ? all : budget > tile ? budget : tile;
+}
 
 WsPlan make_ws_plan(const gvx_model* m, int B, int L, int T, int mode) {
     const gvx_dims& d = m->d;
@@ -169,6 +183,8 @@
     m->debug_skip_resident = flag("GVX_DEBUG_SKIP_RESIDENT", false);
     m->debug_enc_skip_block = number("GVX_DEBUG_ENC_SKIP_BLOCK", -1);
     m->debug_plan = std::getenv("GVX_DEBUG_PLAN") != nullptr;
+    m->winograd = number("GVX_CONV_WINOGRAD", 1);
+    if (m->winograd < 0 || m->winograd > 2) m->winograd = 1;
 }
 
 }
@@ -346,7 +362,7 @@
 }
 
 int postnet_impl(gvx_model* m, const float* mel_in, const int32_t* mel_lengths, int B, int T, float* mel_post_out, float* ya,
-                 float* yb, hipStream_t s) {
+                 float* yb, float* wino, size_t wino_floats, hipStream_t s) {
     const gvx_dims& d = m->d;
     const int M = d.n_mels, pp = (d.postnet_kernel - 1) / 2, n = d.postnet_n_conv;
     HIP_TRY(launch_to_channels_last(mel_in, ya, B, M, T, pp, mel_lengths, s));
@@ -355,6 +371,32 @@
     for (int i = 0; i < n; ++i) {
         const int cin = i == 0 ? M : d.postnet_dim, cout = i == n - 1 ? M : d.postnet_dim;
         const bool last = i == n - 1;
+        if (postnet_layer_winograd_shape(d, i) && conv_uses_winograd(m, cin, cout, d.postnet_kernel)) {
+            const int C = cin;
+            const long total = (long)B * ((T + WINO_OUT - 1) / WINO_OUT);
+            const size_t tile = (size_t)2 * WINO_PTS * C, budget = WINOGRAD_GROUP_BYTES / sizeof(float);
+            long fit = (long)((wino_floats < budget ? wino_floats : budget) / tile);
+            if (fit < 1) return fail(GVX_ERR_WORKSPACE, "Postnet: %zu floats of scratch do not hold one Winograd tile (%zu)", wino_floats, tile);
+            if (m->wino_group > 0 && m->wino_group < fit) fit = m->wino_group;
+            if (fit > total) fit = total;
+            const long groups = (total + fit - 1) / fit, per_group = (total + groups - 1) / groups;
+            for (long mt0 = 0; mt0 < total; mt0 += per_group) {
+                const long Mt = total - mt0 < per_group ? total - mt0 : per_group;
+                float* V = wino;
+                float* Mm = wino + (size_t)WINO_PTS * Mt * C;
+                HIP_TRY(launch_winograd_input(cur, V, B, mt0, Mt, T, C, s));
+                GemmParams g{};
+                g.A = V; g.amap = RowMap{(int)Mt, 0, (long)C};
+                g.W = m->dev_blob + m->blob.post_u[i]; g.ldw = C;
+                g.C = Mm; g.cmap = RowMap{(int)Mt, 0, (long)C};
+                g.bias = nullptr; g.M = (int)Mt; g.N = C; g.K = C; g.act = ACT_NONE;
+                g.slices = WINO_PTS; g.a_slice = Mt * C; g.w_slice = (long)C * C; g.c_slice = Mt * C;
+                HIP_TRY(launch_gemm(g, s));
+                HIP_TRY(launch_winograd_output(Mm, m->dev_blob + m->blob.post_b[i], mel_lengths, nxt, B, mt0, Mt, T, C, s));
+            }
+            float* t = cur; cur = nxt; nxt = t;
+            continue;
+        }
         const int out_halo = last ? 0 : pp;
         const bool fused_halo = out_halo > 0 && T >= out_halo;
         if (out_halo > 0 && !fused_halo) HIP_TRY(launch_zero_halo(nxt, B, T, pp, cout, s));
@@ -373,7 +415,7 @@
     return GVX_OK;
 }
 
-struct PostnetPlan { size_t ya, yb, total; };
+struct PostnetPlan { size_t ya, yb, wino, wino_floats, total; };
 PostnetPlan make_postnet_plan(const gvx_model* m, int B, int T) {
     const gvx_dims& d = m->d;
     const int pp = (d.postnet_kernel - 1) / 2, cmax = d.postnet_dim > d.n_mels ? d.postnet_dim : d.n_mels;
@@ -381,7 +423,12 @@
     PostnetPlan p;
     p.ya = align_up((128 + HANDOFF_WORDS) * sizeof(float), 256);
     p.yb = p.ya + buf;
-    p.total = p.yb + buf;
+    p.wino = p.yb + buf;
+    const WsPlan w = make_ws_plan(m, B, 1, T, WS_AUTOREGRESSIVE);
+    const size_t tile = (size_t)2 * WINO_PTS * d.postnet_dim, room = (w.ya - w.xa) / sizeof(float) / tile * tile;
+    p.wino_floats = winograd_scratch_floats(m, B, T);
+    if (p.wino_floats > room) p.wino_floats = room > tile ? room : tile;
+    p.total = p.wino + align_up(p.wino_floats * sizeof(float), 256);
     return p;
 }
 
@@ -443,6 +490,35 @@
 int gvx_model_set_persistent_attention(gvx_model* m, int enable) {
     if (!m) return fail(GVX_ERR_INVALID_ARG, "null argument");
     m->attn_persistent = enable != 0;
+    return GVX_OK;
+}
+
+int gvx_model_set_winograd(gvx_model* m, int mode) {
+    if (!m) return fail(GVX_ERR_INVALID_ARG, "null argument");
+    if (mode < 0 || mode > 2) return fail(GVX_ERR_INVALID_ARG, "winograd mode must be 0, 1 or 2 (got %d)", mode);
+    m->winograd = mode;
+    return GVX_OK;
+}
+
+int gvx_debug_conv_plan(const gvx_model* m, int cin, int cout, int k) {
+    if (!m || cin < 1 || cout < 1 || k < 1) return -1;
+    return conv_uses_winograd(m, cin, cout, k) ? 1 : 0;
+}
+
+int gvx_debug_set_winograd_group(gvx_model* m, int tiles) {
+    if (!m || tiles < 0) return fail(GVX_ERR_INVALID_ARG, "bad argument");
+    m->wino_group = tiles;
+    return GVX_OK;
+}
+
+int gvx_debug_winograd_constants(double* at, double* g, double* bt) {
+    if (!at || !g || !bt) return fail(GVX_ERR_INVALID_ARG, "null argument");
+    for (int i = 0; i < WINO_OUT; ++i)
+        for (int s = 0; s < WINO_PTS; ++s) at[i * WINO_PTS + s] = wino_AT(i, s);
+    for (int s = 0; s < WINO_PTS; ++s) {
+        for (int k = 0; k < WINO_TAPS; ++k) g[s * WINO_TAPS + k] = wino_G(s, k);
+        for (int i = 0; i < WINO_PTS; ++i) bt[s * WINO_PTS + i] = wino_BT(s, i);
+    }
     return GVX_OK;
 }
 
@@ -572,7 +648,8 @@
     const PostnetPlan pp = make_postnet_plan(m, B, T);
     if (ws_bytes < pp.total) return fail(GVX_ERR_WORKSPACE, "workspace too small: %zu < %zu bytes", ws_bytes, pp.total);
     if (!mel_in || !mel_post_out) return fail(GVX_ERR_INVALID_ARG, "null argument");
-    return postnet_impl(m, mel_in, mel_lengths, B, T, mel_post_out, ws_ptr<float>(ws, pp.ya), ws_ptr<float>(ws, pp.yb), (hipStream_t)stream);
+    return postnet_impl(m, mel_in, mel_lengths, B, T, mel_post_out, ws_ptr<float>(ws, pp.ya), ws_ptr<float>(ws, pp.yb), ws_ptr<float>(ws, pp.wino), pp.wino_floats,
+                        (hipStream_t)stream);
 }
 
 int gvx_mask_padding(float* mel, float* mel_post, float* gate, const int32_t* mel_lengths, int B, int n_mels, int T, void* stream) {
@@ -617,7 +694,8 @@
     if (rc != GVX_OK) return rc;
     if (timed) HIP_TRY(hipEventRecord(m->ev[4], s));
     if (mel_post_out) {
-        rc = postnet_impl(m, mel_out, nullptr, B, T, mel_post_out, ws_ptr<float>(ws, wp.ya), ws_ptr<float>(ws, wp.yb), s);
+        rc = postnet_impl(m, mel_out, nullptr, B, T, mel_post_out, ws_ptr<float>(ws, wp.ya), ws_ptr<float>(ws, wp.yb), ws_ptr<float>(ws, wp.xa),
+                          (wp.ya - wp.xa) / sizeof(float), s);
         if (rc != GVX_OK) return rc;
         if (mel_lengths) HIP_TRY(launch_mask_padding(mel_out, mel_post_out, gate_out, mel_lengths, B, m->d.n_mels, T, s));
     }
diff --git a/genvox_amd/csrc/gvx_internal.h b/genvox_amd/csrc/gvx_internal.h
--- a/genvox_amd/csrc/gvx_internal.h
+++ b/genvox_amd/csrc/gvx_internal.h
@@ -1,6 +1,7 @@
 #pragma once
 #include "../../include/genvox_amd.h"
 #include "gvx_kernels.h"
+#include "winograd_f45.h"
 
 #include <cmath>
 #include <cstdarg>
@@ -34,8 +35,13 @@
     size_t dec_frag, dec_bias;
     size_t proj_w, proj_b, proj_frag, proj_hd_t, proj_ctx_frag, proj_ctx_t;
     size_t post_w[MAX_CONV], post_b[MAX_CONV];
+    size_t post_u[MAX_CONV];
     size_t total;
 };
+inline bool winograd_shape_ok(int cin, int cout, int k) { return k == WINO_TAPS && cin == cout && cin % 32 == 0; }
+inline bool postnet_layer_winograd_shape(const gvx_dims& d, int i) {
+    return i > 0 && i < d.postnet_n_conv - 1 && winograd_shape_ok(d.postnet_dim, d.postnet_dim, d.postnet_kernel);
+}
 Blob make_blob_layout(const gvx_dims& d);
 
 inline size_t frag_floats(int N, int K) { return (size_t)((N + 31) / 32) * (K / 8) * 64 * 4; }
@@ -68,6 +74,8 @@
     bool train_resident = true;
     bool train_resident_loop = true;
     bool attn_prefetch = true;
+    int winograd = 1;
+    int wino_group = 0;
     int enc_fork_after = 1;
     int pa_depth = 4;
     unsigned side_pool = 1;
@@ -158,6 +166,11 @@
 
 enum WsMode : int { WS_TEACHER_FORCED = 0, WS_AUTOREGRESSIVE = 1 };
 
+constexpr int WINOGRAD_MIN_CHANNELS = 256;
+constexpr size_t WINOGRAD_GROUP_BYTES = (size_t)128 << 20;
+bool conv_uses_winograd(const gvx_model* m, int cin, int cout, int k);
+size_t winograd_scratch_floats(const gvx_model* m, int B, int T);
+
 constexpr int FLAG_TOKEN = 0;
 constexpr int FLAG_AR_DONE = 1;
 constexpr int FLAG_TIMEOUT = 2;
diff --git a/genvox_amd/csrc/gvx_kernels.h b/genvox_amd/csrc/gvx_kernels.h
--- a/genvox_amd/csrc/gvx_kernels.h
+++ b/genvox_amd/csrc/gvx_kernels.h
@@ -39,6 +39,7 @@
     int m_begin = 0;
     const int32_t* row_len = nullptr;
     int c_halo = 0;
+    int slices = 1; long a_slice = 0, w_slice = 0, c_slice = 0;
 };
 hipError_t launch_gemm(const GemmParams& p, hipStream_t s);
 struct GemmPlan { hipError_t err; int tile; int rows_big; };
@@ -272,6 +273,8 @@
 hipError_t launch_residual_to_channels_first(const float* mel, const float* y, float* mel_post, int B, int M, int T,
                                              const int32_t* lens, hipStream_t s);
 hipError_t launch_zero_halo(float* buf, int B, int T, int halo, int C, hipStream_t s);
+hipError_t launch_winograd_input(const float* x, float* V, int B, long mt0, long nmt, int T, int C, hipStream_t s);
+hipError_t launch_winograd_output(const float* M, const float* bias, const int32_t* row_len, float* y, int B, long mt0, long nmt, int T, int C, hipStream_t s);
 hipError_t launch_mask_padding(float* mel, float* mel_post, float* gate, const int32_t* mel_lengths, int B, int M, int T,
                                hipStream_t s);
 hipError_t launch_zero_many(void* const* ptrs, const size_t* bytes, int n_arrays, hipStream_t s);
diff --git a/genvox_amd/csrc/gvx_pack.hip b/genvox_amd/csrc/gvx_pack.hip
--- a/genvox_amd/csrc/gvx_pack.hip
+++ b/genvox_amd/csrc/gvx_pack.hip
@@ -34,6 +34,8 @@
         b.post_w[i] = take((size_t)cout * d.postnet_kernel * cin);
         b.post_b[i] = take(cout);
     }
+    for (int i = 0; i < d.postnet_n_conv; ++i)
+        if (postnet_layer_winograd_shape(d, i)) b.post_u[i] = take((size_t)WINO_PTS * d.postnet_dim * d.postnet_dim);
     b.total = off;
     return b;
 }
@@ -66,7 +68,7 @@
     }
 };
 
-int pack_conv(const WeightTable& wt, const std::string& prefix, int cout, int cin, int k, float* w_out, float* b_out) {
+int pack_conv(const WeightTable& wt, const std::string& prefix, int cout, int cin, int k, float* w_out, float* b_out, float* u_out = nullptr) {
     int rc = GVX_OK;
     const float* w = wt.get(prefix + ".0.conv.weight", (int64_t)cout * cin * k, &rc); if (!w) return rc;
     const float* b = wt.get(prefix + ".0.conv.bias", cout, &rc); if (!b) return rc;
@@ -79,6 +81,10 @@
         for (int kk = 0; kk < k; ++kk)
             for (int ci = 0; ci < cin; ++ci)
                 w_out[((size_t)co * k + kk) * cin + ci] = (float)((double)w[((size_t)co * cin + ci) * k + kk] * scale);
+        if (u_out)
+            for (int ci = 0; ci < cin; ++ci)
+                for (int s = 0; s < WINO_PTS; ++s)
+                    u_out[((size_t)s * cout + co) * cin + ci] = wino_weight(w + ((size_t)co * cin + ci) * k, 1, scale, s);
         b_out[co] = (float)(((double)b[co] - (double)mu[co]) * scale + (double)beta[co]);
     }
     return GVX_OK;
@@ -214,7 +220,8 @@
     }
     for (int i = 0; i < d.postnet_n_conv; ++i) {
         const int cin = i == 0 ? M : d.postnet_dim, cout = i == d.postnet_n_conv - 1 ? M : d.postnet_dim;
-        rc = pack_conv(wt, "postnet.convolutions." + std::to_string(i), cout, cin, d.postnet_kernel, out + bl.post_w[i], out + bl.post_b[i]);
+        rc = pack_conv(wt, "postnet.convolutions." + std::to_string(i), cout, cin, d.postnet_kernel, out + bl.post_w[i], out + bl.post_b[i],
+                       postnet_layer_winograd_shape(d, i) ? out + bl.post_u[i] : nullptr);
         if (rc != GVX_OK) return rc;
     }
     return GVX_OK;
@@ -235,12 +242,14 @@
     }
 }
 __global__ void pack_conv_fold_kernel(const float* w, const float* b, const float* g, const float* beta, const float* mu, const float* var,
-                                      int cout, int cin, int k, float* w_out, float* b_out) {
+                                      int cout, int cin, int k, float* w_out, float* b_out, float* u_out) {
     const long n = (long)cout * cin * k;
     for (long i = (long)blockIdx.x * blockDim.x + threadIdx.x; i < n; i += (long)gridDim.x * blockDim.x) {
         const int ci = (int)(i % cin), kk = (int)((i / cin) % k), co = (int)(i / ((long)cin * k));
         const double scale = (double)g[co] / sqrt((double)var[co] + BN_EPS);
         w_out[i] = (float)((double)w[((long)co * cin + ci) * k + kk] * scale);
+        if (u_out && kk == 0)
+            for (int s = 0; s < WINO_PTS; ++s) u_out[((long)s * cout + co) * cin + ci] = wino_weight(w + ((long)co * cin + ci) * k, 1, scale, s);
         if (ci == 0 && kk == 0) b_out[co] = (float)(((double)b[co] - (double)mu[co]) * scale + (double)beta[co]);
     }
 }
@@ -297,6 +306,7 @@
     for (int i = 0; i < d.postnet_n_conv; ++i) {
         const int cin = i == 0 ? M : d.postnet_dim, cout = i == d.postnet_n_conv - 1 ? M : d.postnet_dim;
         mark(b.post_w[i], (size_t)cout * d.postnet_kernel * cin); mark(b.post_b[i], cout);
+        if (postnet_layer_winograd_shape(d, i)) mark(b.post_u[i], (size_t)WINO_PTS * cout * cin);
     }
     mark(b.enc_bih, (size_t)8 * H); mark(b.att_bias, (size_t)4 * d.att_rnn_dim); mark(b.dec_bias, (size_t)4 * d.dec_rnn_dim);
     for (size_t i = 0; i < total; ++i)
@@ -333,7 +343,7 @@
     const gvx_dims& d = m->d;
     const Blob& bl = m->blob;
     const int E = d.embed_dim, H = E / 2, M = d.n_mels;
-    auto conv = [&](const std::string& prefix, int cout, int cin, int k, size_t w_off, size_t b_off) -> int {
+    auto conv = [&](const std::string& prefix, int cout, int cin, int k, size_t w_off, size_t b_off, const size_t* u_off = nullptr) -> int {
         int r = GVX_OK;
         const float* w = dt.get(prefix + ".0.conv.weight", (int64_t)cout * cin * k, &r); if (!w) return r;
         const float* b = dt.get(prefix + ".0.conv.bias", cout, &r); if (!b) return r;
@@ -342,14 +352,16 @@
         const float* mu = dt.get(prefix + ".1.running_mean", cout, &r); if (!mu) return r;
         const float* var = dt.get(prefix + ".1.running_var", cout, &r); if (!var) return r;
         const long cnt = (long)cout * cin * k;
-        hipLaunchKernelGGL(pack_conv_fold_kernel, dim3((unsigned)((cnt + 255) / 256)), dim3(256), 0, s, w, b, g, beta, mu, var, cout, cin, k, out + w_off, out + b_off);
+        hipLaunchKernelGGL(pack_conv_fold_kernel, dim3((unsigned)((cnt + 255) / 256)), dim3(256), 0, s, w, b, g, beta, mu, var, cout, cin, k, out + w_off, out + b_off,
+                           u_off ? out + *u_off : (float*)nullptr);
         return GVX_OK;
     };
     for (int i = 0; i < d.enc_n_conv; ++i)
         if ((rc = conv("encoder.convolutions." + std::to_string(i), E, E, d.enc_kernel, bl.enc_w[i], bl.enc_b[i])) != GVX_OK) return rc;
     for (int i = 0; i < d.postnet_n_conv; ++i) {
         const int cin = i == 0 ? M : d.postnet_dim, cout = i == d.postnet_n_conv - 1 ? M : d.postnet_dim;
-        if ((rc = conv("postnet.convolutions." + std::to_string(i), cout, cin, d.postnet_kernel, bl.post_w[i], bl.post_b[i])) != GVX_OK) return rc;
+        if ((rc = conv("postnet.convolutions." + std::to_string(i), cout, cin, d.postnet_kernel, bl.post_w[i], bl.post_b[i],
+                       postnet_layer_winograd_shape(d, i) ? &bl.post_u[i] : nullptr)) != GVX_OK) return rc;
     }
     auto bias = [&](const std::string& bih_n, const std::string& bhh_n, int Hd, size_t o) -> int {
         int r = GVX_OK;
diff --git a/genvox_amd/csrc/train_ops.hip b/genvox_amd/csrc/train_ops.hip
--- a/genvox_amd/csrc/train_ops.hip
+++ b/genvox_amd/csrc/train_ops.hip
@@ -192,6 +192,17 @@
     return pl.err == hipSuccess ? GVX_OK : GVX_ERR_INVALID_ARG;
 }
 
+int gvx_debug_gemm_plan_batched(int M, int N, int K, int slices, int* tile_out, int* rows_big_out) {
+    if (!tile_out || !rows_big_out || M < 1 || N < 1 || K < 1 || slices < 1) return GVX_ERR_INVALID_ARG;
+    GemmParams g{};
+    g.amap = RowMap{M, 0, (long)K};
+    g.M = M; g.N = N; g.K = K;
+    g.slices = slices; g.a_slice = (long)M * K; g.w_slice = (long)N * K; g.c_slice = (long)M * N;
+    const GemmPlan pl = plan_gemm(g);
+    *tile_out = pl.tile; *rows_big_out = pl.rows_big;
+    return pl.err == hipSuccess ? GVX_OK : GVX_ERR_INVALID_ARG;
+}
+
 int gvx_train_gemm_nt(const float* A, long lda, const float* W, long ldw, float* C, long ldc, int M, int N, int K, const float* bias,
                       float* scratch, size_t scratch_bytes, void* stream) {
     if (!A || !W || !C || M < 1 || N < 1 || K < 4 || (K & 3)) return tfail(GVX_ERR_INVALID_ARG, "gemm_nt: null argument or K not a positive multiple of 4");
diff --git a/genvox_amd/csrc/winograd_conv.hip b/genvox_amd/csrc/winograd_conv.hip
--- /dev/null
+++ b/genvox_amd/csrc/winograd_conv.hip
@@ -0,0 +1,99 @@
+#include "gvx_kernels.h"
+#include "winograd_f45.h"
+
+namespace gvx {
+
+namespace {
+
+__device__ __forceinline__ float4 f4_fma(float a, const float4& x, const float4& y) {
+    return make_float4(fmaf(a, x.x, y.x), fmaf(a, x.y, y.y), fmaf(a, x.z, y.z), fmaf(a, x.w, y.w));
+}
+
+__global__ void __launch_bounds__(256) winograd_input_kernel(const float* __restrict__ x, float* __restrict__ V, long mt0, long nmt, int T, int C) {
+    const int tiles = (T + WINO_OUT - 1) / WINO_OUT, c4n = C >> 2;
+    const long total = nmt * c4n;
+    const long idx = (long)blockIdx.x * blockDim.x + threadIdx.x;
+    if (idx >= total) return;
+    const int c = (int)(idx % c4n) * 4;
+    const long lt = idx / c4n, mt = mt0 + lt;
+    const int b = (int)(mt / tiles), j = (int)(mt - (long)b * tiles);
+    const int rows = T + WINO_TAPS - 1;
+    const float* src = x + ((long)b * rows + 4 * j) * C + c;
+    float4 d[WINO_PTS];
+#pragma unroll
+    for (int i = 0; i < WINO_PTS; ++i)
+        d[i] = 4 * j + i < rows ? *reinterpret_cast<const float4*>(src + (long)i * C) : make_float4(0.f, 0.f, 0.f, 0.f);
+    const long slice = nmt * C;
+    float* dst = V + lt * C + c;
+#pragma unroll
+    for (int s = 0; s < WINO_PTS; ++s) {
+        float4 v = make_float4(0.f, 0.f, 0.f, 0.f);
+#pragma unroll
+        for (int i = 0; i < WINO_PTS; ++i)
+            if (wino_BT(s, i) != 0.f) v = f4_fma(wino_BT(s, i), d[i], v);
+        *reinterpret_cast<float4*>(dst + s * slice) = v;
+    }
+}
+
+__global__ void __launch_bounds__(256) winograd_output_kernel(const float* __restrict__ Mm, const float* __restrict__ bias, const int32_t* __restrict__ row_len,
+                                                              float* __restrict__ y, long mt0, long nmt, int T, int C) {
+    const int tiles = (T + WINO_OUT - 1) / WINO_OUT, c4n = C >> 2;
+    const long total = nmt * c4n;
+    const long idx = (long)blockIdx.x * blockDim.x + threadIdx.x;
+    if (idx >= total) return;
+    const int c = (int)(idx % c4n) * 4;
+    const long lt = idx / c4n, mt = mt0 + lt;
+    const int b = (int)(mt / tiles), j = (int)(mt - (long)b * tiles);
+    const long slice = nmt * C;
+    const float* src = Mm + lt * C + c;
+    float4 m[WINO_PTS];
+#pragma unroll
+    for (int s = 0; s < WINO_PTS; ++s) m[s] = *reinterpret_cast<const float4*>(src + s * slice);
+    const float4 bv = *reinterpret_cast<const float4*>(bias + c);
+    const int len = row_len ? row_len[b] : T;
+    constexpr int HALO = (WINO_TAPS - 1) / 2;
+    const int rows = T + 2 * HALO;
+    float* dst = y + ((long)b * rows + HALO) * C + c;
+    const float4 zero = make_float4(0.f, 0.f, 0.f, 0.f);
+#pragma unroll
+    for (int i = 0; i < WINO_OUT; ++i) {
+        const int t = 4 * j + i;
+        float4 v = zero;
+#pragma unroll
+        for (int s = 0; s < WINO_PTS; ++s)
+            if (wino_AT(i, s) != 0.f) v = f4_fma(wino_AT(i, s), m[s], v);
+        const bool live = t < len;
+        v = make_float4(live ? tanhf(v.x + bv.x) : 0.f, live ? tanhf(v.y + bv.y) : 0.f, live ? tanhf(v.z + bv.z) : 0.f, live ? tanhf(v.w + bv.w) : 0.f);
+        if (t < T) *reinterpret_cast<float4*>(dst + (long)t * C) = v;
+    }
+    if (j == 0) {
+#pragma unroll
+        for (int h = 1; h <= HALO; ++h) *reinterpret_cast<float4*>(dst - (long)h * C) = zero;
+    }
+    if (j == tiles - 1) {
+#pragma unroll
+        for (int h = 0; h < HALO; ++h) *reinterpret_cast<float4*>(dst + (long)(T + h) * C) = zero;
+    }
+}
+
+unsigned blocks_of(long nmt, int C) { return (unsigned)((nmt * (C >> 2) + 255) / 256); }
+bool bad_shape(int B, long mt0, long nmt, int T, int C) {
+    if (B < 1 || T < 1 || C < 4 || (C & 3) || mt0 < 0 || nmt < 1) return true;
+    return mt0 + nmt > (long)B * ((T + WINO_OUT - 1) / WINO_OUT) || nmt * (C >> 2) > ((long)1 << 38);
+}
+
+}
+
+hipError_t launch_winograd_input(const float* x, float* V, int B, long mt0, long nmt, int T, int C, hipStream_t s) {
+    if (bad_shape(B, mt0, nmt, T, C)) return hipErrorInvalidValue;
+    winograd_input_kernel<<<dim3(blocks_of(nmt, C)), dim3(256), 0, s>>>(x, V, mt0, nmt, T, C);
+    return hipGetLastError();
+}
+
+hipError_t launch_winograd_output(const float* Mm, const float* bias, const int32_t* row_len, float* y, int B, long mt0, long nmt, int T, int C, hipStream_t s) {
+    if (bad_shape(B, mt0, nmt, T, C)) return hipErrorInvalidValue;
+    winograd_output_kernel<<<dim3(blocks_of(nmt, C)), dim3(256), 0, s>>>(Mm, bias, row_len, y, mt0, nmt, T, C);
+    return hipGetLastError();
+}
+
+}
diff --git a/genvox_amd/csrc/winograd_f45.h b/genvox_amd/csrc/winograd_f45.h
--- /dev/null
+++ b/genvox_amd/csrc/winograd_f45.h
@@ -0,0 +1,54 @@
+#pragma once
+#include <hip/hip_runtime.h>
+
+namespace gvx {
+
+constexpr int WINO_OUT = 4;
+constexpr int WINO_TAPS = 5;
+constexpr int WINO_PTS = 8;
+
+__host__ __device__ inline double wino_G(int s, int k) {
+    constexpr double G[WINO_PTS][WINO_TAPS] = {
+        {1.0 / 4.0, 0, 0, 0, 0},
+        {1.0 / 18.0, 1.0 / 18.0, 1.0 / 18.0, 1.0 / 18.0, 1.0 / 18.0},
+        {1.0 / 18.0, -1.0 / 18.0, 1.0 / 18.0, -1.0 / 18.0, 1.0 / 18.0},
+        {1.0 / 360.0, 1.0 / 180.0, 1.0 / 90.0, 1.0 / 45.0, 2.0 / 45.0},
+        {1.0 / 360.0, -1.0 / 180.0, 1.0 / 90.0, -1.0 / 45.0, 2.0 / 45.0},
+        {16.0 / 45.0, 8.0 / 45.0, 4.0 / 45.0, 2.0 / 45.0, 1.0 / 45.0},
+        {16.0 / 45.0, -8.0 / 45.0, 4.0 / 45.0, -2.0 / 45.0, 1.0 / 45.0},
+        {0, 0, 0, 0, 1.0 / 4.0},
+    };
+    return G[s][k];
+}
+
+__host__ __device__ inline float wino_BT(int s, int i) {
+    constexpr float BT[WINO_PTS][WINO_PTS] = {
+        {4, 0, -21, 0, 21, 0, -4, 0},
+        {0, -4, -4, 17, 17, -4, -4, 0},
+        {0, 4, -4, -17, 17, 4, -4, 0},
+        {0, 2, 1, -10, -5, 8, 4, 0},
+        {0, -2, 1, 10, -5, -8, 4, 0},
+        {0, 4, 8, -5, -10, 1, 2, 0},
+        {0, -4, 8, 5, -10, -1, 2, 0},
+        {0, -4, 0, 21, 0, -21, 0, 4},
+    };
+    return BT[s][i];
+}
+
+__host__ __device__ inline float wino_AT(int i, int s) {
+    constexpr float AT[WINO_OUT][WINO_PTS] = {
+        {1, 1, 1, 1, 1, 1, 1, 0},
+        {0, 1, -1, 2, -2, 0.5f, -0.5f, 0},
+        {0, 1, 1, 4, 4, 0.25f, 0.25f, 0},
+        {0, 1, -1, 8, -8, 0.125f, -0.125f, 1},
+    };
+    return AT[i][s];
+}
+
+__host__ __device__ inline float wino_weight(const float* w, long ws, double scale, int s) {
+    double u = 0.0;
+    for (int k = 0; k < WINO_TAPS; ++k) u += wino_G(s, k) * ((double)w[k * ws] * scale);
+    return (float)u;
+}
+
+}
diff --git a/genvox_amd/tacotron2.py b/genvox_amd/tacotron2.py
--- a/genvox_amd/tacotron2.py
+++ b/genvox_amd/tacotron2.py
@@ -74,6 +74,7 @@
         self._workspace: Optional[torch.Tensor] = None
         self._lane_ws = [None, None]
         self._lane_streams = None
+        self._winograd_mode: Optional[int] = None
         self._lane_handles = [None, None]
         self._timing = False
         self._sticky_bad = False
@@ -260,6 +261,8 @@
                 _lib.check(lib.gvx_model_set_persistent_attention(h.value, 0))
                 if self._resident_off:
                     _lib.check(lib.gvx_model_set_resident_kernels(h.value, 0))
+                if self._winograd_mode is not None:
+                    _lib.check(lib.gvx_model_set_winograd(h.value, self._winograd_mode))
                 _lib.check(lib.gvx_model_bind_blob(h.value, self._blob.data_ptr()))
                 if self._timing:
                     _lib.check(lib.gvx_stage_timing_enable(h.value, 1))
@@ -291,6 +294,16 @@
     def enable_kernel_timing(self, enable: bool = True) -> None:
         self._ensure_packed()
         _lib.check(_lib.load().gvx_kernel_timing_enable(self._handle, int(enable)))
+
+    def set_winograd(self, mode: int) -> None:
+        self._ensure_handle()
+        for h in [self._handle] + self._lane_handles:
+            if h is not None:
+                _lib.check(_lib.load().gvx_model_set_winograd(h, int(mode)))
+        self._winograd_mode = int(mode)
+
+    def conv_plan(self, cin: int, cout: int, k: int) -> int:
+        return int(_lib.load().gvx_debug_conv_plan(self._ensure_handle(), cin, cout, k))
 
     def loop_kind(self, B: int, L: int) -> int:
         self._ensure_packed()
diff --git a/include/genvox_amd.h b/include/genvox_amd.h
--- a/include/genvox_amd.h
+++ b/include/genvox_amd.h
@@ -64,6 +64,9 @@
 int gvx_model_set_persistent_attention(gvx_model* model, int enable);
 
 int gvx_model_set_resident_kernels(gvx_model* model, int enable);
+
+int gvx_model_set_winograd(gvx_model* model, int mode);
+int gvx_debug_conv_plan(const gvx_model* model, int cin, int cout, int k);
 
 int gvx_teacher_forced_rows_per_call(const gvx_model* model, int L);
 
```

After: 1.971 million (median of 6 runs). 5.8% higher.
